# paulrozdeba/varanneal

Measured on AMD Instinct MI355X. Metric: action+grad evals/sec, Lorenz-96 D=20 N=1000, higher is better.
Workload: dtype f64; 1 GPU; lorenz96_D20_N1000_L7_B64_trapezoid; seeds_per_gpu=64, D=20, N=1000, L=7, disc=trapezoid, tile_rows=84, ntiles=12, parallelism=seeds sharded, 64 per GPU, rccl_ranks=1, ramp_launches=16000, launch_mode=hipGraph replay

## Files before the change

include/varanneal_amd.h:

```cpp
#ifndef VARANNEAL_AMD_H
#define VARANNEAL_AMD_H
#include <stdint.h>

#ifdef __cplusplus
extern "C" {
#endif

#define VA_ABI_VERSION 12

enum { VA_OK = 0, VA_EINVAL = -1, VA_ENOMEM = -2, VA_EHIP = -3, VA_EUNSUPPORTED = -4,
       VA_ESTATE = -5 };

enum { VA_DISC_EULER = 0, VA_DISC_TRAPEZOID = 1, VA_DISC_SIMPSON_HERMITE = 2,
       VA_DISC_FORWARDMAP = 3 };

enum { VA_RHS_LORENZ96 = 0, VA_RHS_USER_BASE = 1000 };

enum { VA_MEM_HOST = 0, VA_MEM_DEVICE = 1 };

typedef struct va_problem_s *va_handle;

typedef struct va_problem_desc {
    int32_t struct_size;
    int32_t device;
    int32_t batch;
    int32_t D;
    int32_t N_model;
    int32_t N_data;
    int32_t merr_nskip;
    int32_t L;
    const int32_t *Lidx;
    const double *Y;
    double dt_model;
    int32_t rm_kind;
    double rm;
    const double *rm_array;
    int32_t rf_kind;
    double rf0;
    const double *rf0_array;
    int32_t NP;
    int32_t NPest;
    const int32_t *Pidx;
    const double *P;
    int32_t disc;
    int32_t rhs;
    int32_t lbfgs_m;
    int32_t max_beta;
    int32_t keep_paths;
    int32_t tile_rows;
    int32_t eval_kernel;
    const double *t_model;
    const double *stim;
    int32_t n_stim;
    int32_t p_time_dependent;
    void *stream;
    const double *lower;
    const double *upper;
} va_problem_desc;

typedef struct va_lbfgs_opts {
    int32_t maxcor;
    double ftol;
    double gtol;
    int32_t maxiter;
    int64_t maxfun;
    int32_t maxls;
} va_lbfgs_opts;

int32_t va_abi_version(void);
const char *va_last_error(void);
int va_device_count(int32_t *count);

int va_rhs_load_module(const char *path, int32_t *rhs_id);

int va_eval_plan(const va_problem_desc *desc, int32_t ne, int32_t ghost, int32_t *out);
int va_eval_plan_reach(const va_problem_desc *desc, int32_t ne, int32_t ghost, const int32_t *reach, int32_t *out);

int va_problem_create(const va_problem_desc *desc, va_handle *out);
void va_problem_destroy(va_handle h);

int va_problem_info(va_handle h, int64_t *n_var, int64_t *ld_internal, int32_t *tile_rows,
                    int32_t *ntiles);

#define VA_TUNE_FOLD 1
#define VA_TUNE_GRAD_SC1 2
#define VA_TUNE_PRIO 3
#define VA_TUNE_GRAPH 4
#define VA_TUNE_PERSIST 5
#define VA_TUNE_PERSIST_ROWS 6
#define VA_TUNE_NNET_FUSED 7
int va_problem_tune(va_handle h, int32_t what, int32_t value);
int va_problem_persistent(va_handle h, int32_t *workgroups_per_seed, int32_t *rows_per_workgroup);

int va_problem_eval_kernel(va_handle h, int32_t *eval_kernel, int32_t *run_rows);

int va_action_grad(va_handle h, const double *XP, int64_t ld, int32_t mem, double rf_scale,
                   double *A, double *me, double *fe, double *grad, int64_t ldg);

int va_minimize_lbfgs(va_handle h, double *XP_inout, int64_t ld, int32_t mem, double rf_scale,
                      const va_lbfgs_opts *opts, double *Amin, double *me, double *fe,
                      int32_t *status, int32_t *nit, int64_t *nfev);

int va_anneal(va_handle h, double *XP_inout, int64_t ld, int32_t mem, const double *rf_scale,
              int32_t nbeta, const va_lbfgs_opts *opts, double *ame, double *pest,
              int32_t *status, int32_t *nit, int64_t *nfev, double *minpaths);

int va_get_minpath(va_handle h, int32_t seed, int32_t beta_idx, double *out);

int va_predict(va_handle h, const double *x0, const double *p, int32_t T, double t0,
               int32_t n_steps, int32_t substeps, int32_t every, const double *stim, double *out);

int va_hess_vec(va_handle h, const double *XP, const double *P, const double *V, int32_t npts, int32_t nvec, int64_t ld,
                double rf_scale, int32_t gauss_newton, int32_t tile_rows, double *HV);

int va_blocktri_selinv(va_handle h, int32_t npts, int32_t K, int32_t W, int32_t NPe, const double *Dk, const double *Bk,
                       const double *Pk, const double *Hpp, double *Skk, double *Snk, double *Spk, double *Spp, double *logdet,
                       int32_t *status);

int va_laplace(va_handle h, const double *XP, const double *P, int32_t npts, int64_t ld, const double *rf_scale,
               int32_t gauss_newton, int32_t chunk_pts, double *var_x, double *cov_xx, double *cov_px, double *cov_pp,
               double *logdet, int32_t *status);

int va_predict_tangent(va_handle h, const double *x0, const double *p, const double *V0, int32_t T, int32_t nvec, double t0,
                       int32_t n_steps, int32_t substeps, int32_t every, const double *stim, double *out, double *dX,
                       double *var, double *cov);

int va_hmc(va_handle h, double *XP, int64_t ld, int32_t mem, double rf_scale, int32_t n_iter, int32_t n_leap, const double *eps,
           double jitter, const double *minv, int64_t minv_n, uint64_t seed, const double *noise, int32_t thin,
           const int64_t *keep_idx, int32_t n_keep_idx, double *mean, double *var, double *A_trace, double *dH, int32_t *accepted,
           int32_t *n_divergent, double *kept);
int va_hmc_noise(uint64_t seed, int32_t chain, int32_t iteration, int64_t n, uint32_t *words, double *normals, double *uniforms);

int va_eval_timed(va_handle h, double rf_scale, int32_t iters, float *elapsed_ms);
int va_eval_timed_prepare(va_handle h, double rf_scale, int32_t iters);

int va_lbfgs_timed(va_handle h, int32_t iters, float *ms_update, float *ms_direction);
int va_eval_ls_timed(va_handle h, double rf_scale, int32_t iters, float *ms_eval);

int va_read_eval_outputs(va_handle h, double *A, double *me, double *fe, double *grad, int64_t ldg);

int va_debug_read_partials(va_handle h, double *out, int64_t n);

int va_debug_read_persist(va_handle h, double *out, int64_t n);

int va_get_counters(va_handle h, int64_t *eval_launches, int64_t *seed_evals, int64_t *cycles);

typedef struct va_comm_s *va_comm;
#define VA_COMM_ID_BYTES 128
int va_comm_unique_id(char id[VA_COMM_ID_BYTES]);
int va_comm_create(const char id[VA_COMM_ID_BYTES], int32_t world, int32_t rank, int32_t device, va_comm *out);
void va_comm_destroy(va_comm c);
int va_gather_results(va_handle h, va_comm c, int32_t nbeta, double *table, int32_t *status);

enum { VA_ACT_SIGMOID = 0,
       VA_ACT_TANH = 1, VA_ACT_LINEAR = 2,
       VA_ACT_RELU = 3,
       VA_ACT_SOFTPLUS = 4,
       VA_ACT_USER_BASE = 1000  };

typedef struct va_nnet_desc {
    int32_t struct_size;
    int32_t device;
    int32_t batch;
    int32_t n_layers;
    const int32_t *structure;
    int32_t M;
    int32_t L_in, L_out;
    const int32_t *Lidx_in;
    const int32_t *Lidx_out;
    const double *data_in;
    const double *data_out;
    double rm_in, rm_out;
    double rf0;
    int32_t NP, NPest;
    const int32_t *Pidx;
    const double *P;
    int32_t activation;
    int32_t lbfgs_m;
    int32_t max_beta;
    int32_t keep_paths;
    void *stream;
    const double *rm_in_matrix;
    const double *rm_out_matrix;
} va_nnet_desc;

int va_act_load_module(const char *path, int32_t *act_id);

int va_nnet_problem_create(const va_nnet_desc *desc, va_handle *out);

#ifdef __cplusplus
}
#endif
#endif
```

varanneal_amd/_build.py:

```python
import os
import subprocess
import sys

HERE = os.path.dirname(os.path.abspath(__file__))
CSRC = os.path.join(HERE, "csrc")
OUT = os.path.join(HERE, "libvaranneal_amd.so")
SOURCES = ["va_capi.hip", "va_kernels.hip", "va_eval5.hip", "va_lbfgsb.hip", "va_nnet.hip", "va_hmc.hip"]
HEADERS = ["va_core.h", "va_tile2.h", "va_tile3.h", "va_tile4.h", "va_tile5.h", "va_eval3.h", "va_eval4.h", "va_eval5.h", "va_eval_flat.h", "va_epilogue.h", "va_persist.h", "va_persist_geo.h", "va_predict.h", "va_predict_geo.h", "va_predict_tlm.h", "va_predict_tlm_geo.h", "va_hvp.h", "va_hvp_geo.h", "va_selinv.h", "va_selinv_geo.h", "va_hmc.h", "va_hmc_geo.h", "va_eval_geo.h", "va_measure.h", "va_device.h", "va_nnet.h", "va_nnet_geo.h", "va_nnet_kernels.h", os.path.join("..", "..", "include", "varanneal_amd.h")]
HIPCC = os.environ.get("HIPCC", "/opt/rocm/bin/hipcc")
SCHED = ["-mllvm", "-amdgpu-sched-strategy=iterative-maxocc"]
FLAGS = ["--offload-arch=gfx950", "-O3", "-std=c++17", "-fPIC", "-shared", "-Wall", "-Wno-unused-function", "-ldl"] + SCHED


def needs_build():
    if not os.path.exists(OUT):
        return True
    t = os.path.getmtime(OUT)
    deps = [os.path.join(CSRC, f) for f in SOURCES + HEADERS] + [os.path.abspath(__file__)]
    return any(os.path.getmtime(d) > t for d in deps)


def _compile_link(out, defines, verbose):
    from concurrent.futures import ThreadPoolExecutor
    objdir = os.path.join(HERE, "build", os.path.basename(out).replace(".so", ""))
    os.makedirs(objdir, exist_ok=True)
    cflags = [f for f in FLAGS if f not in ("-shared", "-ldl")]

    def stale(obj, dep, cmd):
        try:
            with open(dep) as fh:
                txt = fh.read()
            if txt.split("\n", 1)[0] != "# " + " ".join(cmd):
                return True
            t = os.path.getmtime(obj)
            files = txt.split(":", 1)[1].replace("\\\n", " ").split()
            return any(os.path.getmtime(f) > t for f in files)
        except (OSError, IndexError):
            return True

    def one(src):
        obj = os.path.join(objdir, src.replace(".hip", ".o"))
        dep = obj + ".d"
        cmd = [HIPCC] + cflags + defines + ["-c", "-o", obj, os.path.join(CSRC, src)]
        if not stale(obj, dep, cmd):
            return obj
        if verbose:
            print(" ".join(cmd), flush=True)
        subprocess.check_call(cmd + ["-MD", "-MF", dep + ".tmp"])
        with open(dep + ".tmp") as fh:
            body = fh.read()
        with open(dep, "w") as fh:
            fh.write("# " + " ".join(cmd) + "\n" + body)
        os.remove(dep + ".tmp")
        return obj
    with ThreadPoolExecutor(max_workers=min(len(SOURCES), os.cpu_count() or 1)) as ex:
        objs = list(ex.map(one, SOURCES))
    cmd = [HIPCC, "--offload-arch=gfx950", "-shared", "-fPIC", "-o", out] + objs + ["-ldl"]
    if verbose:
        print(" ".join(cmd), flush=True)
    subprocess.check_call(cmd)
    return out


def build_stamps(verbose=True):
    return _compile_link(os.path.join(HERE, "libvaranneal_amd_stamps.so"), ["-DVA_STAMPS"], verbose)


def build_variant(tag, defines, verbose=True):
    return _compile_link(os.path.join(HERE, "libvaranneal_amd_%s.so" % tag), list(defines), verbose)


def build(force=False, verbose=True):
    if not force and not needs_build():
        return OUT
    return _compile_link(OUT, [], verbose)


if __name__ == "__main__":
    if "--variant" in sys.argv:
        i = sys.argv.index("--variant")
        build_variant(sys.argv[i + 1], sys.argv[i + 2:])
    elif "--stamps" in sys.argv:
        build_stamps()
    else:
        build(force="--force" in sys.argv)
```

varanneal_amd/_capi.py:

```python
import ctypes as C
import os

import numpy as np

_HERE = os.path.dirname(os.path.abspath(__file__))
LIB_PATH = os.environ.get("VARANNEAL_AMD_LIB", os.path.join(_HERE, "libvaranneal_amd.so"))

VA_OK = 0
VA_EUNSUPPORTED = -4
ABI_VERSION = 12
ERRNAMES = {-1: "VA_EINVAL", -2: "VA_ENOMEM", -3: "VA_EHIP", -4: "VA_EUNSUPPORTED", -5: "VA_ESTATE"}
DISC = {"euler": 0, "trapezoid": 1, "SimpsonHermite": 2, "forwardmap": 3}
RHS = {"lorenz96": 0}
MEM_HOST, MEM_DEVICE = 0, 1

c_dp = C.POINTER(C.c_double)
c_ip = C.POINTER(C.c_int32)
c_lp = C.POINTER(C.c_int64)


class VaLibraryError(RuntimeError):
    pass


# ... 43 lines not shown
                ("maxiter", C.c_int32), ("maxfun", C.c_int64), ("maxls", C.c_int32)]


def make_opts(opt_args=None):
    o = dict(opt_args or {})
    return LbfgsOpts(int(o.get("maxcor", 10)), float(o.get("ftol", 2.2204460492503131e-09)),
                     float(o.get("gtol", 1e-5)), int(min(int(o.get("maxiter", 15000)), 2 ** 31 - 1)),
                     int(o.get("maxfun", 15000)), int(o.get("maxls", 20)))


def _f64(a):
    return np.ascontiguousarray(a, dtype=np.float64)


def make_desc(batch, D, N_model, Y, Lidx, dt_model, RM, RF0, P, Pidx, disc="trapezoid",
              rhs="lorenz96", merr_nskip=1, lbfgs_m=10, max_beta=1, keep_paths=0, tile_rows=0,
              eval_kernel=0, device=0, stream=None, t_model=None, stim=None, p_time_dependent=False, bounds=None):
    Y = _f64(Y)
    N_data, L = Y.shape
    Lidx = np.ascontiguousarray(Lidx, dtype=np.int32)
    Pidx = np.ascontiguousarray(Pidx, dtype=np.int32)
    P = _f64(P)
    if p_time_dependent:
        if P.ndim == 2:
            P = np.ascontiguousarray(np.broadcast_to(P, (batch,) + P.shape))
        if P.ndim != 3 or P.shape[:2] != (batch, N_model):
            raise ValueError("time-dependent P must have shape (batch, N_model, NP)")
    elif P.ndim == 1:
        P = np.ascontiguousarray(np.broadcast_to(P, (batch, P.shape[0])))
    keep = [Y, Lidx, Pidx, P]
    d = ProblemDesc()
    d.struct_size = C.sizeof(ProblemDesc)
    d.device, d.batch, d.D, d.N_model, d.N_data = device, batch, D, N_model, N_data
    d.merr_nskip, d.L = merr_nskip, L
    d.Lidx = Lidx.ctypes.data_as(c_ip)
    d.Y = Y.ctypes.data_as(c_dp)
    d.dt_model = float(dt_model)
    if isinstance(RM, np.ndarray):
        rm = _f64(RM)
        if rm.shape not in [(N_data, L), (N_data, L, L)]:
            raise ValueError("RM array must have shape (N_data, L) or (N_data, L, L)")
        keep.append(rm)
        d.rm_kind, d.rm, d.rm_array = rm.ndim - 1, 0.0, rm.ctypes.data_as(c_dp)
    else:
        d.rm_kind, d.rm, d.rm_array = 0, float(RM), None
    if isinstance(RF0, np.ndarray):
        rf = _f64(RF0)
        if rf.shape not in [(N_model - 1, D), (N_model - 1, D, D)]:
            raise ValueError("RF0 array must have shape (N_model-1, D) or (N_model-1, D, D)")
        keep.append(rf)
        d.rf_kind, d.rf0, d.rf0_array = rf.ndim - 1, 0.0, rf.ctypes.data_as(c_dp)
    else:
        d.rf_kind, d.rf0, d.rf0_array = 0, float(RF0), None
    d.NP, d.NPest = P.shape[-1], len(Pidx)
    d.p_time_dependent = 1 if p_time_dependent else 0
    d.Pidx = Pidx.ctypes.data_as(c_ip)
    d.P = P.ctypes.data_as(c_dp)
    d.disc = DISC[disc] if isinstance(disc, str) else int(disc)
    d.rhs = RHS[rhs] if isinstance(rhs, str) else int(rhs)
    d.lbfgs_m, d.max_beta, d.keep_paths, d.tile_rows = lbfgs_m, max_beta, keep_paths, tile_rows
    d.eval_kernel = eval_kernel
    if t_model is not None:
        tm = _f64(t_model)
        if tm.shape != (N_model,):
            raise ValueError("t_model must have shape (N_model,)")
        keep.append(tm)
        d.t_model = tm.ctypes.data_as(c_dp)
    else:
        d.t_model = None
    if stim is not None:
        st = _f64(stim)
        st = st.reshape(N_model, -1)
        keep.append(st)
        d.stim, d.n_stim = st.ctypes.data_as(c_dp), st.shape[1]
    else:
        d.stim, d.n_stim = None, 0
    d.stream = stream
    d.lower = d.upper = None
    if bounds is not None:
        n_var = N_model * (D + len(Pidx)) if p_time_dependent else N_model * D + len(Pidx)
        if len(bounds) != n_var:
            raise ValueError("bounds must have one (lo, hi) pair per entry of the path vector (%d), got %d" % (n_var, len(bounds)))
        lo = np.array([-np.inf if b[0] is None else b[0] for b in bounds], dtype=np.float64)
        hi = np.array([np.inf if b[1] is None else b[1] for b in bounds], dtype=np.float64)
        keep += [lo, hi]
        d.lower, d.upper = lo.ctypes.data_as(c_dp), hi.ctypes.data_as(c_dp)
    return d, keep


_lib = None


def lib():
    global _lib
    if _lib is not None:
        return _lib
    if not os.path.exists(LIB_PATH):
        raise VaLibraryError("%s not found: build it with `python -m varanneal_amd._build` "
                             "(hipcc --offload-arch=gfx950). There is no CPU fallback." % LIB_PATH)
    try:
        L = C.CDLL(LIB_PATH)
    except OSError as e:
        raise VaLibraryError("cannot load %s: %s" % (LIB_PATH, e))
    h = C.c_void_p
    L.va_abi_version.restype = C.c_int32
    if L.va_abi_version() != ABI_VERSION:
        raise VaLibraryError("%s has ABI version %d, this binding expects %d: rebuild it with "
                             "`python -m varanneal_amd._build --force`" % (LIB_PATH, L.va_abi_version(), ABI_VERSION))
    L.va_last_error.restype = C.c_char_p
    L.va_device_count.argtypes = [c_ip]
    L.va_problem_create.argtypes = [C.POINTER(ProblemDesc), C.POINTER(h)]
    L.va_nnet_problem_create.argtypes = [C.POINTER(NnetDesc), C.POINTER(h)]
    L.va_rhs_load_module.argtypes = [C.c_char_p, c_ip]
    L.va_act_load_module.argtypes = [C.c_char_p, c_ip]
    L.va_eval_plan.argtypes = [C.POINTER(ProblemDesc), C.c_int32, C.c_int32, C.POINTER(C.c_int32)]
    L.va_eval_plan_reach.argtypes = [C.POINTER(ProblemDesc), C.c_int32, C.c_int32, C.POINTER(C.c_int32), C.POINTER(C.c_int32)]
    L.va_problem_destroy.argtypes = [h]
    L.va_problem_destroy.restype = None
    L.va_problem_info.argtypes = [h, c_lp, c_lp, c_ip, c_ip]
    L.va_action_grad.argtypes = [h, C.c_void_p, C.c_int64, C.c_int32, C.c_double, C.c_void_p,
                                 C.c_void_p, C.c_void_p, C.c_void_p, C.c_int64]
    L.va_minimize_lbfgs.argtypes = [h, C.c_void_p, C.c_int64, C.c_int32, C.c_double,
                                    C.POINTER(LbfgsOpts), c_dp, c_dp, c_dp, c_ip, c_ip, c_lp]
    L.va_anneal.argtypes = [h, C.c_void_p, C.c_int64, C.c_int32, c_dp, C.c_int32,
                            C.POINTER(LbfgsOpts), c_dp, c_dp, c_ip, c_ip, c_lp, c_dp]
    L.va_get_minpath.argtypes = [h, C.c_int32, C.c_int32, c_dp]
    L.va_predict.argtypes = [h, c_dp, c_dp, C.c_int32, C.c_double, C.c_int32, C.c_int32, C.c_int32, c_dp, c_dp]
    L.va_predict_tangent.argtypes = [h, c_dp, c_dp, c_dp, C.c_int32, C.c_int32, C.c_double, C.c_int32, C.c_int32, C.c_int32] + [c_dp] * 5
    L.va_predict_tangent.restype = C.c_int
    L.va_hess_vec.argtypes = [h, c_dp, c_dp, c_dp, C.c_int32, C.c_int32, C.c_int64, C.c_double, C.c_int32, C.c_int32, c_dp]
    L.va_hess_vec.restype = C.c_int
    L.va_blocktri_selinv.argtypes = [h, C.c_int32, C.c_int32, C.c_int32, C.c_int32] + [c_dp] * 9 + [c_ip]
    L.va_blocktri_selinv.restype = C.c_int
    L.va_laplace.argtypes = [h, c_dp, c_dp, C.c_int32, C.c_int64, c_dp, C.c_int32, C.c_int32] + [c_dp] * 5 + [c_ip]
    L.va_laplace.restype = C.c_int
    L.va_hmc.argtypes = [h, C.c_void_p, C.c_int64, C.c_int32, C.c_double, C.c_int32, C.c_int32, c_dp, C.c_double, c_dp, C.c_int64,
                         C.c_uint64, c_dp, C.c_int32, c_lp, C.c_int32, c_dp, c_dp, c_dp, c_dp, c_ip, c_ip, c_dp]
    L.va_hmc.restype = C.c_int
    L.va_hmc_noise.argtypes = [C.c_uint64, C.c_int32, C.c_int32, C.c_int64, C.POINTER(C.c_uint32), c_dp, c_dp]
    L.va_hmc_noise.restype = C.c_int
    L.va_eval_timed.argtypes = [h, C.c_double, C.c_int32, C.POINTER(C.c_float)]
    L.va_eval_timed_prepare.argtypes = [h, C.c_double, C.c_int32]
    L.va_get_counters.argtypes = [h, c_lp, c_lp, c_lp]
    L.va_comm_unique_id.argtypes = [C.c_char_p]
    L.va_comm_create.argtypes = [C.c_char_p, C.c_int32, C.c_int32, C.c_int32, C.POINTER(h)]
    L.va_comm_destroy.argtypes = [h]
    L.va_comm_destroy.restype = None
    L.va_gather_results.argtypes = [h, h, C.c_int32, c_dp, c_ip]
    L.va_lbfgs_timed.argtypes = [h, C.c_int32, C.POINTER(C.c_float), C.POINTER(C.c_float)]
    L.va_eval_ls_timed.argtypes = [h, C.c_double, C.c_int32, C.POINTER(C.c_float)]
    L.va_read_eval_outputs.argtypes = [h, C.c_void_p, C.c_void_p, C.c_void_p, C.c_void_p, C.c_int64]
    L.va_debug_read_partials.argtypes = [h, c_dp, C.c_int64]
    L.va_problem_eval_kernel.argtypes = [h, c_ip, c_ip]
    L.va_problem_tune.argtypes = [h, C.c_int32, C.c_int32]
    L.va_debug_read_persist.argtypes = [h, c_dp, C.c_int64]
    L.va_debug_read_persist.restype = C.c_int
    L.va_problem_persistent.argtypes = [h, c_ip, c_ip]
    L.va_problem_persistent.restype = C.c_int
    for fn in ("va_device_count", "va_rhs_load_module", "va_act_load_module", "va_eval_plan", "va_eval_plan_reach", "va_problem_eval_kernel", "va_problem_tune", "va_problem_create", "va_nnet_problem_create",
               "va_problem_info", "va_action_grad",
               "va_minimize_lbfgs", "va_anneal", "va_get_minpath", "va_predict", "va_eval_timed", "va_eval_timed_prepare",
               "va_get_counters", "va_debug_read_partials", "va_read_eval_outputs", "va_lbfgs_timed", "va_eval_ls_timed",
               "va_comm_unique_id", "va_comm_create", "va_gather_results"):
        getattr(L, fn).restype = C.c_int
    _lib = L
    return L


EXPORTS = ["va_abi_version", "va_last_error", "va_device_count", "va_rhs_load_module", "va_act_load_module", "va_eval_plan", "va_eval_plan_reach", "va_problem_eval_kernel", "va_problem_tune", "va_problem_create",
           "va_problem_destroy", "va_problem_info", "va_action_grad", "va_minimize_lbfgs",
           "va_anneal", "va_get_minpath", "va_predict", "va_predict_tangent", "va_hess_vec", "va_blocktri_selinv", "va_laplace", "va_hmc", "va_hmc_noise", "va_eval_timed", "va_eval_timed_prepare", "va_problem_persistent", "va_debug_read_persist", "va_get_counters", "va_nnet_problem_create", "va_debug_read_partials",
           "va_read_eval_outputs", "va_lbfgs_timed", "va_eval_ls_timed", "va_comm_unique_id", "va_comm_create", "va_comm_destroy",
           "va_gather_results"]


def check(rc):
    if rc != VA_OK:
        raise (VaUnsupported if rc == VA_EUNSUPPORTED else VaError)(rc, lib().va_last_error().decode("utf-8", "replace"))


def eval_plan(batch, D, N_model, disc, ne, ghost=0, rm_array=False, rm_full=False, rf_array=False, rf_full=False,
              merr_nskip=1, tile_rows=0, eval_kernel=0, bounded=False, p_time_dependent=False, reach=None, Lidx=None,
              builtin=False):
    d = ProblemDesc()
    d.struct_size = C.sizeof(ProblemDesc)
    d.rhs = 0 if builtin else 1000
    d.batch, d.D, d.N_model, d.merr_nskip = batch, D, N_model, merr_nskip
    d.N_data = (N_model - 1) // merr_nskip + 1
    d.rm_kind = (2 if rm_full else 1) if rm_array else 0
    d.rf_kind = (2 if rf_full else 1) if rf_array else 0
    d.disc = DISC[disc] if isinstance(disc, str) else int(disc)
    d.tile_rows, d.eval_kernel = tile_rows, eval_kernel
    d.p_time_dependent = 1 if p_time_dependent else 0
    dummy = (C.c_double * 1)()
    if bounded:
        d.lower = C.cast(dummy, c_dp); d.upper = C.cast(dummy, c_dp)
    out = (C.c_int32 * 4)()
    if reach is not None and Lidx is not None and len(Lidx) > 0:
        li = np.ascontiguousarray(Lidx, dtype=np.int32)
        d.L = len(li)
        d.Lidx = li.ctypes.data_as(c_ip)
        r = (C.c_int32 * 4)(*[int(v) for v in reach])
        check(lib().va_eval_plan_reach(C.byref(d), int(ne), int(ghost), r, out))
    else:
        check(lib().va_eval_plan(C.byref(d), int(ne), int(ghost), out))
    return (out[0], out[1], out[2], out[3]) if out[0] else None


def hmc_noise(seed, chain, iteration, n):
    n = int(n)
    words = np.empty((n + 1, 4), np.uint32); normals = np.empty(n); uniforms = np.empty(2)
    check(lib().va_hmc_noise(int(seed) & (2 ** 64 - 1), int(chain), int(iteration), n, words.ctypes.data_as(C.POINTER(C.c_uint32)),
                             normals.ctypes.data_as(c_dp), uniforms.ctypes.data_as(c_dp)))
    return words, normals, uniforms


_modules = {}


def load_rhs_module(path):
    path = os.path.abspath(path)
    if path not in _modules:
        rid = C.c_int32()
        check(lib().va_rhs_load_module(path.encode(), C.byref(rid)))
        _modules[path] = rid.value
    return _modules[path]


_act_modules = {}


def load_act_module(path):
    path = os.path.abspath(path)
    if path not in _act_modules:
        aid = C.c_int32()
        check(lib().va_act_load_module(path.encode(), C.byref(aid)))
        _act_modules[path] = aid.value
    return _act_modules[path]


class Comm(object):

    @staticmethod
    def unique_id():
        buf = C.create_string_buffer(128)
        check(lib().va_comm_unique_id(buf))
        return buf.raw

    def __init__(self, uid, world, rank, device=0):
        self._L = lib()
        self.world, self.rank = world, rank
        self._c = C.c_void_p()
        check(self._L.va_comm_create(uid, world, rank, device, C.byref(self._c)))

    def close(self):
        if getattr(self, "_c", None) is not None and self._c.value:
            self._L.va_comm_destroy(self._c)
            self._c = C.c_void_p()

    __del__ = close


class Problem(object):

    def __init__(self, batch, D, N_model, Y, Lidx, dt_model, RM, RF0, P, Pidx, **kw):
        self._L = lib()
        self.desc, self._keep = make_desc(batch, D, N_model, Y, Lidx, dt_model, RM, RF0, P, Pidx, **kw)
        self.B, self.D, self.N = batch, D, N_model
        self.NP, self.NPest = self.desc.NP, self.desc.NPest
        self.n_var = N_model * D + self.NPest
        if self.desc.p_time_dependent:
            self.n_var = N_model * (D + self.NPest)
            self.NPe_t, self.NPt = self.NPest, self.NP
            self.N, self.D, self.NP, self.NPest = 1, self.n_var, 0, 0
        self.max_beta = self.desc.max_beta
        self._h = C.c_void_p()
        check(self._L.va_problem_create(C.byref(self.desc), C.byref(self._h)))

    def close(self):
        if getattr(self, "_h", None) is not None and self._h.value:
            self._L.va_problem_destroy(self._h)
            self._h = C.c_void_p()

    __del__ = close

    def __enter__(self):
        return self

    def __exit__(self, *a):
        self.close()

    def info(self):
        nv, ld = C.c_int64(), C.c_int64()
        T, nt = C.c_int32(), C.c_int32()
        check(self._L.va_problem_info(self._h, C.byref(nv), C.byref(ld), C.byref(T), C.byref(nt)))
        ek, rr = C.c_int32(), C.c_int32()
        check(self._L.va_problem_eval_kernel(self._h, C.byref(ek), C.byref(rr)))
        return dict(n_var=nv.value, ld=ld.value, tile_rows=T.value, ntiles=nt.value, eval_kernel=ek.value,
                    run_rows=rr.value)

    TUNE = {"fold": 1, "grad_sc1": 2, "prio": 3, "graph": 4, "persist": 5, "persist_rows": 6, "nnet_fused": 7}

    def debug_read_persist(self, n):
        out = np.empty(n)
        check(self._L.va_debug_read_persist(self._h, out.ctypes.data_as(c_dp), n))
        return out

    def persistent(self):
        g, t = C.c_int32(), C.c_int32()
        on = self._L.va_problem_persistent(self._h, C.byref(g), C.byref(t))
        return (g.value, t.value) if on else None

    def tune(self, **knobs):
        for k, v in knobs.items():
            check(self._L.va_problem_tune(self._h, self.TUNE[k], int(v)))

    def _xp(self, XP):
        XP = _f64(XP)
        if XP.shape != (self.B, self.n_var):
            raise ValueError("XP must have shape (B, N*D+NPest) = (%d, %d), got %s" %
                             (self.B, self.n_var, XP.shape))
        return XP

    def action_grad(self, XP, rf_scale=1.0, want_grad=True):
        XP = self._xp(XP)
        A = np.empty(self.B); me = np.empty(self.B); fe = np.empty(self.B)
        g = np.empty((self.B, self.n_var)) if want_grad else None
        check(self._L.va_action_grad(self._h, XP.ctypes.data, self.n_var, MEM_HOST, float(rf_scale),
                                     A.ctypes.data, me.ctypes.data, fe.ctypes.data,
                                     g.ctypes.data if want_grad else None, self.n_var))
        return A, me, fe, g

    def action_grad_device(self, xp_ptr, ld, rf_scale, A_ptr, me_ptr, fe_ptr, g_ptr, ldg):
        check(self._L.va_action_grad(self._h, xp_ptr, ld, MEM_DEVICE, float(rf_scale), A_ptr, me_ptr,
                                     fe_ptr, g_ptr, ldg))

    def minimize_lbfgs(self, XP, rf_scale, opt_args=None):
        XP = self._xp(XP).copy()
        o = make_opts(opt_args)
        A = np.empty(self.B); me = np.empty(self.B); fe = np.empty(self.B)
        st = np.empty(self.B, np.int32); nit = np.empty(self.B, np.int32); nfev = np.empty(self.B, np.int64)
        check(self._L.va_minimize_lbfgs(self._h, XP.ctypes.data, self.n_var, MEM_HOST, float(rf_scale),
                                        C.byref(o), A.ctypes.data_as(c_dp), me.ctypes.data_as(c_dp),
                                        fe.ctypes.data_as(c_dp), st.ctypes.data_as(c_ip),
                                        nit.ctypes.data_as(c_ip), nfev.ctypes.data_as(c_lp)))
        return dict(x=XP, A=A, me=me, fe=fe, status=st, nit=nit, nfev=nfev)

    def anneal(self, XP, rf_scale, opt_args=None, want_paths=False, xp_device=None, ld=None):
        rf = _f64(rf_scale)
        nb = rf.shape[0]
        o = make_opts(opt_args)
        B = self.B
        ame = np.empty((B, nb, 3)); pest = np.empty((B, nb, self.NPest))
        st = np.empty((B, nb), np.int32); nit = np.empty((B, nb), np.int32); nfev = np.empty((B, nb), np.int64)
        mp = np.empty((B, nb, self.N * self.D + self.NP)) if want_paths else None
        if xp_device is None:
            XP = self._xp(XP).copy()
            ptr, stride, mem = XP.ctypes.data, self.n_var, MEM_HOST
        else:
            ptr, stride, mem = xp_device, ld, MEM_DEVICE
        check(self._L.va_anneal(self._h, ptr, stride, mem, rf.ctypes.data_as(c_dp), nb, C.byref(o),
                                ame.ctypes.data_as(c_dp), pest.ctypes.data_as(c_dp),
                                st.ctypes.data_as(c_ip), nit.ctypes.data_as(c_ip),
                                nfev.ctypes.data_as(c_lp), mp.ctypes.data_as(c_dp) if want_paths else None))
        return dict(x=XP if xp_device is None else None, A=ame[:, :, 0], me=ame[:, :, 1],
                    fe=ame[:, :, 2], pest=pest, status=st, nit=nit, nfev=nfev, minpaths=mp)

    def predict(self, x0, p, n_steps, t0=0.0, substeps=1, every=1, stim=None):
        if not isinstance(self.desc, ProblemDesc):
            raise NotImplementedError("predict: a network handle has no differential equation to integrate")
        D, NP = self.desc.D, self.desc.NP
        x0 = _f64(x0).reshape(-1, D)
        T = x0.shape[0]
        p = _f64(p).reshape(-1, NP) if NP else np.zeros((T, 0))
        if p.shape[0] == 1 and T > 1:
            p = np.ascontiguousarray(np.broadcast_to(p, (T, NP)))
        if p.shape[0] != T:
            raise ValueError("predict: %d states but %d parameter vectors" % (T, p.shape[0]))
        n_steps, substeps, every = int(n_steps), int(substeps), int(every)
        st = None
        if stim is not None:
            st = _f64(stim).reshape(max(n_steps, 0) + 1, -1)
            if st.shape[1] != self.desc.n_stim and self.desc.n_stim:
                raise ValueError("predict: the stimulus must have %d rows of %d column(s)" % (n_steps + 1, self.desc.n_stim))
        out = np.empty((T, n_steps // every + 1 if every >= 1 and n_steps >= 1 else 1, D))
        check(self._L.va_predict(self._h, x0.ctypes.data_as(c_dp), p.ctypes.data_as(c_dp), T, float(t0), n_steps, substeps,
                                 every, st.ctypes.data_as(c_dp) if st is not None else None, out.ctypes.data_as(c_dp)))
        return out

    def predict_tangent(self, x0, p, V0, n_steps, t0=0.0, substeps=1, every=1, stim=None, want=("dx", "var")):
        if not isinstance(self.desc, ProblemDesc):
            raise NotImplementedError("predict_tangent: a network handle has no differential equation to integrate")
        bad = set(want) - {"dx", "var", "cov"}
        if bad:
            raise ValueError("predict_tangent: want holds 'dx', 'var', 'cov', not %s" % sorted(bad))
        D, NP, nw = self.desc.D, self.desc.NP, self.desc.D + self.NPest
        x0 = _f64(x0).reshape(-1, D)
        T = x0.shape[0]
        p = _f64(p).reshape(-1, NP) if NP else np.zeros((T, 0))
        if p.shape[0] == 1 and T > 1:
            p = np.ascontiguousarray(np.broadcast_to(p, (T, NP)))
        if p.shape[0] != T:
            raise ValueError("predict_tangent: %d states but %d parameter vectors" % (T, p.shape[0]))
        V0 = _f64(V0)
        if V0.size == 0:
            raise ValueError("predict_tangent: at least one direction (nvec = 0)")
        if V0.shape[-1:] != (nw,) or V0.size % (T * nw):
            raise ValueError("predict_tangent: V0 must have shape (%d, nvec, D + NPest = %d), got %s" % (T, nw, V0.shape))
        V0 = V0.reshape(T, -1, nw)
        nvec = V0.shape[1]
        n_steps, substeps, every = int(n_steps), int(substeps), int(every)
        st = None
        if stim is not None:
            st = _f64(stim).reshape(max(n_steps, 0) + 1, -1)
            if st.shape[1] != self.desc.n_stim and self.desc.n_stim:
                raise ValueError("predict_tangent: the stimulus must have %d rows of %d column(s)" % (n_steps + 1, self.desc.n_stim))
        n_out = n_steps // every + 1 if every >= 1 and n_steps >= 1 else 1
        r = dict(out=np.empty((T, n_out, D)))
        for name, shape in (("dx", (T, nvec, n_out, D)), ("var", (T, n_out, D)), ("cov", (T, n_out, D, D))):
            if name in want:
                r[name] = np.empty(shape)
        ptr = lambda a: a.ctypes.data_as(c_dp) if a is not None else None
        check(self._L.va_predict_tangent(self._h, ptr(x0), ptr(p), ptr(V0), T, nvec, float(t0), n_steps, substeps, every, ptr(st),
                                         ptr(r["out"]), ptr(r.get("dx")), ptr(r.get("var")), ptr(r.get("cov"))))
        return r

    def hess_vec(self, XP, V, rf_scale, P=None, gauss_newton=False, tile_rows=0):
        if not isinstance(self.desc, ProblemDesc):
            raise NotImplementedError("hess_vec: the network action has no second derivatives here (ODE handles only)")
        n = self.n_var
        XP = _f64(XP).reshape(-1, n)
        npts = XP.shape[0]
        V = _f64(V)
        one = V.ndim == 2 and npts == 1
        V = V.reshape(npts, -1, n)
        NP = self.desc.NP
        if P is None:
            P = np.ctypeslib.as_array(self.desc.P, shape=(NP,)) if (NP and not self.desc.p_time_dependent) else np.zeros(NP)
        P = _f64(P).reshape(-1, NP) if NP else np.zeros((npts, 0))
        if P.shape[0] == 1 and npts > 1:
            P = np.ascontiguousarray(np.broadcast_to(P, (npts, NP)))
        if P.shape[0] != npts:
            raise ValueError("hess_vec: %d points but %d parameter vectors" % (npts, P.shape[0]))
        HV = np.empty_like(V)
        check(self._L.va_hess_vec(self._h, XP.ctypes.data_as(c_dp), P.ctypes.data_as(c_dp), V.ctypes.data_as(c_dp), npts,
                                  V.shape[1], n, float(rf_scale), 1 if gauss_newton else 0, int(tile_rows), HV.ctypes.data_as(c_dp)))
        return HV[0] if one else HV

    def blocktri_selinv(self, Dk, Bk, Pk, Hpp, want=("Skk", "Snk", "Spk", "Spp")):
        Dk = _f64(Dk)
        npts, K, W = Dk.shape[:3]
        Hpp = _f64(Hpp).reshape(npts, -1)
        NPe = int(round(np.sqrt(Hpp.shape[1])))
        Bk, Pk = _f64(Bk).reshape(npts, K - 1, W, W), _f64(Pk).reshape(npts, K, NPe, W)
# ... 164 lines not shown
```

varanneal_amd/csrc/va_capi.hip:

```cpp
#include <dlfcn.h>
#include <link.h>
#include <stdarg.h>
#include <stdio.h>
#include <stdlib.h>
#include <string.h>

#include <algorithm>
#include <memory>
#include <mutex>
#include <string>
#include <vector>

#include "../../include/varanneal_amd.h"
#include "va_device.h"
#include "va_eval_geo.h"
#include "va_nnet.h"
#include "va_eval_flat.h"
#include "va_persist.h"
#include "va_predict.h"
#include "va_predict_tlm.h"
#include "va_hvp.h"
#include "va_selinv.h"
#include "va_hmc.h"

using namespace va;

namespace {

thread_local std::string g_err;

int fail(int code, const char *fmt, ...)
{
    char buf[512];
    va_list ap;
    va_start(ap, fmt);
    vsnprintf(buf, sizeof buf, fmt, ap);
    va_end(ap);
    g_err = buf;
    return code;
}

#define HIPCHK(expr)                                                                       \
    do {                                                                                   \
        hipError_t e_ = (expr);                                                            \
        if (e_ != hipSuccess)                                                              \
            return fail(e_ == hipErrorOutOfMemory ? VA_ENOMEM : VA_EHIP, "%s: %s (%s:%d)", \
                        #expr, hipGetErrorString(e_), __FILE__, __LINE__);                 \
    } while (0)

#define TRY(expr)                       \
    do {                                \
        if (int rc_ = (expr)) return rc_; \
    } while (0)
#define UPLOAD(dst, src, n) h->upload(dst, src, n, #dst)

struct UserRhs {
    ModuleVariant variant;
    std::string path;
    void *dl = nullptr;
    RhsTable table = {};
    HvpTable hvp = {};
    std::vector<int> colp;
};
struct UserAct {
    std::string path;
    void *dl = nullptr;
    NnetActLaunch launch = nullptr;
};
std::vector<UserAct> g_user_act;
std::vector<UserRhs> g_user_rhs;
std::mutex g_user_rhs_mutex;

}

struct va_problem_s {
    Dev dv;
    int device = 0, rhs = 0, keep_paths = 0;
    RhsTable rt = {};
    HvpTable rt_hvp = {};
    NnetActLaunch nn_act = nullptr;
    bool persist = false, tune_persist = true;
    int pz_G = 0, pz_T = 0, pz_maxG = 0;
    void *pz_misc = nullptr;
    size_t pz_xch_bytes = 0;
    bool is_nnet = false;
    bool fold = false;
    bool tune_graph = true;
    hipGraphExec_t timed_gexec = nullptr;
    int timed_chunk = 0;
    Dev timed_dv;
    NnetDev timed_nn;
    double timed_armed_rf = -1.0;
    NnetDev nn;
    hipStream_t stream = nullptr;
    bool own_stream = false;
    std::vector<void *> allocs;
    int *h_nactive = nullptr;
    double *d_rf = nullptr;
    hipEvent_t ev0 = nullptr, ev1 = nullptr;
    int64_t n_eval_launch = 0, n_seed_evals = 0, n_seed_evals_direct = 0, n_cycles = 0;
    int last_nbeta = 0;

    template <class T> int alloc(T **p, size_t n, bool zero = true)
    {
        void *q = nullptr;
        size_t bytes = sizeof(T) * (n ? n : 1);
        HIPCHK(hipMalloc(&q, bytes));
        allocs.push_back(q);
        if (zero) HIPCHK(hipMemsetAsync(q, 0, bytes, stream));
        *p = (T *)q;
        return VA_OK;
    }
    template <class T> int upload(T *dst, const T *src, size_t n, const char *name)
    {
        hipError_t e = hipMemcpyAsync(dst, src, sizeof(T) * n, hipMemcpyHostToDevice, stream);
        if (e != hipSuccess) return fail(VA_EHIP, "H2D %s: %s", name, hipGetErrorString(e));
        return VA_OK;
    }
};

struct HandleDeleter { void operator()(va_problem_s *h) const { va_problem_destroy(h); } };
typedef std::unique_ptr<va_problem_s, HandleDeleter> HandleOwner;

namespace {

void run_eval(va_handle h, int epi)
{
    if (epi != EPI_FINALIZE) h->timed_armed_rf = -1.0;
    h->dv.lsrun = epi == EPI_LS ? 1 : 0;
    EvalOp op{false, h->stream, hipSuccess};
    if (h->is_nnet ? !h->nn.small : !h->fold) {
        h->dv.epi = EPI_NONE;
        if (h->is_nnet) launch_nnet_eval(h->dv, h->nn, h->stream, h->nn_act);
        else h->rt.eval(h->dv, op);
        if (epi == EPI_FINALIZE) launch_finalize_eval(h->dv, h->stream);
        else if (epi == EPI_LS) launch_ls(h->dv, h->stream);
        return;
    }
    h->dv.epi = epi;
    if (h->is_nnet) { launch_nnet_eval(h->dv, h->nn, h->stream, h->nn_act); return; }
    h->rt.eval(h->dv, op);
}

int alloc_solver_state(va_handle h)
{
    Dev &dv = h->dv;
    const Dims &dm = dv.dm;
    const size_t B = dm.B, ld = dm.ld, m = dm.m, max_beta = dv.max_beta;
    const size_t guard = (((size_t)(dm.T + 8) * dm.D + 15) / 16) * 16;
    TRY(h->alloc(&dv.x, B * ld + 2 * guard)); TRY(h->alloc(&dv.g, B * ld));
    TRY(h->alloc(&dv.gt, B * ld)); TRY(h->alloc(&dv.d, B * ld + 2 * guard));
    dv.x += guard; dv.d += guard;
    TRY(h->alloc(&dv.S, B * m * ld)); TRY(h->alloc(&dv.Y, B * m * ld));
    TRY(h->alloc(&dv.st, B));
    TRY(h->alloc(&dv.evp, B * dm.nprow * EP_N));
    dv.npbig = (!h->is_nnet && !dv.cpv && dm.NPt > RHS_MAX_NP) ? dm.NPt - RHS_MAX_NP : 0;
    if (dv.npbig) TRY(h->alloc(&dv.evp_big, B * dm.nprow * dv.npbig));
    if (dv.cpv) TRY(h->alloc(&dv.evv, B * dm.nprow * dv.cpv));
    TRY(h->alloc(&dv.upp, B * dm.nchunks * dv.ups));
    TRY(h->alloc(&dv.dpp, B * dm.nchunks * DP_N));
    TRY(h->alloc(&h->d_rf, max_beta));
    TRY(h->alloc(&dv.ame, B * max_beta * 3));
    TRY(h->alloc(&dv.pest, B * max_beta * (dm.NPest ? dm.NPest : 1)));
    TRY(h->alloc(&dv.status, B * max_beta)); TRY(h->alloc(&dv.nit, B * max_beta));
    TRY(h->alloc(&dv.nfev, B * max_beta));
    if (h->keep_paths) TRY(h->alloc(&dv.minpaths, B * max_beta * (size_t)(dm.ND + dm.NP), false));
    if (dm.bounded) {
        TRY(h->alloc(&dv.lb_z, B * ld)); TRY(h->alloc(&dv.lb_r, B * ld)); TRY(h->alloc(&dv.lb_xp, B * ld));
        TRY(h->alloc(&dv.lb_t, B * ld)); TRY(h->alloc(&dv.lb_iwhere, B * ld));
        TRY(h->alloc(&dv.lb_mat, B * 3 * m * m)); TRY(h->alloc(&dv.lb_dtd, B));
    }
    TRY(h->alloc(&dv.cnt_eval, B * CNT_STRIDE)); TRY(h->alloc(&dv.cnt_upd, B * CNT_STRIDE)); TRY(h->alloc(&dv.cnt_dir, B * CNT_STRIDE));
    TRY(h->alloc(&dv.n_active, 1));
    TRY(h->alloc(&dv.n_evals, 1));
    TRY(h->alloc(&dv.outA, B)); TRY(h->alloc(&dv.outme, B)); TRY(h->alloc(&dv.outfe, B));
    dv.rf_ladder = h->d_rf;
    return VA_OK;
}

int finish_create(va_handle h)
{
    hipError_t e = hipHostMalloc((void **)&h->h_nactive, 4 * sizeof(int), hipHostMallocDefault);
    if (e != hipSuccess) return fail(VA_ENOMEM, "hipHostMalloc: %s", hipGetErrorString(e));
    e = hipEventCreate(&h->ev0);
    if (e == hipSuccess) e = hipEventCreate(&h->ev1);
    if (e != hipSuccess) return fail(VA_EHIP, "hipEventCreate: %s", hipGetErrorString(e));
    e = hipStreamSynchronize(h->stream);
    if (e != hipSuccess) return fail(VA_EHIP, "create sync: %s", hipGetErrorString(e));
    launch_init_states(h->dv, PH_IDLE, 1.0, h->stream);
    return VA_OK;
}

int copy_in(va_handle h, const double *XP, int64_t ld, int32_t mem)
{
    const Dims &dm = h->dv.dm;
    const size_t w = sizeof(double) * (dm.ND + dm.NPest);
    HIPCHK(hipMemcpy2DAsync(h->dv.x, sizeof(double) * dm.ld, XP, sizeof(double) * ld, w, dm.B,
                            mem == VA_MEM_DEVICE ? hipMemcpyDeviceToDevice : hipMemcpyHostToDevice,
                            h->stream));
    return VA_OK;
}

int copy_out(va_handle h, const double *src, double *dst, int64_t ld, int32_t mem)
{
    const Dims &dm = h->dv.dm;
    const size_t w = sizeof(double) * (dm.ND + dm.NPest);
    HIPCHK(hipMemcpy2DAsync(dst, sizeof(double) * ld, src, sizeof(double) * dm.ld, w, dm.B,
                            mem == VA_MEM_DEVICE ? hipMemcpyDeviceToDevice : hipMemcpyDeviceToHost,
                            h->stream));
    return VA_OK;
}

int check_xp(va_handle h, const void *XP, int64_t ld, int32_t mem)
{
    if (!h) return fail(VA_EINVAL, "null handle");
    if (!XP) return fail(VA_EINVAL, "XP is NULL");
    if (ld < h->dv.dm.ND + h->dv.dm.NPest) return fail(VA_EINVAL, "ld (%lld) < n_var (%d)", (long long)ld, h->dv.dm.ND + h->dv.dm.NPest);
    if (mem != VA_MEM_HOST && mem != VA_MEM_DEVICE) return fail(VA_EINVAL, "bad mem kind %d", mem);
    return VA_OK;
}

int set_opts(va_handle h, const va_lbfgs_opts *o)
{
    if (!o) return fail(VA_EINVAL, "opts is NULL");
    if (o->maxls <= 0) return fail(VA_EINVAL, "maxls must be positive");
    if (o->maxcor <= 0) return fail(VA_EINVAL, "maxcor must be positive");
    Opts &d = h->dv.o;
    d.m = o->maxcor < h->dv.dm.m ? o->maxcor : h->dv.dm.m;
    d.maxiter = o->maxiter; d.maxls = o->maxls; d.maxfun = o->maxfun;
    d.ftol = o->ftol; d.gtol = o->gtol;
    return VA_OK;
}

bool profiler_attached()
{
    static const bool attached = [] {
        bool found = false;
        dl_iterate_phdr([](struct dl_phdr_info *info, size_t, void *out) -> int {
            const char *n = info->dlpi_name;
            if (n && (strstr(n, "librocprofiler-sdk.so") || strstr(n, "librocprofiler-sdk-tool"))) { *(bool *)out = true; return 1; }
            return 0;
        }, &found);
        return found;
    }();
    return attached;
}

long long ladder_cycle_bound(const Dev &dv, int nbeta)
{
    const double per_step = (double)dv.o.maxfun + dv.o.maxls + 4.0;
    const double bound = per_step * nbeta;
    return bound > 4e18 ? (long long)4e18 : (long long)bound;
}

int arm_ladder(va_handle h, const double *rf_scale, int nbeta, bool zero_dpp)
{
    Dev &dv = h->dv;
    HIPCHK(hipMemcpyAsync(h->d_rf, rf_scale, sizeof(double) * nbeta, hipMemcpyHostToDevice, h->stream));
    dv.nbeta = nbeta; h->last_nbeta = nbeta;
    *h->h_nactive = dv.dm.B;
    HIPCHK(hipMemcpyAsync(dv.n_active, h->h_nactive, sizeof(int), hipMemcpyHostToDevice, h->stream));
    if (zero_dpp) HIPCHK(hipMemsetAsync(dv.dpp, 0, sizeof(double) * dv.dm.B * dv.dm.nchunks * DP_N, h->stream));
    launch_init_states(dv, PH_START, -1.0, h->stream);
    h->timed_armed_rf = -1.0;
    return VA_OK;
}

int read_progress(va_handle h, void *misc = nullptr)
{
    const Dev &dv = h->dv;
    HIPCHK(hipMemcpyAsync(h->h_nactive, dv.n_active, sizeof(int), hipMemcpyDeviceToHost, h->stream));
    HIPCHK(hipMemcpyAsync(h->h_nactive + 2, dv.n_evals, sizeof(unsigned long long), hipMemcpyDeviceToHost, h->stream));
    if (misc) HIPCHK(hipMemcpyAsync(misc, h->pz_misc, 16, hipMemcpyDeviceToHost, h->stream));
    HIPCHK(hipStreamSynchronize(h->stream));
    return VA_OK;
}

void book_ladder(va_handle h, long long cyc)
{
    h->n_cycles += cyc; h->n_eval_launch += cyc;
    h->n_seed_evals = h->n_seed_evals_direct + (int64_t)*(unsigned long long *)(h->h_nactive + 2);
}

int run_ladder_persist(va_handle h, const double *rf_scale, int nbeta, bool *fell_back);

int run_ladder(va_handle h, const double *rf_scale, int nbeta)
{
    Dev &dv = h->dv;
    if (nbeta < 1 || nbeta > dv.max_beta) return fail(VA_EINVAL, "nbeta=%d outside [1, max_beta=%d]", nbeta, dv.max_beta);
    if (h->persist && h->tune_persist) {
        bool fell_back = false;
        const int rc = run_ladder_persist(h, rf_scale, nbeta, &fell_back);
        if (!fell_back) return rc;
    }
    TRY(arm_ladder(h, rf_scale, nbeta, true));
    if (dv.dm.bounded) launch_clamp_x(dv, h->stream);
    const long long max_cycles = ladder_cycle_bound(dv, nbeta);
    long long cyc = 0;
    int poll = 4;
    hipGraphExec_t gexec = nullptr;
    bool use_graph = h->tune_graph && !profiler_attached();
    auto enqueue = [&](int n) {
// ... 55 lines not shown
    TRY(read_progress(h, &misc));
    HIPCHK(hipGetLastError());
    book_ladder(h, (long long)misc.cycles);
    if (misc.abort_flag == 1) {
        h->persist = false;
        *fell_back = true;
        return VA_OK;
    }
    if (misc.abort_flag == 2) return fail(VA_ESTATE, "ladder did not finish within %lld cycles", max_cycles);
    if (*h->h_nactive > 0) return fail(VA_ESTATE, "persistent ladder ended with %d live seeds", *h->h_nactive);
    return VA_OK;
}

template <class T>
int fetch_table(va_handle h, const T *dev, T *host, int nbeta, int per)
{
    if (!host) return VA_OK;
    const Dev &dv = h->dv;
    HIPCHK(hipMemcpy2DAsync(host, sizeof(T) * nbeta * per, dev, sizeof(T) * dv.max_beta * per,
                            sizeof(T) * nbeta * per, dv.dm.B, hipMemcpyDeviceToHost, h->stream));
    return VA_OK;
}

void colp_refusal(const va_problem_desc *d, const ModuleVariant &mv, char *msg, size_t n)
{
    if (const char *flat_only = flat_only_reason(d)) snprintf(msg, n, "%s", flat_only);
    else if (d->D > 64 && (d->D & 1)) snprintf(msg, n, "odd D = %d > 64 (k_eval3, which has no column-parameter form)", d->D);
    else if (d->D > 64 && mv.kernel != 5) snprintf(msg, n, "a non-autonomous model (model time or stimulus) on the streaming kernel k_eval5");
    else if (d->D <= 64 && !tile4_ok(d->D)) snprintf(msg, n, "D = %d fits neither k_eval4 (even D <= 64 filling a wave) nor k_eval5", d->D);
    else if (d->eval_kernel != 0 && d->eval_kernel != mv.kernel) snprintf(msg, n, "eval_kernel = %d (the module carries kernel %d)", d->eval_kernel, mv.kernel);
    else snprintf(msg, n, "the module's column-run instantiation does not fit this problem (weights, discretisation or run length): regenerate it");
}

struct ModulePlan {
    EvalPlan plan;
    bool variant = false;
    int cps = 0, cpv = 0;
};
int plan_module(const va_problem_desc *d, const UserRhs &u, ModulePlan &mp)
{
    const ModuleVariant &mv = u.variant;
    const bool bigp = d->NP > RHS_MAX_NP;
    mp.plan = plan_eval(d, bigp && !mv.column_params() ? mv.flat_form() : mv.form());
    mp.variant = mp.plan.emode != 1 && variant_key(mp.plan, d) == mv.key();
    if (!mp.variant && mp.plan.emode != 1) mp.plan = plan_eval(d, mv.flat_form());
    if (mp.variant && mv.column_params()) { mp.cps = u.colp[0]; mp.cpv = u.colp[1] * d->D; }
    if (d->NP > RHS_BIG_NP && !mp.cpv) {
        char why[192];
        colp_refusal(d, mv, why, sizeof why);
        return fail(VA_EUNSUPPORTED, "%d parameters: only the column-parameter form on k_eval4 / k_eval5 carries more than %d, "
                                     "and this problem cannot run it: %s", d->NP, RHS_BIG_NP, why);
    }
    if (mp.plan.emode == 4 && mp.cpv > mp.plan.g4.XW)
        return fail(VA_EUNSUPPORTED, "runs of %d rows are too short for %d vector entries on k_eval4", mp.plan.g4.K, mp.cpv);
    return VA_OK;
}


int begin_create(int device, void *stream, int lbfgs_m, int max_beta, int keep_paths, HandleOwner &h)
{
    const int m = lbfgs_m > 0 ? lbfgs_m : 10;
    if (m > MAX_M) return fail(VA_EINVAL, "lbfgs_m=%d > %d", m, MAX_M);
    int ndev = 0;
    HIPCHK(hipGetDeviceCount(&ndev));
    if (device < 0 || device >= ndev) return fail(VA_EINVAL, "device %d of %d", device, ndev);
    HIPCHK(hipSetDevice(device));

    h.reset(new va_problem_s());
    h->device = device; h->keep_paths = keep_paths;
    if (stream) h->stream = (hipStream_t)stream;
    else {
        hipError_t e = hipStreamCreateWithFlags(&h->stream, hipStreamNonBlocking);
        if (e != hipSuccess) return fail(VA_EHIP, "hipStreamCreate: %s", hipGetErrorString(e));
        h->own_stream = true;
    }
    Dev &dv = h->dv;
    memset(&dv, 0, sizeof dv);
    dv.dm.m = m;
    dv.ups = UP_OLD + 4 * m; dv.max_beta = max_beta > 0 ? max_beta : 1; dv.nbeta = 1;
    dv.o.m = m; dv.o.maxiter = 15000; dv.o.maxls = 20; dv.o.maxfun = 15000; dv.o.ftol = 2.2204460492503131e-09; dv.o.gtol = 1e-5;
    return VA_OK;
}

void set_ld(Dims &dm)
{
    dm.ld = ((dm.ND + dm.NPest + 15) / 16) * 16;
    dm.chunk = VEC_CHUNK; dm.nchunks = (dm.ld + VEC_CHUNK - 1) / VEC_CHUNK;
}

int validate_desc(const va_problem_desc *d, UserRhs &user_copy, const UserRhs **user)
{
    if (d->struct_size != (int32_t)sizeof(va_problem_desc)) return fail(VA_EINVAL, "struct_size %d != %zu", d->struct_size, sizeof(va_problem_desc));
    if (d->batch < 1 || d->D < 1 || d->N_model < 2 || d->N_data < 1 || d->L < 0 || d->merr_nskip < 1)
        return fail(VA_EINVAL, "bad sizes (batch=%d D=%d N_model=%d N_data=%d L=%d nskip=%d)", d->batch, d->D, d->N_model, d->N_data, d->L, d->merr_nskip);
    if ((int64_t)(d->N_data - 1) * d->merr_nskip + 1 != d->N_model)
        return fail(VA_EINVAL, "N_model (%d) must equal (N_data-1)*merr_nskip+1 (%lld)", d->N_model,
                    (long long)(d->N_data - 1) * d->merr_nskip + 1);
    if (d->disc < VA_DISC_EULER || d->disc > VA_DISC_FORWARDMAP) return fail(VA_EINVAL, "unknown disc %d", d->disc);
    if (d->disc == VA_DISC_SIMPSON_HERMITE && (d->N_model % 2) == 0)
        return fail(VA_EINVAL, "SimpsonHermite needs an odd number of time points (N_model=%d)", d->N_model);
    *user = nullptr;
    if (d->rhs >= VA_RHS_USER_BASE) {
        std::lock_guard<std::mutex> lock(g_user_rhs_mutex);
        if ((size_t)(d->rhs - VA_RHS_USER_BASE) >= g_user_rhs.size()) return fail(VA_EINVAL, "rhs module id %d was never registered", d->rhs);
        user_copy = g_user_rhs[d->rhs - VA_RHS_USER_BASE];
        *user = &user_copy;
        const RhsTable &t = user_copy.table;
        if (t.NP != d->NP || t.D != d->D || t.NSTIM != d->n_stim)
            return fail(VA_EINVAL, "rhs module %s was generated for D=%d NP=%d n_stim=%d, problem has D=%d NP=%d n_stim=%d",
                        user_copy.path.c_str(), t.D, t.NP, t.NSTIM, d->D, d->NP, d->n_stim);
    } else if (d->rhs != VA_RHS_LORENZ96) return fail(VA_EUNSUPPORTED, "unknown built-in rhs %d", d->rhs);
    if (d->rhs == VA_RHS_LORENZ96 && (d->NP != RhsL96::NP || d->D < 4))
        return fail(VA_EINVAL, "Lorenz-96 needs NP=1 and D>=4 (NP=%d D=%d)", d->NP, d->D);
    if (d->n_stim < 0 || (d->n_stim > 0 && !d->stim)) return fail(VA_EINVAL, "n_stim=%d without a stimulus array", d->n_stim);
    if (d->NP > RHS_BIG_NP && !(*user && !user_copy.colp.empty()))
        return fail(VA_EUNSUPPORTED, "NP=%d > %d: only a generated module in column-parameter form (shared scalars + per-column "
                                     "vectors) carries more, and this model has none", d->NP, RHS_BIG_NP);
    if (d->NPest < 0 || d->NPest > d->NP) return fail(VA_EINVAL, "bad NP/NPest (%d/%d)", d->NP, d->NPest);
    const bool tdp = d->p_time_dependent != 0;
    if (d->NP > RHS_MAX_NP && tdp) return fail(VA_EUNSUPPORTED, "time-dependent parameters: at most %d of them", RHS_MAX_NP);
    if (tdp && d->disc != VA_DISC_TRAPEZOID && d->disc != VA_DISC_SIMPSON_HERMITE)
        return fail(VA_EUNSUPPORTED, "time-dependent parameters: trapezoid and SimpsonHermite only (upstream's euler/forwardmap "
                                     "branches are inconsistent, va_ode.py:345-349)");
    if (tdp && (int64_t)d->N_model * (d->D + d->NPest) > 2000000000LL) return fail(VA_EUNSUPPORTED, "n_var does not fit 32-bit indexing");
    if (!d->Y || (d->L > 0 && !d->Lidx) || !d->P || (d->NPest > 0 && !d->Pidx)) return fail(VA_EINVAL, "null array in desc");
    if ((d->rm_kind && !d->rm_array) || (d->rf_kind && !d->rf0_array)) return fail(VA_EINVAL, "rm/rf array kind without array");
    if ((d->lower != nullptr) != (d->upper != nullptr)) return fail(VA_EINVAL, "lower and upper bounds come together");
    std::vector<char> seen(d->D, 0);
    for (int l = 0; l < d->L; ++l) {
        if (d->Lidx[l] < 0 || d->Lidx[l] >= d->D) return fail(VA_EINVAL, "Lidx[%d]=%d outside [0,D)", l, d->Lidx[l]);
        if (seen[d->Lidx[l]] && d->rm_kind != 2) return fail(VA_EUNSUPPORTED, "Lidx lists state column %d twice", d->Lidx[l]);
        seen[d->Lidx[l]] = 1;
    }
    for (int k = 0; k < d->NPest; ++k)
        if (d->Pidx[k] < 0 || d->Pidx[k] >= d->NP) return fail(VA_EINVAL, "Pidx[%d]=%d outside [0,NP)", k, d->Pidx[k]);
    if (d->lbfgs_m > MAX_M) return fail(VA_EINVAL, "lbfgs_m=%d > %d", d->lbfgs_m, MAX_M);
    if (d->rm_kind < 0 || d->rm_kind > 2) return fail(VA_EINVAL, "rm_kind %d", d->rm_kind);
    if (d->lower) {
        const int nv = tdp ? d->N_model * (d->D + d->NPest) : d->D * d->N_model + d->NPest;
        for (int i = 0; i < nv; ++i)
            if (!(d->lower[i] <= d->upper[i])) return fail(VA_EINVAL, "lower[%d] > upper[%d] (or NaN)", i, i);
    }
    return VA_OK;
}

int plan_problem(va_handle h, const va_problem_desc *d, const UserRhs *user, EvalPlan &plan)
{
    Dev &dv = h->dv;
    h->rhs = d->rhs;
    if (!user) {
        builtin_rhs_table(h->rt);
        builtin_hvp_table(h->rt_hvp);
        EvalForm l96;
        l96.ne = RhsL96s::NE; l96.ghost = RhsL96g::GHOST; l96.has_reach5 = true;
        l96.reach5[0] = t5_xl<RhsL96s>(); l96.reach5[1] = t5_xr<RhsL96s>(); l96.reach5[2] = t5_gl<RhsL96s>(); l96.reach5[3] = t5_gr<RhsL96s>();
        plan = plan_eval(d, l96);
        return VA_OK;
    }
    ModulePlan mp;
    TRY(plan_module(d, *user, mp));
    plan = mp.plan;
    h->rt = user->table;
    h->rt_hvp = user->hvp;
    if (mp.variant) h->rt.eval = user->table.eval_var;
    dv.dm.lin = user->variant.has_linear;
    dv.cps = mp.cps; dv.cpv = mp.cpv;
    dv.cpnsg = (mp.cpv && plan.emode == 5) ? plan.g5.NSG : 0;
    return VA_OK;
}

int fill_dims(va_handle h, const va_problem_desc *d, const EvalPlan &plan)
{
    Dev &dv = h->dv;
    Dims &dm = dv.dm;
    const bool tdp = d->p_time_dependent != 0;
    dm.D = d->D; dm.N = d->N_model; dm.ND = dm.D * dm.N; dm.L = d->L; dm.N_data = d->N_data;
    dm.nskip = d->merr_nskip; dm.NP = d->NP; dm.NPest = d->NPest; dm.B = d->batch;
    dm.disc = d->disc;
    dm.tdp = tdp ? 1 : 0; dm.NPt = d->NP; dm.NPe = d->NPest;
    dm.bounded = (d->lower && d->upper) ? 1 : 0;
    if (tdp) { dm.ND = dm.N * (dm.D + dm.NPe); dm.NP = 0; dm.NPest = 0; }
    set_ld(dm);
    dm.emode = plan.emode; dm.RY = plan.RY; dm.NT = plan.NT; dm.maxr = plan.maxr; dm.T = plan.T; dm.ntiles = plan.ntiles;
    dm.ghost = plan.ghost;
    dv.g4 = plan.g4; dv.g5 = plan.g5;
    if (dm.emode == 4 && (unsigned long long)dm.B * dm.ntiles * dm.ntiles >= (1ull << 32))
        return fail(VA_EUNSUPPORTED, "batch x tiles too large for the wave-private kernel: pass eval_kernel=3");
    dv.ntiles_magic = (unsigned)(((1ull << 32) + dm.ntiles - 1) / dm.ntiles);
    h->fold = (long)dm.B * dm.ntiles <= 8L * 256;
    dm.nprow = dm.ntiles;
    dm.dt = d->dt_model;
    dm.cme = d->L > 0 ? 1.0 / ((double)dm.L * dm.N_data) : 0.0;
    dm.cfe = 1.0 / ((double)dm.D * (dm.N - 1));
    dm.rm = d->rm; dm.rf0 = d->rf0;
    const int npcols = dv.cpv ? dv.cps : d->NP;
    dv.evcols = EP_GP + npcols <= 8 ? 8 : (EP_GP + npcols <= 16 ? 16 : 32);
    dv.gaux = h->fold ? 1 : 0;
    dv.prio = 1;
    return VA_OK;
}

int prepare_kernels(va_handle h)
{
    Dev &dv = h->dv;
    const Dims &dm = dv.dm;
    size_t need = eval_lds_bytes(dv);
    if (dm.emode == 5) { dv.lsrun = 1; need = std::max(need, eval_lds_bytes(dv)); dv.lsrun = 0; }
    const size_t cap = 160 * 1024;
    if (need > cap)
        return fail(VA_EUNSUPPORTED, "a tile of %d rows x D=%d needs %zu B of LDS (> %zu): state too wide for this kernel",
                    dm.T, dm.D, need, cap);
    EvalOp op{true, nullptr, hipSuccess};
    h->rt.eval(dv, op);
    hipError_t e = op.err;
    if (e == hipSuccess && dm.bounded) e = prepare_lbfgsb(dv);
    if (e != hipSuccess) return fail(VA_EHIP, "hipFuncSetAttribute(MaxDynamicSharedMemorySize): %s", hipGetErrorString(e));
    return VA_OK;
}

struct OdeData {
    std::vector<double> Ys, rms, rf_fill, lo, hi;
    std::vector<int> lmap, colp_map;
    size_t LY = 0, np_seed = 0, rm_elems = 0;
    bool warr5 = false;
    int *lmap_d = nullptr, *pidx_d = nullptr, *ystrip_d = nullptr, *lidx_d = nullptr;
    double *Y_d = nullptr, *rm_d = nullptr, *rf_d = nullptr, *P_d = nullptr, *t_d = nullptr, *st_d = nullptr, *lo_d = nullptr, *hi_d = nullptr;
};

int alloc_problem_data(va_handle h, const va_problem_desc *d, const EvalPlan &plan, OdeData &o)
{
    Dev &dv = h->dv;
    Dims &dm = dv.dm;
    const size_t B = dm.B;
    TRY(h->alloc(&o.lmap_d, dm.D));
    const size_t LY = dm.emode == 5 ? (size_t)dv.g5.LY : (size_t)dm.L;
    o.LY = LY;
    TRY(h->alloc(&o.Y_d, (size_t)dm.N_data * LY + 4 * LY + 16));
    o.Y_d += 2 * (LY / 2) + (LY & 1) * 2;
    if (dm.emode == 5) TRY(h->alloc(&o.ystrip_d, plan.ystrip.size()));
    o.np_seed = dm.tdp ? (size_t)dm.N * dm.NPt : (size_t)dm.NPt;
    TRY(h->alloc(&o.pidx_d, dm.NPe));
    TRY(h->alloc(&o.P_d, B * o.np_seed));
    o.rm_elems = (size_t)dm.N_data * dm.L * (d->rm_kind == 2 ? dm.L : 1);
    o.warr5 = dm.emode == 5 && dv.g5.warr;
    if (o.warr5) {
        TRY(h->alloc(&o.rm_d, (size_t)dm.N_data * LY + 4 * LY + 16));
        o.rm_d += LY;
    } else if (d->rm_kind) TRY(h->alloc(&o.rm_d, o.rm_elems));
    if (d->rm_kind == 2) TRY(h->alloc(&o.lidx_d, dm.L));
    if (o.warr5) {
        TRY(h->alloc(&o.rf_d, (size_t)(dm.N + 3) * dm.D + 16));
        o.rf_d += dm.D;
    } else if (d->rf_kind) TRY(h->alloc(&o.rf_d, (size_t)(dm.N - 1) * dm.D * (d->rf_kind == 2 ? dm.D : 1)));
    if (dm.bounded) {
        const int nv = dm.ND + dm.NPest;
        o.lo.assign(dm.ld, -HUGE_VAL); o.hi.assign(dm.ld, HUGE_VAL);
        for (int i = 0; i < nv; ++i) { o.lo[i] = d->lower[i]; o.hi[i] = d->upper[i]; }
        bool boxed = true;
        for (int i = 0; i < nv; ++i) boxed = boxed && o.lo[i] > -HUGE_VAL && o.hi[i] < HUGE_VAL;
        if (boxed) dm.bounded |= 2;
        TRY(h->alloc(&o.lo_d, (size_t)dm.ld)); TRY(h->alloc(&o.hi_d, (size_t)dm.ld));
    }
    if (d->t_model) TRY(h->alloc(&o.t_d, (size_t)dm.N));
    if (d->n_stim > 0) TRY(h->alloc(&o.st_d, (size_t)dm.N * d->n_stim));
    return VA_OK;
}

int upload_problem_data(va_handle h, const va_problem_desc *d, const UserRhs *user, const EvalPlan &plan, OdeData &o)
{
    Dev &dv = h->dv;
    Dims &dm = dv.dm;
    const size_t B = dm.B, LY = o.LY;
    std::vector<int> perm(dm.L), lidx_sorted(dm.L);
    for (int l = 0; l < dm.L; ++l) perm[l] = l;
    if (d->rm_kind != 2) std::stable_sort(perm.begin(), perm.end(), [&](int a, int b) { return d->Lidx[a] < d->Lidx[b]; });
    for (int l = 0; l < dm.L; ++l) lidx_sorted[l] = d->Lidx[perm[l]];
    o.Ys.assign((size_t)dm.N_data * LY, 0.0);
    for (int n = 0; n < dm.N_data; ++n)
        for (int l = 0; l < dm.L; ++l) o.Ys[(size_t)n * LY + l] = d->Y[(size_t)n * dm.L + perm[l]];
    if (o.warr5 && d->rm_kind == 0) o.rms.assign((size_t)dm.N_data * LY, d->rm);
    if (d->rm_kind == 1) {
        o.rms.assign((size_t)dm.N_data * LY, 0.0);
        for (int n = 0; n < dm.N_data; ++n)
            for (int l = 0; l < dm.L; ++l) o.rms[(size_t)n * LY + l] = d->rm_array[(size_t)n * dm.L + perm[l]];
    }
    o.lmap.assign(dm.D, -1);
    for (int l = 0; l < dm.L; ++l) o.lmap[lidx_sorted[l]] = l;
    dm.obsmask = 0ull;
    if (dm.D <= 64) for (int l = 0; l < dm.L; ++l) dm.obsmask |= 1ull << lidx_sorted[l];
    TRY(UPLOAD(o.lmap_d, o.lmap.data(), dm.D));
    if (dm.emode == 5) { TRY(UPLOAD(o.ystrip_d, plan.ystrip.data(), plan.ystrip.size())); dv.ystrip = o.ystrip_d; }
    TRY(UPLOAD(o.Y_d, o.Ys.data(), (size_t)dm.N_data * LY));
    if (dm.NPe) TRY(UPLOAD(o.pidx_d, d->Pidx, dm.NPe));
    TRY(UPLOAD(o.P_d, d->P, B * o.np_seed));
    if (d->rm_kind || o.warr5) TRY(UPLOAD(o.rm_d, d->rm_kind != 2 ? o.rms.data() : d->rm_array, d->rm_kind != 2 ? o.rms.size() : o.rm_elems));
    if (d->rm_kind == 2) TRY(UPLOAD(o.lidx_d, d->Lidx, dm.L));
    if (o.warr5 && d->rf_kind == 0) o.rf_fill.assign((size_t)(dm.N - 1) * dm.D, d->rf0);
    if (d->rf_kind || o.warr5) TRY(UPLOAD(o.rf_d, d->rf_kind ? d->rf0_array : o.rf_fill.data(), (size_t)(dm.N - 1) * dm.D * (d->rf_kind == 2 ? dm.D : 1)));
    if (dm.bounded) { TRY(UPLOAD(o.lo_d, o.lo.data(), (size_t)dm.ld)); TRY(UPLOAD(o.hi_d, o.hi.data(), (size_t)dm.ld)); }
    dv.pp.lo = o.lo_d; dv.pp.hi = o.hi_d;
    if (d->t_model) TRY(UPLOAD(o.t_d, d->t_model, (size_t)dm.N));
    if (d->n_stim > 0) TRY(UPLOAD(o.st_d, d->stim, (size_t)dm.N * d->n_stim));
    dv.pp.lmap = o.lmap_d; dv.pp.Y = o.Y_d; dv.pp.rf0_arr = (d->rf_kind == 1 || o.warr5) ? o.rf_d : nullptr;
    dv.pp.rf0_full = d->rf_kind == 2 ? o.rf_d : nullptr;
    dv.pp.rm_arr = (d->rm_kind == 1 || o.warr5) ? o.rm_d : nullptr;
    dv.pp.rm_full = d->rm_kind == 2 ? o.rm_d : nullptr; dv.pp.Lidx = o.lidx_d;
    dv.pp.Pidx = o.pidx_d; dv.pp.Pfull = o.P_d;
    if (dv.cpv) {
        const int NT = dv.cps + dv.cpv;
        std::vector<int> pest(d->NP, -1);
        o.colp_map.assign(2 * (size_t)NT, 0);
        for (int k = 0; k < d->NPest; ++k) pest[d->Pidx[k]] = k;
        for (int j = 0; j < NT; ++j) { o.colp_map[j] = user->colp[2 + j]; o.colp_map[NT + j] = pest[o.colp_map[j]]; }
        int *cm_d = nullptr;
        TRY(h->alloc(&cm_d, o.colp_map.size()));
        TRY(UPLOAD(cm_d, o.colp_map.data(), o.colp_map.size()));
        dv.cpmap = cm_d;
    }
    dv.pp.tmodel = o.t_d; dv.pp.stim = o.st_d; dv.pp.nstim = d->n_stim;
    return VA_OK;
}

int choose_persist(va_handle h, const va_problem_desc *d)
{
    Dev &dv = h->dv;
    const Dims &dm = dv.dm;
    const size_t B = dm.B;
    if (dm.bounded || dm.tdp || dm.lin || d->NP > RHS_MAX_NP || dm.emode == 5 || !h->rt.seed) return VA_OK;
    int G = 0, T = 0, ncu = 0;
    HIPCHK(hipDeviceGetAttribute(&ncu, hipDeviceAttributeMultiprocessorCount, d->device));
    h->pz_maxG = ncu / (int)B;
    if (h->pz_maxG < 1 || !persist_geometry(dm.N, dm.D, dm.L, dm.NP, dm.NPest, dm.m, dm.disc, PZ_LDS_BYTES, h->pz_maxG, 0, &G, &T)) return VA_OK;
    Dev dvp = dv;
    dvp.dm.T = T; dvp.dm.ntiles = G;
    EvalOp op{true, nullptr, hipSuccess};
    h->rt.seed(dvp, op);
    if (op.err != hipSuccess) { (void)hipGetLastError(); return VA_OK; }
    h->persist = true; h->pz_G = G; h->pz_T = T;
    const size_t units = B * 2 * (size_t)h->pz_maxG * (size_t)pz_row_granules(dm.D) * 2;
    TRY(h->alloc(&dv.pz.xch, units));
    h->pz_xch_bytes = units * 8;
    unsigned long long *misc = nullptr;
    TRY(h->alloc(&misc, 2 + PZ_NSTAMP));
    h->pz_misc = misc;
    dv.pz.abort_flag = (int *)misc; dv.pz.cycles = misc + 1; dv.pz.stamps = (double *)(misc + 2);
    return VA_OK;
}

int cu_count(int device)
{
    int ncu = 256;
    if (hipDeviceGetAttribute(&ncu, hipDeviceAttributeMultiprocessorCount, device) != hipSuccess) { (void)hipGetLastError(); ncu = 256; }
    return ncu;
}

void fill_nnet_dims(va_handle h, const va_nnet_desc *d, const NnetPlan &p)
{
    Dev &dv = h->dv;
    NnetDev &nn = h->nn;
    memset(&nn, 0, sizeof nn);
    Dims &dm = dv.dm;
    dm.D = p.NDnet; dm.N = d->M; dm.ND = (int)p.nvar; dm.NP = 0; dm.NPest = 0; dm.B = d->batch;
    dm.L = d->L_in + d->L_out; dm.N_data = d->M; dm.nskip = 1; dm.disc = VA_DISC_FORWARDMAP;
    set_ld(dm);
    dm.cme = 1.0 / ((double)(d->L_in + d->L_out) * d->M);
    dm.cfe = d->rf0 / ((double)(p.NDnet - p.s[0]) * d->M);
    dm.rm = d->rm_in; dm.rf0 = d->rf0;
    dv.evcols = 8;
    dm.nprow = p.nprow;
    dm.ntiles = dm.nprow; dm.T = NN_TILE; dm.emode = 0;

    nn.NL = d->n_layers; nn.M = d->M; nn.NDnet = p.NDnet; nn.NDens = p.NDnet * d->M; nn.NP = d->NP; nn.NPest = d->NPest;
    nn.act = d->activation; nn.Lin = d->L_in; nn.Lout = d->L_out; nn.rm_in = d->rm_in; nn.rm_out = d->rm_out;
    nn.mch = p.mch; nn.nmch = p.nmch;
    nn.n0 = p.n0; nn.n1 = p.n1; nn.n2 = p.n2; nn.n3 = p.n3; nn.n4 = p.n4; nn.nraw = p.nraw;
    nn.small = p.small;
    nn.nfb = p.nfb; nn.wfsz = p.wfsz; nn.fb_slots = p.fb_slots; nn.fused = p.fused;
}

int create_nnet_image(va_handle h, const va_nnet_desc *d, const NnetPlan &p)
{
    Dev &dv = h->dv;
    NnetDev &nn = h->nn;
    const Dims &dm = dv.dm;
    const int NL = d->n_layers;
    const size_t B = dm.B;
    int *s_d = nullptr, *off_d = nullptr, *woff_d = nullptr, *boff_d = nullptr, *lin_d = nullptr, *lout_d = nullptr, *pmap_d = nullptr;
    double *din_d = nullptr, *dout_d = nullptr, *P_d = nullptr;
    NnetTile *t1_d = nullptr, *t2_d = nullptr, *t3_d = nullptr;
    TRY(h->alloc(&s_d, NL)); TRY(h->alloc(&off_d, NL + 1)); TRY(h->alloc(&woff_d, NL - 1)); TRY(h->alloc(&boff_d, NL - 1));
    TRY(h->alloc(&lin_d, p.s[0])); TRY(h->alloc(&lout_d, p.s[NL - 1])); TRY(h->alloc(&pmap_d, d->NP));
    TRY(h->alloc(&din_d, (size_t)d->M * d->L_in)); TRY(h->alloc(&dout_d, (size_t)d->M * d->L_out));
    TRY(h->alloc(&P_d, B * d->NP)); TRY(h->alloc(&nn.Pw, B * d->NP));
    TRY(h->alloc(&nn.delta, B * dm.ld));
    TRY(h->alloc(&nn.Xw, B * dm.ld));
    if (p.fold_rows) TRY(h->alloc(&nn.raw, B * nn.nraw * EP_GP));
    TRY(h->alloc(&nn.gpart, B * nn.nmch * (size_t)d->NP));
    int *wfoff_d = nullptr;
    if (p.fb_ok) {
        TRY(h->alloc(&nn.Wf, B * (size_t)nn.wfsz));
        TRY(h->alloc(&wfoff_d, 2 * (NL - 1)));
        TRY(h->alloc(&dv.pz.stamps, (size_t)PZ_NSTAMP));
        TRY(h->alloc(&nn.fb_cu, (size_t)16));
    }
    TRY(h->alloc(&t1_d, p.t1.size())); TRY(h->alloc(&t2_d, p.t2.size())); TRY(h->alloc(&t3_d, p.t3.size()));
    TRY(alloc_solver_state(h));
    TRY(UPLOAD(s_d, p.s.data(), NL)); TRY(UPLOAD(off_d, p.off.data(), NL + 1));
    TRY(UPLOAD(woff_d, p.woff.data(), NL - 1)); TRY(UPLOAD(boff_d, p.boff.data(), NL - 1));
    TRY(UPLOAD(lin_d, p.lin.data(), p.s[0])); TRY(UPLOAD(lout_d, p.lout.data(), p.s[NL - 1])); TRY(UPLOAD(pmap_d, p.pmap.data(), d->NP));
    if (d->L_in) TRY(UPLOAD(din_d, d->data_in, (size_t)d->M * d->L_in));
    if (d->L_out) TRY(UPLOAD(dout_d, d->data_out, (size_t)d->M * d->L_out));
    TRY(UPLOAD(P_d, d->P, B * d->NP));
    if (p.fb_ok) { TRY(UPLOAD(wfoff_d, p.wfoff.data(), 2 * (NL - 1))); nn.wfoff = wfoff_d; }
    TRY(UPLOAD(t1_d, p.t1.data(), p.t1.size())); TRY(UPLOAD(t2_d, p.t2.data(), p.t2.size()));
    if (!p.t3.empty()) TRY(UPLOAD(t3_d, p.t3.data(), p.t3.size()));
    nn.s = s_d; nn.off = off_d; nn.woff = woff_d; nn.boff = boff_d; nn.lmap_in = lin_d; nn.lmap_out = lout_d;
    nn.pmap = pmap_d; nn.din = din_d; nn.dout = dout_d; nn.Pfix = P_d; nn.t1 = t1_d; nn.t2 = t2_d; nn.t3 = t3_d;
    if (d->rm_in_matrix) {
        double *ri = nullptr, *ro = nullptr; int *li = nullptr, *lo = nullptr;
        TRY(h->alloc(&ri, (size_t)d->L_in * d->L_in + 1)); TRY(h->alloc(&ro, (size_t)d->L_out * d->L_out + 1));
        TRY(h->alloc(&li, d->L_in + 1)); TRY(h->alloc(&lo, d->L_out + 1));
        if (d->L_in) { TRY(UPLOAD(ri, d->rm_in_matrix, (size_t)d->L_in * d->L_in)); TRY(UPLOAD(li, d->Lidx_in, d->L_in)); }
        if (d->L_out) { TRY(UPLOAD(ro, d->rm_out_matrix, (size_t)d->L_out * d->L_out)); TRY(UPLOAD(lo, d->Lidx_out, d->L_out)); }
        nn.rmm_in = ri; nn.rmm_out = ro; nn.lidx_in = li; nn.lidx_out = lo;
    }
    if (p.fb_ok) {
        const hipError_t e = prepare_nnet_fb(nn, h->nn_act);
        if (e != hipSuccess) { (void)hipGetLastError(); nn.Wf = nullptr; }
    }
    return VA_OK;
}

}

extern "C" {

int32_t va_abi_version(void) { return VA_ABI_VERSION; }
const char *va_last_error(void) { return g_err.c_str(); }

int va_device_count(int32_t *count)
{
    if (!count) return fail(VA_EINVAL, "count is NULL");
    int n = 0;
    HIPCHK(hipGetDeviceCount(&n));
    *count = n;
    return VA_OK;
}

int va_eval_plan_reach(const va_problem_desc *d, int32_t ne, int32_t ghost, const int32_t *reach, int32_t *out)
{
    if (!d || !out) return fail(VA_EINVAL, "null argument");
    if (d->struct_size != (int32_t)sizeof(va_problem_desc)) return fail(VA_EINVAL, "struct_size %d != %zu", d->struct_size, sizeof(va_problem_desc));
    out[0] = out[1] = out[2] = out[3] = 0;
    if ((ne <= 0 && ghost <= 0) || d->D < 1 || d->N_model < 2 || d->batch < 1) return VA_OK;
    if (d->L > 0 && !d->Lidx) return fail(VA_EINVAL, "Lidx is NULL");
    EvalForm form;
    form.ne = ne; form.ghost = ghost; form.has_reach5 = reach != nullptr;
    if (reach) for (int k = 0; k < 4; ++k) form.reach5[k] = reach[k];
    const VariantKey key = variant_key(plan_eval(d, form), d);
    out[0] = key.kernel; out[1] = key.disc; out[2] = key.K; out[3] = key.W;
    return VA_OK;
}

int va_eval_plan(const va_problem_desc *d, int32_t ne, int32_t ghost, int32_t *out)
{
    return va_eval_plan_reach(d, ne, ghost, nullptr, out);
}

int va_rhs_load_module(const char *path, int32_t *rhs_id)
{
    if (!path || !rhs_id) return fail(VA_EINVAL, "null argument");
    std::lock_guard<std::mutex> lock(g_user_rhs_mutex);
    for (size_t i = 0; i < g_user_rhs.size(); ++i)
        if (g_user_rhs[i].path == path) { *rhs_id = VA_RHS_USER_BASE + (int32_t)i; return VA_OK; }
    UserRhs u;
    u.path = path;
    u.dl = dlopen(path, RTLD_NOW | RTLD_LOCAL);
    if (!u.dl) return fail(VA_EINVAL, "dlopen(%s): %s", path, dlerror());
    typedef void (*info_fn)(int *);
    typedef int (*table_fn)(RhsTable *, int);
    table_fn table = (table_fn)dlsym(u.dl, "va_user_rhs_table");
    if (!table) { dlclose(u.dl); return fail(VA_EINVAL, "%s lacks va_user_rhs_table", path); }
    RhsTable &t = u.table;
    const int table_bytes = table(&t, (int)sizeof(RhsTable));
    if (table_bytes != (int)sizeof(RhsTable) || t.dev_bytes != (int)sizeof(Dev) || t.seed_bytes != (int)sizeof(SeedState)
        || t.predict_bytes != (int)sizeof(PredictArgs)) {
        dlclose(u.dl);
        return fail(VA_EINVAL, "%s was built against different headers (table %d vs %zu bytes, Dev %d vs %zu bytes): rebuild it", path,
                    table_bytes, sizeof(RhsTable), t.dev_bytes, sizeof(Dev));
    }
    typedef int (*hvp_fn)(HvpTable *, int);
    if (hvp_fn hv = (hvp_fn)dlsym(u.dl, "va_user_hvp_table")) {
        const int hb = hv(&u.hvp, (int)sizeof(HvpTable));
        if (hb != (int)sizeof(HvpTable) || u.hvp.hvp_bytes != (int)sizeof(HvpArgs) || u.hvp.tlm_bytes != (int)sizeof(PredictTlmArgs)) {
            dlclose(u.dl);
            return fail(VA_EINVAL, "%s was built against different headers (HvpTable %d vs %zu bytes): rebuild it", path, hb, sizeof(HvpTable));
        }
    }
    if (info_fn vinfo = (info_fn)dlsym(u.dl, "va_user_variant_info")) {
        int uv[UV_N];
        vinfo(uv);
        u.variant = ModuleVariant::decode(uv);
        if (!t.eval_var) u.variant.kernel = 0;
    }
    if (info_fn cmap = (info_fn)dlsym(u.dl, "va_user_colp_map")) {
        u.colp.assign(2 + RHS_MAX_NP + (size_t)CP_VMAX * (t.D > 0 ? t.D : 1), 0);
        cmap(u.colp.data());
        u.colp.resize(2 + (size_t)u.colp[0] + (size_t)u.colp[1] * t.D);
    }
    if (u.colp.empty()) u.variant.n_colp_vectors = 0;
    if (t.NP < 0 || (t.NP > RHS_BIG_NP && u.colp.empty())) {
        dlclose(u.dl);
        return fail(VA_EUNSUPPORTED, "%s: NP=%d > %d and no column-parameter form", path, t.NP, RHS_BIG_NP);
    }
    g_user_rhs.push_back(u);
    *rhs_id = VA_RHS_USER_BASE + (int32_t)g_user_rhs.size() - 1;
    return VA_OK;
}

int va_act_load_module(const char *path, int32_t *act_id)
{
    if (!path || !act_id) return fail(VA_EINVAL, "null argument");
    std::lock_guard<std::mutex> lock(g_user_rhs_mutex);
    for (size_t i = 0; i < g_user_act.size(); ++i)
        if (g_user_act[i].path == path) { *act_id = VA_ACT_USER_BASE + (int32_t)i; return VA_OK; }
    UserAct u;
    u.path = path;
    u.dl = dlopen(path, RTLD_NOW | RTLD_LOCAL);
    if (!u.dl) return fail(VA_EINVAL, "dlopen(%s): %s", path, dlerror());
    typedef void (*info_fn)(int *);
    info_fn info = (info_fn)dlsym(u.dl, "va_user_act_info");
    u.launch = (NnetActLaunch)dlsym(u.dl, "va_user_act_launch");
    if (!info || !u.launch) { dlclose(u.dl); return fail(VA_EINVAL, "%s lacks va_user_act_info / va_user_act_launch", path); }
    int ai[3] = {0, 0, 0};
    info(ai);
    if (ai[0] != (int)sizeof(Dev) || ai[1] != (int)sizeof(NnetDev) || ai[2] != (int)sizeof(SeedState)) {
        dlclose(u.dl);
        return fail(VA_EINVAL, "%s was built against different headers: rebuild it", path);
    }
    g_user_act.push_back(u);
    *act_id = VA_ACT_USER_BASE + (int32_t)g_user_act.size() - 1;
    return VA_OK;
}

int va_problem_create(const va_problem_desc *d, va_handle *out)
{
    if (!d || !out) return fail(VA_EINVAL, "null argument");
    *out = nullptr;
    UserRhs user_copy;
    const UserRhs *user = nullptr;
    TRY(validate_desc(d, user_copy, &user));
    EvalPlan plan;
    OdeData data;
    HandleOwner h;
    TRY(begin_create(d->device, d->stream, d->lbfgs_m, d->max_beta, d->keep_paths, h));
    TRY(plan_problem(h.get(), d, user, plan));
    TRY(fill_dims(h.get(), d, plan));
    TRY(prepare_kernels(h.get()));
    TRY(alloc_problem_data(h.get(), d, plan, data));
    TRY(alloc_solver_state(h.get()));
    TRY(upload_problem_data(h.get(), d, user, plan, data));
    TRY(choose_persist(h.get(), d));
    TRY(finish_create(h.get()));
    *out = h.release();
    return VA_OK;
}

int va_nnet_problem_create(const va_nnet_desc *d, va_handle *out)
{
    if (!d || !out) return fail(VA_EINVAL, "null argument");
    *out = nullptr;
    if (d->struct_size != (int32_t)sizeof(va_nnet_desc)) return fail(VA_EINVAL, "struct_size %d != %zu", d->struct_size, sizeof(va_nnet_desc));
    if (d->batch < 1 || d->n_layers < 2 || d->M < 1 || !d->structure) return fail(VA_EINVAL, "bad sizes (batch=%d n_layers=%d M=%d)", d->batch, d->n_layers, d->M);
    if ((d->rm_in_matrix != nullptr) != (d->rm_out_matrix != nullptr)) return fail(VA_EINVAL, "rm_in_matrix and rm_out_matrix come together");
    NnetActLaunch user_act = nullptr;
    if (d->activation >= VA_ACT_USER_BASE) {
        std::lock_guard<std::mutex> lock(g_user_rhs_mutex);
        if ((size_t)(d->activation - VA_ACT_USER_BASE) >= g_user_act.size()) return fail(VA_EINVAL, "activation module id %d was never registered", d->activation);
        user_act = g_user_act[d->activation - VA_ACT_USER_BASE].launch;
    } else if (d->activation < VA_ACT_SIGMOID || d->activation > VA_ACT_SOFTPLUS) return fail(VA_EUNSUPPORTED, "unknown activation %d", d->activation);
    NnetPlan plan;
    const char *why = "";
    if (int rc = plan_nnet(d, cu_count(d->device), plan, &why)) return fail(rc, "%s", why);
    HandleOwner h;
    TRY(begin_create(d->device, d->stream, d->lbfgs_m, d->max_beta, d->keep_paths, h));
    h->rhs = -1; h->is_nnet = true; h->nn_act = user_act;
    fill_nnet_dims(h.get(), d, plan);
    TRY(create_nnet_image(h.get(), d, plan));
    TRY(finish_create(h.get()));
    *out = h.release();
    return VA_OK;
}

void va_problem_destroy(va_handle h)
{
    if (!h) return;
    (void)hipSetDevice(h->device);
    if (h->stream) (void)hipStreamSynchronize(h->stream);
    if (h->timed_gexec) (void)hipGraphExecDestroy(h->timed_gexec);
    for (void *p : h->allocs) (void)hipFree(p);
    if (h->h_nactive) (void)hipHostFree(h->h_nactive);
    if (h->ev0) (void)hipEventDestroy(h->ev0);
    if (h->ev1) (void)hipEventDestroy(h->ev1);
    if (h->own_stream && h->stream) (void)hipStreamDestroy(h->stream);
    delete h;
}

int va_problem_info(va_handle h, int64_t *n_var, int64_t *ld_internal, int32_t *tile_rows, int32_t *ntiles)
{
    if (!h) return fail(VA_EINVAL, "null handle");
    if (n_var) *n_var = h->dv.dm.ND + h->dv.dm.NPest;
    if (ld_internal) *ld_internal = h->dv.dm.ld;
    if (tile_rows) *tile_rows = h->dv.dm.T;
    if (ntiles) *ntiles = h->dv.dm.ntiles;
    return VA_OK;
}

int va_problem_eval_kernel(va_handle h, int32_t *eval_kernel, int32_t *run_rows)
{
    if (!h) return fail(VA_EINVAL, "null handle");
    if (eval_kernel) *eval_kernel = h->is_nnet ? 0 : h->dv.dm.emode;
    if (run_rows) *run_rows = h->is_nnet ? 0 : h->dv.dm.maxr;
    return VA_OK;
}

int va_problem_persistent(va_handle h, int32_t *workgroups_per_seed, int32_t *rows_per_workgroup)
{
    if (!h) return 0;
    const bool on = h->persist && h->tune_persist;
    if (workgroups_per_seed) *workgroups_per_seed = on ? h->pz_G : 0;
    if (rows_per_workgroup) *rows_per_workgroup = on ? h->pz_T : 0;
    return on ? 1 : 0;
}

int va_action_grad(va_handle h, const double *XP, int64_t ld, int32_t mem, double rf_scale,
                   double *A, double *me, double *fe, double *grad, int64_t ldg)
{
    int rc = check_xp(h, XP, ld, mem);
    if (rc) return rc;
    if (!A || !me || !fe) return fail(VA_EINVAL, "A/me/fe must not be NULL");
    if (grad && ldg < h->dv.dm.ND + h->dv.dm.NPest) return fail(VA_EINVAL, "ldg < n_var");
    HIPCHK(hipSetDevice(h->device));
    Dev &dv = h->dv;
    if ((rc = copy_in(h, XP, ld, mem))) return rc;
    launch_init_states(dv, PH_START, rf_scale, h->stream);
    h->timed_armed_rf = rf_scale;
    run_eval(h, EPI_FINALIZE);
    const hipMemcpyKind k = mem == VA_MEM_DEVICE ? hipMemcpyDeviceToDevice : hipMemcpyDeviceToHost;
    HIPCHK(hipMemcpyAsync(A, dv.outA, sizeof(double) * dv.dm.B, k, h->stream));
    HIPCHK(hipMemcpyAsync(me, dv.outme, sizeof(double) * dv.dm.B, k, h->stream));
    HIPCHK(hipMemcpyAsync(fe, dv.outfe, sizeof(double) * dv.dm.B, k, h->stream));
    if (grad && (rc = copy_out(h, dv.gt, grad, ldg, mem))) return rc;
    HIPCHK(hipStreamSynchronize(h->stream));
    HIPCHK(hipGetLastError());
    h->n_eval_launch += 1; h->n_seed_evals += dv.dm.B; h->n_seed_evals_direct += dv.dm.B;
    return VA_OK;
}

int va_anneal(va_handle h, double *XP, int64_t ld, int32_t mem, const double *rf_scale, int32_t nbeta,
              const va_lbfgs_opts *opts, double *ame, double *pest, int32_t *status, int32_t *nit,
              int64_t *nfev, double *minpaths)
{
    int rc = check_xp(h, XP, ld, mem);
    if (rc) return rc;
    if (!rf_scale) return fail(VA_EINVAL, "rf_scale is NULL");
    if (minpaths && !h->dv.minpaths) return fail(VA_ESTATE, "minpaths requested but the problem was created with keep_paths=0");
    if ((rc = set_opts(h, opts))) return rc;
    HIPCHK(hipSetDevice(h->device));
    Dev &dv = h->dv;
    if ((rc = copy_in(h, XP, ld, mem))) return rc;
    if ((rc = run_ladder(h, rf_scale, nbeta))) return rc;
    if ((rc = copy_out(h, dv.x, XP, ld, mem))) return rc;
    if ((rc = fetch_table(h, dv.ame, ame, nbeta, 3))) return rc;
    if (dv.dm.NPest && (rc = fetch_table(h, dv.pest, pest, nbeta, dv.dm.NPest))) return rc;
    if ((rc = fetch_table(h, dv.status, status, nbeta, 1))) return rc;
    if ((rc = fetch_table(h, dv.nit, nit, nbeta, 1))) return rc;
    if ((rc = fetch_table(h, (const int64_t *)dv.nfev, nfev, nbeta, 1))) return rc;
    if ((rc = fetch_table(h, dv.minpaths, minpaths, nbeta, dv.dm.ND + dv.dm.NP))) return rc;
    HIPCHK(hipStreamSynchronize(h->stream));
    return VA_OK;
}

int va_minimize_lbfgs(va_handle h, double *XP, int64_t ld, int32_t mem, double rf_scale,
                      const va_lbfgs_opts *opts, double *Amin, double *me, double *fe,
                      int32_t *status, int32_t *nit, int64_t *nfev)
{
    if (!h) return fail(VA_EINVAL, "null handle");
    const int B = h->dv.dm.B;
    std::vector<double> ame((size_t)B * 3);
    int rc = va_anneal(h, XP, ld, mem, &rf_scale, 1, opts, ame.data(), nullptr, status, nit, nfev, nullptr);
    if (rc) return rc;
    for (int b = 0; b < B; ++b) {
        if (Amin) Amin[b] = ame[3 * b];
        if (me) me[b] = ame[3 * b + 1];
        if (fe) fe[b] = ame[3 * b + 2];
    }
    return VA_OK;
}

int va_predict(va_handle h, const double *x0, const double *p, int32_t T, double t0, int32_t n_steps, int32_t substeps,
               int32_t every, const double *stim, double *out)
{
    if (!h) return fail(VA_EINVAL, "null handle");
    if (!x0 || !p || !out) return fail(VA_EINVAL, "x0 / p / out must not be NULL");
    if (T < 1 || n_steps < 1 || substeps < 1 || every < 1)
        return fail(VA_EINVAL, "T, n_steps, substeps and every must be at least 1 (T=%d n_steps=%d substeps=%d every=%d)", T, n_steps, substeps, every);
    if (h->is_nnet) return fail(VA_EUNSUPPORTED, "a network handle has no differential equation to integrate");
    const Dims &dm = h->dv.dm;
    const int nstim = h->dv.pp.nstim;
    if (nstim > 0 && !stim) return fail(VA_EINVAL, "the model takes a stimulus of %d column(s): pass its %d rows from t0 on", nstim, n_steps + 1);
    if (nstim == 0 && stim) return fail(VA_EINVAL, "the model takes no stimulus, but one was passed");
    if (!h->rt.predict)
        return fail(VA_EUNSUPPORTED, "the model has no flat form f(x, i, p) for the integrator to call (more than %d parameters: "
                                     "its module carries the column-parameter form only)", RHS_BIG_NP);
    if ((int64_t)n_steps * substeps > 2000000000LL) return fail(VA_EUNSUPPORTED, "n_steps x substeps does not fit 32-bit indexing");
    PredictArgs a;
    a.T = T; a.D = dm.D; a.NP = dm.NPt; a.nstim = nstim; a.n_steps = n_steps; a.substeps = substeps; a.every = every;
    a.n_out = n_steps / every + 1; a.t0 = t0; a.dt = dm.dt;
    if (!plan_predict(a.D, T, a.NP, nstim, a.geo)) return fail(VA_EUNSUPPORTED, "va_predict: D=%d: %s", a.D, a.geo.why);
    HIPCHK(hipSetDevice(h->device));
    const size_t nx = (size_t)T * a.D, np = (size_t)T * a.NP, ns = (size_t)(n_steps + 1) * nstim, no = (size_t)T * a.n_out * a.D;
    double *buf = nullptr;
    HIPCHK(hipMalloc((void **)&buf, sizeof(double) * (nx + np + ns + no + 1)));
    struct Free { double *q; ~Free() { (void)hipFree(q); } } guard{buf};
    double *x0_d = buf, *p_d = x0_d + nx, *st_d = p_d + np, *out_d = st_d + ns;
    HIPCHK(hipMemcpyAsync(x0_d, x0, sizeof(double) * nx, hipMemcpyHostToDevice, h->stream));
    if (np) HIPCHK(hipMemcpyAsync(p_d, p, sizeof(double) * np, hipMemcpyHostToDevice, h->stream));
    if (ns) HIPCHK(hipMemcpyAsync(st_d, stim, sizeof(double) * ns, hipMemcpyHostToDevice, h->stream));
    a.x0 = x0_d; a.p = p_d; a.stim = ns ? st_d : nullptr; a.out = out_d;
    const hipError_t e = h->rt.predict(a, h->stream);
    if (e != hipSuccess) {
        (void)hipStreamSynchronize(h->stream);
        return fail(VA_EHIP, "k_predict launch: %s", hipGetErrorString(e));
    }
    HIPCHK(hipMemcpyAsync(out, out_d, sizeof(double) * no, hipMemcpyDeviceToHost, h->stream));
    HIPCHK(hipStreamSynchronize(h->stream));
    HIPCHK(hipGetLastError());
    return VA_OK;
}

int va_predict_tangent(va_handle h, const double *x0, const double *p, const double *V0, int32_t T, int32_t nvec, double t0,
                       int32_t n_steps, int32_t substeps, int32_t every, const double *stim, double *out, double *dX, double *var,
                       double *cov)
{
    if (!h) return fail(VA_EINVAL, "null handle");
    if (!x0 || !p || !V0 || !out) return fail(VA_EINVAL, "x0 / p / V0 / out must not be NULL");
    if (T < 1 || n_steps < 1 || substeps < 1 || every < 1)
        return fail(VA_EINVAL, "T, n_steps, substeps and every must be at least 1 (T=%d n_steps=%d substeps=%d every=%d)", T, n_steps, substeps, every);
    if (nvec < 1) return fail(VA_EINVAL, "nvec must be at least 1 (nvec=%d)", nvec);
    if (h->is_nnet) return fail(VA_EUNSUPPORTED, "a network handle has no differential equation to integrate");
    const Dims &dm = h->dv.dm;
    const int nstim = h->dv.pp.nstim;
    if (nstim > 0 && !stim) return fail(VA_EINVAL, "the model takes a stimulus of %d column(s): pass its %d rows from t0 on", nstim, n_steps + 1);
    if (nstim == 0 && stim) return fail(VA_EINVAL, "the model takes no stimulus, but one was passed");
    if (dm.lin) return fail(VA_EUNSUPPORTED, "va_predict_tangent: the module's dense linear part was split off (LINEAR): build it with linear=False");
    if (!h->rt.predict || !h->rt_hvp.predict_tlm)
        return fail(VA_EUNSUPPORTED, "va_predict_tangent: the model has no flat form f(x, i, p) to differentiate (more than %d parameters: "
                                     "its module carries the column-parameter form only)", RHS_BIG_NP);
    if ((int64_t)n_steps * substeps > 2000000000LL) return fail(VA_EUNSUPPORTED, "n_steps x substeps does not fit 32-bit indexing");
    PredictTlmArgs a;
    a.T = T; a.D = dm.D; a.NP = dm.NPt; a.NPest = dm.NPest; a.nvec = nvec; a.nstim = nstim; a.n_steps = n_steps; a.substeps = substeps;
    a.every = every; a.n_out = n_steps / every + 1; a.t0 = t0; a.dt = dm.dt; a.Pidx = h->dv.pp.Pidx;
    const bool reduce = var || cov;
    const size_t per = predict_tlm_traj_doubles(a.D, a.NP, a.NPest, nvec, a.n_out, cov != nullptr);
    const long C = predict_tlm_chunk_trajs(per, T);
    if (C < 1)
        return fail(VA_EUNSUPPORTED, "va_predict_tangent: one trajectory with %d direction(s) and %d output row(s) takes %.1f MiB of device "
// ... 306 lines not shown
    const size_t tot = nx + np + 2 * nv + npart + nd + nb + npk + nh + nws + nd + npk + nh + C + nvar + nxx + npx;
    double *buf = nullptr;
    HIPCHK(hipMalloc((void **)&buf, sizeof(double) * (tot + 1) + sizeof(int) * C));
    struct Free { double *q; ~Free() { (void)hipFree(q); } } guard{buf};
    double *x_d = buf, *p_d = x_d + nx, *v_d = p_d + np, *hv_d = v_d + nv, *part_d = hv_d + nv, *d_d = part_d + npart, *b_d = d_d + nd,
           *pk_d = b_d + nb, *h_d = pk_d + npk, *ws_d = h_d + nh, *skk_d = ws_d + nws, *spk_d = skk_d + nd, *spp_d = spk_d + npk,
           *ld_d = spp_d + nh, *var_d = ld_d + C, *xx_d = var_d + nvar, *px_d = xx_d + nxx;
    int *st_d = (int *)(px_d + npx + 1);
    hipError_t e = launch_hcolour(hg, v_d, C, h->stream);
    if (e != hipSuccess) return fail(VA_EHIP, "k_hcolour launch: %s", hipGetErrorString(e));
    for (int p0 = 0; p0 < npts; p0 += C) {
        const int n = npts - p0 < C ? npts - p0 : C;
        HIPCHK(hipMemcpyAsync(x_d, XP + (size_t)p0 * ld, sizeof(double) * n * ld, hipMemcpyHostToDevice, h->stream));
        if (hd.NPt) HIPCHK(hipMemcpyAsync(p_d, P + (size_t)p0 * hd.NPt, sizeof(double) * n * hd.NPt, hipMemcpyHostToDevice, h->stream));
        HIPCHK(hipMemsetAsync(hv_d, 0, sizeof(double) * (size_t)n * nvec * ld, h->stream));
        for (int q0 = 0; q0 < n;) {
            int q1 = q0 + 1;
            while (q1 < n && rf_scale[p0 + q1] == rf_scale[p0 + q0]) ++q1;
            e = hvp_on_device(h, geo, x_d + (size_t)q0 * ld, p_d + (size_t)q0 * hd.NPt, v_d, hv_d + (size_t)q0 * nvec * ld,
                              part_d + (size_t)q0 * nvec * geo.ntiles * hd.NPt, q1 - q0, nvec, ld, rf_scale[p0 + q0], gauss_newton);
            if (e != hipSuccess) {
                (void)hipStreamSynchronize(h->stream);
                return fail(VA_EHIP, "k_hvp launch: %s", hipGetErrorString(e));
            }
            q0 = q1;
        }
        HblocksArgs ba;
        ba.h = hg; ba.HV = hv_d; ba.Dk = d_d; ba.Bk = b_d; ba.Pk = pk_d; ba.Hpp = h_d; ba.npts = n;
        SelinvArgs sa;
        sa.g = sg; sa.g.grid = n;
        sa.Dk = d_d; sa.Bk = b_d; sa.Pk = pk_d; sa.Hpp = h_d; sa.Skk = skk_d; sa.Snk = nullptr; sa.Spk = spk_d; sa.Spp = spp_d;
        sa.logdet = ld_d; sa.status = st_d; sa.ws = ws_d; sa.npts = n;
        UnpackArgs ua;
        ua.h = hg; ua.Skk = skk_d; ua.Spk = spk_d; ua.var_x = var_d; ua.cov_xx = cov_xx ? xx_d : nullptr; ua.cov_px = cov_px ? px_d : nullptr;
        ua.npts = n;
        if ((e = launch_hblocks(ba, h->stream)) != hipSuccess || (e = launch_selinv(sa, h->stream)) != hipSuccess
            || (e = launch_laplace_unpack(ua, h->stream)) != hipSuccess) {
            (void)hipStreamSynchronize(h->stream);
            return fail(VA_EHIP, "k_hblocks / k_selinv / k_laplace_unpack launch: %s", hipGetErrorString(e));
        }
        HIPCHK(hipMemcpyAsync(var_x + (size_t)p0 * ND, var_d, sizeof(double) * n * ND, hipMemcpyDeviceToHost, h->stream));
        if (cov_xx) HIPCHK(hipMemcpyAsync(cov_xx + (size_t)p0 * ND * hd.D, xx_d, sizeof(double) * n * ND * hd.D, hipMemcpyDeviceToHost, h->stream));
        if (cov_px && NPe) HIPCHK(hipMemcpyAsync(cov_px + (size_t)p0 * NPe * ND, px_d, sizeof(double) * n * NPe * ND, hipMemcpyDeviceToHost, h->stream));
        if (cov_pp && NPe) HIPCHK(hipMemcpyAsync(cov_pp + (size_t)p0 * NPe * NPe, spp_d, sizeof(double) * n * NPe * NPe, hipMemcpyDeviceToHost, h->stream));
        HIPCHK(hipMemcpyAsync(logdet + p0, ld_d, sizeof(double) * n, hipMemcpyDeviceToHost, h->stream));
        HIPCHK(hipMemcpyAsync(status + p0, st_d, sizeof(int) * n, hipMemcpyDeviceToHost, h->stream));
        HIPCHK(hipStreamSynchronize(h->stream));
    }
    HIPCHK(hipGetLastError());
    return VA_OK;
}

int va_get_minpath(va_handle h, int32_t seed, int32_t beta_idx, double *out)
{
    if (!h || !out) return fail(VA_EINVAL, "null argument");
    const Dev &dv = h->dv;
    if (!dv.minpaths) return fail(VA_ESTATE, "problem was created with keep_paths=0");
    if (seed < 0 || seed >= dv.dm.B || beta_idx < 0 || beta_idx >= h->last_nbeta)
        return fail(VA_EINVAL, "seed/beta index out of range");
    HIPCHK(hipSetDevice(h->device));
    const size_t wide = dv.dm.ND + dv.dm.NP;
    HIPCHK(hipMemcpyAsync(out, dv.minpaths + ((size_t)seed * dv.max_beta + beta_idx) * wide,
                          sizeof(double) * wide, hipMemcpyDeviceToHost, h->stream));
    HIPCHK(hipStreamSynchronize(h->stream));
    return VA_OK;
}

namespace {
int timed_chunk_of(int iters) { return iters < 250 ? iters : 250; }

bool timed_graph_current(va_handle h, int chunk)
{
    return h->timed_gexec && h->timed_chunk == chunk && h->tune_graph &&
           memcmp(&h->timed_dv, &h->dv, sizeof(Dev)) == 0 && memcmp(&h->timed_nn, &h->nn, sizeof(NnetDev)) == 0;
}

void timed_graph_drop(va_handle h)
{
    if (h->timed_gexec) { (void)hipGraphExecDestroy(h->timed_gexec); h->timed_gexec = nullptr; }
}

int timed_prepare(va_handle h, double rf_scale, int iters)
{
    Dev &dv = h->dv;
    if (h->timed_armed_rf != rf_scale) {
        launch_init_states(dv, PH_START, rf_scale, h->stream);
        h->timed_armed_rf = rf_scale;
    }
    if (!h->tune_graph || iters < 8) { timed_graph_drop(h); return VA_OK; }
    const int chunk = timed_chunk_of(iters);
    h->dv.lsrun = 0;
    h->dv.epi = (h->is_nnet ? !h->nn.small : !h->fold) ? EPI_NONE : EPI_FINALIZE;
    if (timed_graph_current(h, chunk)) return VA_OK;
    timed_graph_drop(h);
    hipGraph_t g = nullptr;
    if (hipStreamBeginCapture(h->stream, hipStreamCaptureModeThreadLocal) == hipSuccess) {
        for (int i = 0; i < chunk; ++i) run_eval(h, EPI_FINALIZE);
        if (hipStreamEndCapture(h->stream, &g) != hipSuccess || !g ||
            hipGraphInstantiate(&h->timed_gexec, g, nullptr, nullptr, 0) != hipSuccess) h->timed_gexec = nullptr;
        if (g) (void)hipGraphDestroy(g);
    }
    if (!h->timed_gexec) { (void)hipGetLastError(); return VA_OK; }
    h->timed_chunk = chunk;
    memcpy(&h->timed_dv, &h->dv, sizeof(Dev)); memcpy(&h->timed_nn, &h->nn, sizeof(NnetDev));
    (void)hipGraphUpload(h->timed_gexec, h->stream);
    HIPCHK(hipStreamSynchronize(h->stream));
    return VA_OK;
}
}

int va_eval_timed_prepare(va_handle h, double rf_scale, int32_t iters)
{
    if (!h || iters < 1 || !(rf_scale >= 0.0)) return fail(VA_EINVAL, "bad argument");
    HIPCHK(hipSetDevice(h->device));
    return timed_prepare(h, rf_scale, iters);
}

int va_eval_timed(va_handle h, double rf_scale, int32_t iters, float *elapsed_ms)
{
    if (!h || !elapsed_ms || iters < 1 || !(rf_scale >= 0.0)) return fail(VA_EINVAL, "bad argument");
    HIPCHK(hipSetDevice(h->device));
    Dev &dv = h->dv;
    int rc = timed_prepare(h, rf_scale, iters);
    if (rc) return rc;
    const int chunk = timed_chunk_of(iters);
    hipGraphExec_t gexec = (iters >= 8 && timed_graph_current(h, chunk)) ? h->timed_gexec : nullptr;
    HIPCHK(hipEventRecord(h->ev0, h->stream));
    int done = 0;
    if (gexec)
        for (; done + chunk <= iters; done += chunk) HIPCHK(hipGraphLaunch(gexec, h->stream));
    for (; done < iters; ++done) run_eval(h, EPI_FINALIZE);
    HIPCHK(hipEventRecord(h->ev1, h->stream));
    {
        hipError_t q;
        while ((q = hipEventQuery(h->ev1)) == hipErrorNotReady) {}
        if (q != hipSuccess) return fail(VA_EHIP, "hipEventQuery: %s", hipGetErrorString(q));
    }
    HIPCHK(hipEventElapsedTime(elapsed_ms, h->ev0, h->ev1));
    HIPCHK(hipGetLastError());
    h->n_eval_launch += iters; h->n_seed_evals += (int64_t)iters * dv.dm.B;
    h->n_seed_evals_direct += (int64_t)iters * dv.dm.B;
    return VA_OK;
}

int va_problem_tune(va_handle h, int32_t what, int32_t value)
{
    if (!h) return fail(VA_EINVAL, "null handle");
    timed_graph_drop(h);
    switch (what) {
    case VA_TUNE_FOLD:
        if (h->is_nnet) return fail(VA_EUNSUPPORTED, "the network action chooses its tail by the net's size");
        h->fold = value != 0; break;
    case VA_TUNE_GRAD_SC1: h->dv.gaux = value != 0 ? 1 : 0; break;
    case VA_TUNE_PRIO: h->dv.prio = value < 0 ? 0 : (value > 2 ? 2 : value); break;
    case VA_TUNE_GRAPH: h->tune_graph = value != 0; break;
    case VA_TUNE_NNET_FUSED:
        if (!h->is_nnet || !h->nn.Wf) return fail(VA_ESTATE, "not a network handle whose layers fit the fused kernel");
        h->nn.fused = value != 0 ? 1 : 0;
        h->nn.fb_stagger = value >= 2 ? (value - 2) * 100 : h->nn.fb_stagger; break;
    case VA_TUNE_PERSIST: h->tune_persist = value != 0; break;
    case VA_TUNE_PERSIST_ROWS: {
        if (!h->persist) return fail(VA_ESTATE, "the handle does not run the persistent kernel");
        int G = 0, T = 0;
        const Dims &dm = h->dv.dm;
        if (!persist_geometry(dm.N, dm.D, dm.L, dm.NP, dm.NPest, dm.m, dm.disc, PZ_LDS_BYTES, h->pz_maxG, value, &G, &T))
            return fail(VA_EINVAL, "%d rows per workgroup: not an admissible slice (>= 2 rows everywhere, even for SimpsonHermite, "
                                   "at most %d workgroups per seed, LDS)", value, h->pz_maxG);
        h->pz_G = G; h->pz_T = T;
        break;
    }
    default: return fail(VA_EINVAL, "unknown tuning knob %d", what);
    }
    return VA_OK;
}

namespace {

typedef struct ncclComm *ncclComm_t;
struct NcclId { char internal[VA_COMM_ID_BYTES]; };
struct Rccl {
    void *dl = nullptr;
    int (*GetUniqueId)(NcclId *) = nullptr;
    int (*CommInitRank)(ncclComm_t *, int, NcclId, int) = nullptr;
    int (*AllGather)(const void *, void *, size_t, int, ncclComm_t, hipStream_t) = nullptr;
    int (*CommDestroy)(ncclComm_t) = nullptr;
    const char *(*GetErrorString)(int) = nullptr;
};
Rccl g_rccl;
std::mutex g_rccl_mutex;

int rccl_load()
{
    std::lock_guard<std::mutex> lock(g_rccl_mutex);
    if (g_rccl.dl) return VA_OK;
    void *dl = dlopen("librccl.so.1", RTLD_NOW | RTLD_GLOBAL);
    if (!dl) dl = dlopen("librccl.so", RTLD_NOW | RTLD_GLOBAL);
    if (!dl) return fail(VA_EUNSUPPORTED, "librccl.so not found: %s", dlerror());
    Rccl r;
    r.GetUniqueId = (int (*)(NcclId *))dlsym(dl, "ncclGetUniqueId");
    r.CommInitRank = (int (*)(ncclComm_t *, int, NcclId, int))dlsym(dl, "ncclCommInitRank");
    r.AllGather = (int (*)(const void *, void *, size_t, int, ncclComm_t, hipStream_t))dlsym(dl, "ncclAllGather");
    r.CommDestroy = (int (*)(ncclComm_t))dlsym(dl, "ncclCommDestroy");
    r.GetErrorString = (const char *(*)(int))dlsym(dl, "ncclGetErrorString");
    if (!r.GetUniqueId || !r.CommInitRank || !r.AllGather || !r.CommDestroy || !r.GetErrorString)
        return fail(VA_EUNSUPPORTED, "librccl.so lacks an expected symbol");
    r.dl = dl;
    g_rccl = r;
    return VA_OK;
}

__global__ void k_pack_results(const Dev dv, int nbeta, double *out)
{
    const int i = blockIdx.x * blockDim.x + threadIdx.x;
    const int w = 4 + dv.dm.NPest;
    if (i >= dv.dm.B * nbeta) return;
    const int b = i / nbeta, k = i - b * nbeta;
    double *o = out + (size_t)i * w;
    const double *a = dv.ame + ((size_t)b * dv.max_beta + k) * 3;
    o[0] = a[0]; o[1] = a[1]; o[2] = a[2];
    for (int j = 0; j < dv.dm.NPest; ++j) o[3 + j] = dv.pest[((size_t)b * dv.max_beta + k) * dv.dm.NPest + j];
    o[3 + dv.dm.NPest] = (double)dv.status[(size_t)b * dv.max_beta + k];
}

}

struct va_comm_s {
    ncclComm_t comm = nullptr;
    int world = 1, rank = 0, device = 0;
};

int va_comm_unique_id(char id[VA_COMM_ID_BYTES])
{
    if (!id) return fail(VA_EINVAL, "id is NULL");
    int rc = rccl_load();
    if (rc) return rc;
    NcclId nid;
    const int e = g_rccl.GetUniqueId(&nid);
    if (e) return fail(VA_EHIP, "ncclGetUniqueId: %s", g_rccl.GetErrorString(e));
    memcpy(id, nid.internal, VA_COMM_ID_BYTES);
    return VA_OK;
}

int va_comm_create(const char id[VA_COMM_ID_BYTES], int32_t world, int32_t rank, int32_t device, va_comm *out)
{
    if (!id || !out || world < 1 || rank < 0 || rank >= world) return fail(VA_EINVAL, "bad argument");
    *out = nullptr;
    int rc = rccl_load();
    if (rc) return rc;
    HIPCHK(hipSetDevice(device));
    NcclId nid;
    memcpy(nid.internal, id, VA_COMM_ID_BYTES);
    va_comm c = new va_comm_s();
    c->world = world; c->rank = rank; c->device = device;
    const int e = g_rccl.CommInitRank(&c->comm, world, nid, rank);
    if (e) { delete c; return fail(VA_EHIP, "ncclCommInitRank: %s", g_rccl.GetErrorString(e)); }
    *out = c;
    return VA_OK;
}

void va_comm_destroy(va_comm c)
{
    if (!c) return;
    if (c->comm && g_rccl.CommDestroy) (void)g_rccl.CommDestroy(c->comm);
    delete c;
}

int va_gather_results(va_handle h, va_comm c, int32_t nbeta, double *table, int32_t *status)
{
    if (!h || !c || !table) return fail(VA_EINVAL, "null argument");
    const Dev &dv = h->dv;
    if (nbeta < 1 || nbeta > dv.max_beta) return fail(VA_EINVAL, "nbeta=%d outside [1, max_beta=%d]", nbeta, dv.max_beta);
    if (c->device != h->device) return fail(VA_EINVAL, "communicator lives on device %d, the problem on %d", c->device, h->device);
    HIPCHK(hipSetDevice(h->device));
    const int B = dv.dm.B, w = 4 + dv.dm.NPest;
    const size_t mine = (size_t)B * nbeta * w;
    double *send = nullptr, *recv = nullptr;
    HIPCHK(hipMalloc((void **)&send, sizeof(double) * mine));
    hipError_t e1 = hipMalloc((void **)&recv, sizeof(double) * mine * c->world);
    if (e1 != hipSuccess) { (void)hipFree(send); return fail(VA_ENOMEM, "hipMalloc: %s", hipGetErrorString(e1)); }
    hipLaunchKernelGGL(k_pack_results, dim3((B * nbeta + 255) / 256), dim3(256), 0, h->stream, dv, nbeta, send);
    const int e = g_rccl.AllGather(send, recv, mine,  8, c->comm, h->stream);
    std::vector<double> host(mine * c->world);
    hipError_t e2 = e ? hipSuccess : hipMemcpyAsync(host.data(), recv, sizeof(double) * host.size(), hipMemcpyDeviceToHost, h->stream);
    hipError_t e3 = hipStreamSynchronize(h->stream);
    (void)hipFree(send); (void)hipFree(recv);
    if (e) return fail(VA_EHIP, "ncclAllGather: %s", g_rccl.GetErrorString(e));
    if (e2 != hipSuccess || e3 != hipSuccess) return fail(VA_EHIP, "gather copy: %s", hipGetErrorString(e2 != hipSuccess ? e2 : e3));
    const size_t rows = (size_t)c->world * B * nbeta;
    for (size_t i = 0; i < rows; ++i) {
        memcpy(table + i * (w - 1), host.data() + i * w, sizeof(double) * (w - 1));
        if (status) status[i] = (int32_t)host[i * w + w - 1];
    }
    return VA_OK;
}

int va_lbfgs_timed(va_handle h, int32_t iters, float *ms_update, float *ms_direction)
{
    if (!h || !ms_update || !ms_direction || iters < 1) return fail(VA_EINVAL, "bad argument");
    HIPCHK(hipSetDevice(h->device));
    Dev &dv = h->dv;
    if (dv.dm.bounded) return fail(VA_EUNSUPPORTED, "va_lbfgs_timed times k_direction; a bounded handle runs k_lbfgsb_dir");
    dv.sticky = 1;
    h->timed_armed_rf = -1.0;
    auto dir = [&]() { launch_direction(dv, h->stream); };
    launch_arm_full_history(dv, h->stream);
    launch_update(dv, h->stream); dir();
    HIPCHK(hipEventRecord(h->ev0, h->stream));
// ... 93 lines not shown
```

varanneal_amd/csrc/va_device.h:

```cpp
#pragma once
#include <hip/hip_runtime.h>

#include <type_traits>

#include "va_core.h"
#include "va_tile2.h"
#include "va_tile3.h"
#include "va_tile4.h"
#include "va_tile5.h"

namespace va {

constexpr int VEC_THREADS = 256;
constexpr int VEC_CHUNK = 1024;

constexpr int CNT_STRIDE = 64;

enum { EPI_NONE = 0, EPI_FINALIZE = 1, EPI_LS = 2 };

struct Persist {
    unsigned long long *xch;
    unsigned long long *cycles;
    int *abort_flag;
    double *stamps;
    long long max_cycles;
};

struct Dev {
    Dims dm;
    Geo4 g4;
    Geo5 g5;
    const int *ystrip;
    int lsrun;
    int epi;
    unsigned ntiles_magic;
    int gaux;
    int prio;
    int sticky;
    int evcols;
    ProblemPtrs pp;
    Opts o;
    double *x, *g, *gt, *d;
    double *S, *Y;
    SeedState *st;
    double *evp;
    double *evp_big;
    int npbig;
    double *upp;
    double *dpp;
    int ups;
    const double *rf_ladder;
    int nbeta, max_beta;
    double *ame;
    double *pest;
    int *status, *nit;
    long long *nfev;
    double *minpaths;
    int *n_active;
    unsigned *cnt_eval, *cnt_upd, *cnt_dir;
    unsigned long long *n_evals;
    double *outA, *outme, *outfe;
    double *lb_z, *lb_r, *lb_xp, *lb_t, *lb_mat, *lb_dtd;
    int *lb_iwhere;
    Persist pz;
    const int *cpmap;
    double *evv;
    int cps, cpv, cpnsg;
};

struct EvalOp { bool prepare; hipStream_t s; hipError_t err; };

constexpr size_t LDS_DEFAULT_BYTES = 64 * 1024, LDS_OPTIN_BYTES = 160 * 1024;

inline int eval_grid(const Dims &dm) { return ((dm.B * dm.ntiles + 7) / 8) * 8; }

template <class KERNEL>
inline void eval_op(KERNEL kern, const Dev &dv, int threads, size_t lds, EvalOp &op)
{
    if (op.prepare) {
        if (lds <= LDS_DEFAULT_BYTES) return;
        const hipError_t e = hipFuncSetAttribute((const void *)kern, hipFuncAttributeMaxDynamicSharedMemorySize, (int)LDS_OPTIN_BYTES);
        if (e != hipSuccess) op.err = e;
        return;
    }
    hipLaunchKernelGGL(kern, dim3(eval_grid(dv.dm)), dim3(threads), lds, op.s, dv);
}

template <class F>
inline void with_disc(int disc, F &&f)
{
    switch (disc) {
    case DISC_EULER: f(std::integral_constant<int, DISC_EULER>()); break;
    case DISC_TRAPEZOID: f(std::integral_constant<int, DISC_TRAPEZOID>()); break;
    case DISC_SH: f(std::integral_constant<int, DISC_SH>()); break;
    default: f(std::integral_constant<int, DISC_FWDMAP>()); break;
    }
}

struct PredictArgs;
struct HvpArgs;
struct RhsTable {
    int bytes;
    int dev_bytes, seed_bytes, predict_bytes;
    int NP, D, NSTIM;
    void (*eval)(const Dev &, EvalOp &);
    void (*eval_var)(const Dev &, EvalOp &);
    void (*seed)(const Dev &, EvalOp &);
    hipError_t (*predict)(const PredictArgs &, hipStream_t);
};
void builtin_rhs_table(RhsTable &t);
struct PredictTlmArgs;
struct HvpTable {
    int bytes, hvp_bytes, tlm_bytes;
    hipError_t (*hvp)(const HvpArgs &, size_t lds_bytes, hipStream_t);
    hipError_t (*predict_tlm)(const PredictTlmArgs &, hipStream_t);
};
void builtin_hvp_table(HvpTable &t);

void launch_ls(const Dev &dv, hipStream_t s);
void launch_update(const Dev &dv, hipStream_t s);
void launch_direction(const Dev &dv, hipStream_t s);
void launch_init_states(const Dev &dv, int phase, double rf_scale_or_neg, hipStream_t s);
void launch_arm_full_history(const Dev &dv, hipStream_t s);
void launch_arm_ls(const Dev &dv, double rf, hipStream_t s);
void launch_clamp_x(const Dev &dv, hipStream_t s);
void launch_finalize_eval(const Dev &dv, hipStream_t s);
size_t eval_lds_bytes(const Dev &dv);
size_t update_lds_bytes(const Dims &dm);
void launch_lbfgsb_dir(const Dev &dv, hipStream_t s);
hipError_t prepare_lbfgsb(const Dev &dv);
void eval5_builtin(const Dev &dv, EvalOp &op);
size_t eval5_lds(const Dev &dv);

}
```

varanneal_amd/csrc/va_eval4.h:

```cpp
#pragma once
#include "va_eval_flat.h"
#include "va_measure.h"

namespace va {

typedef __attribute__((address_space(3))) void lds_void_t;
typedef const __attribute__((address_space(1))) void glb_void_t;

template <int NI>
__device__ __forceinline__ void tile4_dma(const Geo4 &g, const double *src, double *dst, int lane)
{
#pragma unroll
    for (int i = 0; i < NI; ++i) {
        const int sp = tile4_src_piece(g, i * 64 + lane);
        if (sp >= 0)
            __builtin_amdgcn_global_load_lds((glb_void_t *)(src + 2 * sp), (lds_void_t *)(dst + 128 * i), 16, 0, 0);
    }
}

template <class RHS, int DISC, int K, int DC, int WS, int SUB>
__global__ __launch_bounds__(256, SUB > 1 ? 1 : ((K <= 7 && K * RHS::NB <= 28) ? 3 : 2)) void k_eval4(const Dev dv)
{
    extern __shared__ __attribute__((aligned(16))) double smem[];
    constexpr bool W_SCALAR = WS != 0;
    const Dims &dm = dv.dm;
    const int nwork = dm.B * dm.ntiles;
    const int w = xcd_swizzle(blockIdx.x, nwork);
    if (w >= nwork) return;
    const int b = dm.ntiles > 1 ? (int)__umulhi((unsigned)w, dv.ntiles_magic) : w, tile = w - b * dm.ntiles;

    constexpr int HL = Halo<DISC>::HL, HR = Halo<DISC>::HR, NE = RHS::NE;
    constexpr int NV = EP_GP + RHS::NP;
    constexpr int NCV = rhs_ncv<RHS>::value;
    VA_E4_STAMP_SETUP(dv, w);
    VA_E4_STAMP(0);
    const Geo4 g = DC > 0 ? tile4_geo<HL + HR>(DC > 0 ? DC : 4, K, NE, SUB) : dv.g4;
    constexpr int NI = DC > 0 ? (tile4_geo<HL + HR>(DC > 0 ? DC : 4, K, NE, SUB).XP + 63) / 64 : T4_NI_MAX;
    const int D = DC > 0 ? DC : g.D;
    const int tid = threadIdx.x, lane = tid & 63;
    const int wave = __builtin_amdgcn_readfirstlane(tid >> 6);
    const int RK = g.RW * K;
    const int n0w = tile * g.T + wave * SUB * RK;
    double *xsw = smem + wave * g.WAVE, *r2w = xsw + SUB * g.XW, *strip = r2w + g.R2;
    const double *xg = dv.x + (size_t)b * dm.ld;

#pragma unroll
    for (int s = 0; s < SUB; ++s) tile4_dma<NI>(g, xg + (long)(n0w + s * RK - HL) * D, xsw + s * g.XW, lane);

    const auto *st = as_const(static_cast<const SeedHot *>(dv.st + b));
    const int phase = st->phase;
    if (phase != PH_START && phase != PH_LS) {
        asm volatile("s_waitcnt vmcnt(0)" ::: "memory");
        return;
    }
    const int use_d = (phase == PH_LS);
    const double stp = st->stp;
    const double *dg = dv.d + (size_t)b * dm.ld;
    if (use_d) {
#pragma unroll
        for (int s = 0; s < SUB; ++s) tile4_dma<NI>(g, dg + (long)(n0w + s * RK - HL) * D, r2w + s * g.XW, lane);
    }

    const int a = lane / D, tx = lane - a * D;
    const bool active = a < g.RW;
    Tile4 t;
    t.n0w = n0w; t.a = a; t.tx = tx; t.r0 = n0w + a * K; t.use_d = use_d;
    t.l = obs_index(dm.obsmask, tx);
    t.wobs = t.l >= 0 ? dm.rm : 0.0;
    t.c = 2.0 * st->rf_scale * dm.cfe;
    t.xs = xsw; t.es = r2w;
    t.gtg = dv.gt + (size_t)b * dm.ld;
    if constexpr (NCV > 0) {
        const int nt = dv.cps + dv.cpv;
#pragma unroll
        for (int k = 0; k < RHS::NP; ++k) {
            const int ke = as_const(dv.cpmap)[nt + k];
            double v = as_const(dv.pp.Pfull)[(size_t)b * dm.NP + as_const(dv.cpmap)[k]];
            if (ke >= 0) {
                v = as_const(xg)[dm.ND + ke];
                if (use_d) v = trial(v, stp, as_const(dg)[dm.ND + ke]);
            }
            t.p[k] = v;
        }
#pragma unroll
        for (int u = 0; u < NCV; ++u) {
            const int e = dv.cps + u * D + tx;
            const int ke = dv.cpmap[nt + e];
            double v = dv.pp.Pfull[(size_t)b * dm.NP + dv.cpmap[e]];
            if (ke >= 0) {
                v = xg[dm.ND + ke];
                if (use_d) v = trial(v, stp, dg[dm.ND + ke]);
            }
            t.pv[u] = v;
        }
    } else {
#pragma unroll
        for (int k = 0; k < RHS::NP; ++k) t.p[k] = as_const(dv.pp.Pfull)[(size_t)b * dm.NP + k];
        for (int k = 0; k < dm.NPest; ++k) {
            double v = as_const(xg)[dm.ND + k];
            if (use_d) v = trial(v, stp, as_const(dg)[dm.ND + k]);
            const int dst = as_const(dv.pp.Pidx)[k];
#pragma unroll
            for (int j = 0; j < RHS::NP; ++j) t.p[j] = (dst == j) ? v : t.p[j];
        }
    }
    T4Regs<K, NE> rg[SUB];
    ColAcc<RHS> acc;
    acc.clear();
    if constexpr (WS == 2) {
        const __amdgpu_buffer_rsrc_t yr = __builtin_amdgcn_make_buffer_rsrc(
            (void *)dv.pp.Y, 0, (int)(sizeof(double) * dm.N_data * dm.L), 0x00020000);
        const bool obs = active && t.l >= 0;
#pragma unroll
        for (int s = 0; s < SUB; ++s) {
            const int m0 = t.r0 + s * RK;
            int nd = m0 / dm.nskip, rem = m0 - nd * dm.nskip;
            unsigned has = 0u;
#pragma unroll
            for (int k = 0; k < K; ++k) {
                typedef unsigned v2u __attribute__((ext_vector_type(2)));
                const bool h = obs && rem == 0 && nd < dm.N_data && m0 + k < dm.N;
                const v2u v = __builtin_amdgcn_raw_buffer_load_b64(yr, h ? (nd * dm.L + t.l) * 8 : 0x7ffffff0, 0, 0);
                rg[s].yv[k] = __hiloint2double((int)v.y, (int)v.x);
                has |= h ? (1u << k) : 0u;
                if (++rem == dm.nskip) { rem = 0; ++nd; }
            }
            rg[s].has = has;
        }
    } else if constexpr (W_SCALAR) {
        const __amdgpu_buffer_rsrc_t yr = __builtin_amdgcn_make_buffer_rsrc(
            (void *)dv.pp.Y, 0, (int)(sizeof(double) * dm.N_data * dm.L), 0x00020000);
        const int voff = (active && t.l >= 0) ? (t.r0 * dm.L + t.l) * 8 : 0x7ffffff0;
#pragma unroll
        for (int s = 0; s < SUB; ++s) {
#pragma unroll
            for (int k = 0; k < K; ++k) {
                typedef unsigned v2u __attribute__((ext_vector_type(2)));
                const v2u v = __builtin_amdgcn_raw_buffer_load_b64(yr, voff, (s * RK + k) * dm.L * 8, 0);
                rg[s].yv[k] = __hiloint2double((int)v.y, (int)v.x);
            }
        }
    } else if (active) {
#pragma unroll
        for (int s = 0; s < SUB; ++s) {
            Tile4 ts = t;
            ts.r0 = t.r0 + s * RK;
            tile4_obs<K, NE>(dm, dv.pp, ts, rg[s]);
        }
    }
    static_assert(SUB == 1 || WS != 0, "sub-tiles are compiled for the scalar-weight variants only");
    constexpr bool RFW = WS == 0 && tile4_rfw_in_lds<K, NE, HL, DC>();
    double wq[SUB][K + HL];
    if constexpr (RFW) {
        if (dv.pp.rf0_arr && active) {
#pragma unroll
            for (int s = 0; s < SUB; ++s) {
                Tile4 ts = t;
                ts.r0 = t.r0 + s * RK;
                tile4_rfw_load<K, HL>(dm, dv.pp, ts, D, wq[s]);
            }
        }
    }

    VA_E4_STAMP(1);
    asm volatile("s_waitcnt vmcnt(0)" ::: "memory");
    __builtin_amdgcn_wave_barrier();
    VA_E4_STAMP(2);
    if (dv.prio == 1) {
        const int grp = (int)(blockIdx.x >> 8);
        if (grp == 1) __builtin_amdgcn_s_setprio(1);
        else if (grp >= 2) __builtin_amdgcn_s_setprio(2);
    } else if (dv.prio == 2) {
        if (tile == 0 || tile == dm.ntiles - 1) __builtin_amdgcn_s_setprio(3);
    }
    if (use_d) {
#pragma unroll
        for (int s = 0; s < SUB; ++s) {
#pragma unroll
            for (int i = 0; i < NI; ++i) {
                const int q = i * 64 + lane;
                if (q < g.XP) {
                    double x0, x1, d0, d1;
                    ld2(xsw + s * g.XW + 2 * q, x0, x1); ld2(r2w + s * g.XW + 2 * q, d0, d1);
                    st2(xsw + s * g.XW + 2 * q, trial(x0, stp, d0), trial(x1, stp, d1));
                }
            }
#pragma unroll
            for (int k = 0; k < K; ++k) {
                const int j = k + HL;
                rg[s].dval[k] = active ? r2w[s * g.XW + a * g.PITCH + tx + (j < K ? j * D : g.PITCH + (j - K) * D)] : 0.0;
            }
        }
        wave_sync_lds();
    } else {
#pragma unroll
        for (int s = 0; s < SUB; ++s)
#pragma unroll
            for (int k = 0; k < K; ++k) rg[s].dval[k] = 0.0;
    }
    const bool lsq = dv.epi != EPI_FINALIZE;
    if constexpr (RFW) {
        if (dv.pp.rf0_arr && active) tile4_rfw_store<K, HL>(g, t, D, wq[0]);
    }
    unsigned old = 0;
    double gvv[SUB][K];
    auto publish = [&]() {
#pragma unroll
        for (int k = 0; k < NV; ++k) {
            if ((k == EP_GTD || k == EP_GN2 || k == EP_GMAX) && !lsq) continue;
            if (k == EP_GTD && !use_d) continue;
            const double r = (k == EP_GMAX) ? wave_max(acc.v[k]) : wave_sum_mfma(acc.v[k]);
            if (lane == 0) strip[k] = r;
        }
        if constexpr (NCV > 0) {
#pragma unroll
            for (int u = 0; u < NCV; ++u) {
                double sv = 0.0;
                for (int a2 = 0; a2 < g.RW; ++a2) sv += __shfl(acc.v[EP_N + u], a2 * D + tx, 64);
                if (lane < D) xsw[u * D + lane] = sv;
            }
        }
        asm volatile("s_waitcnt lgkmcnt(0)" ::: "memory");
        VA_E4_STAMP(5);
        __builtin_amdgcn_s_barrier();
        VA_E4_STAMP(6);
        if (wave == 0) {
            if (lane < NV) {
                const double r0 = strip[lane], r1 = strip[g.WAVE + lane], r2 = strip[2 * g.WAVE + lane], r3 = strip[3 * g.WAVE + lane];
                double v = (lane == EP_GMAX) ? fmax(fmax(r0, r1), fmax(r2, r3)) : ((r0 + r1) + r2) + r3;
                if ((lane == EP_GTD && !use_d) || ((lane == EP_GTD || lane == EP_GN2 || lane == EP_GMAX) && !lsq)) v = 0.0;
                st_sc1(dv.evp + ((size_t)b * dm.ntiles + tile) * EP_N + lane, v);
            }
            if constexpr (NCV > 0) {
                double *vrow = dv.evv + ((size_t)b * dm.ntiles + tile) * dv.cpv;
                for (int e = lane; e < NCV * D; e += 64) {
                    const double r0 = smem[e], r1 = smem[g.WAVE + e], r2 = smem[2 * g.WAVE + e], r3 = smem[3 * g.WAVE + e];
                    st_sc1(vrow + e, ((r0 + r1) + r2) + r3);
                }
            }
        }
    };
    auto count = [&]() {
        if (wave == 0 && dv.epi != EPI_NONE) {
            asm volatile("s_waitcnt vmcnt(0)" ::: "memory");
            if (lane == 0) old = __hip_atomic_fetch_add(dv.cnt_eval + (size_t)b * CNT_STRIDE, 1u, __ATOMIC_RELAXED, __HIP_MEMORY_SCOPE_AGENT);
        }
    };
#pragma unroll
    for (int s = 0; s < SUB; ++s) {
        const int n0s = n0w + s * RK;
        const bool edge = (n0s - HL < 0) || (n0s + RK + HR > dm.N);
        t.r0 = n0s + a * K; t.xs = xsw + s * g.XW;
        if (active) {
            if (edge) tile4_rows<RHS, DISC, K, true, DC, WS>(dm, dv.pp, g, t, rg[s], acc);
            else tile4_rows<RHS, DISC, K, false, DC, WS>(dm, dv.pp, g, t, rg[s], acc);
        }
        wave_sync_lds();
        if (s == SUB - 1) VA_E4_STAMP(3);
        if (!lsq && s == SUB - 1) publish();
#pragma unroll
        for (int k = 0; k < K; ++k) gvv[s][k] = 0.0;
        if (active) {
            if (edge) {
                if (lsq) tile4_grad<RHS, DISC, K, true, DC, WS, true>(dm, g, t, rg[s], acc, gvv[s]);
                else tile4_grad<RHS, DISC, K, true, DC, WS, false>(dm, g, t, rg[s], acc, gvv[s]);
            } else {
                if (lsq) tile4_grad<RHS, DISC, K, false, DC, WS, true>(dm, g, t, rg[s], acc, gvv[s]);
                else tile4_grad<RHS, DISC, K, false, DC, WS, false>(dm, g, t, rg[s], acc, gvv[s]);
            }
        }
        if (!lsq && s == SUB - 1) count();
        if (s + 1 < SUB) wave_sync_lds();
    }
    VA_E4_STAMP(4);
    if (lsq) { publish(); count(); }
    {
        const __amdgpu_buffer_rsrc_t gr = __builtin_amdgcn_make_buffer_rsrc(
            (void *)(dv.gt + (size_t)b * dm.ld), 0, (int)(sizeof(double) * dm.N * D), 0x00020000);
        const int npieces = RK * D / 2;
#pragma unroll
        for (int s = 0; s < SUB; ++s) {
            wave_sync_lds();
            if (active) {
#pragma unroll
                for (int k = 0; k < K; ++k) r2w[(a * K + k) * D + tx] = gvv[s][k];
            }
            wave_sync_lds();
            const int base = (n0w + s * RK) * D * 8;
#pragma unroll
            for (int i = 0; i < (K * 32 + 63) / 64; ++i) {
                if (i * 64 >= npieces) break;
                typedef unsigned v4u __attribute__((ext_vector_type(4)));
                const int q = i * 64 + lane;
                double g0, g1;
                ld2(r2w + 2 * (q < npieces ? q : 0), g0, g1);
                const v4u v = {(unsigned)__double2loint(g0), (unsigned)__double2hiint(g0), (unsigned)__double2loint(g1), (unsigned)__double2hiint(g1)};
                const int voff = q < npieces ? q * 16 : 0x7ffffff0;
                if (dv.gaux) __builtin_amdgcn_raw_buffer_store_b128(v, gr, voff, base, 16);
                else __builtin_amdgcn_raw_buffer_store_b128(v, gr, voff, base, 0);
            }
        }
    }
    VA_E4_STAMP_ACK();
    bool last = false;
    if (wave == 0 && dv.epi != EPI_NONE) {
        old = __builtin_amdgcn_readfirstlane(old);
        asm volatile("" ::: "memory");
        last = old == (unsigned)dm.ntiles - 1u;
        if (last) {
            if (lane == 0) __hip_atomic_store(dv.cnt_eval + (size_t)b * CNT_STRIDE, 0u, __ATOMIC_RELAXED, __HIP_MEMORY_SCOPE_AGENT);
            eval_epilogue<true, (NCV > 0)>(dv, b, lane, reinterpret_cast<SeedHot *>(xsw), dv.epi);
        }
    }
    VA_E4_STAMP_TAIL(last);
}


inline size_t eval4_lds_bytes(const Dev &dv) { return sizeof(double) * (size_t)dv.g4.NW * dv.g4.WAVE; }

template <class RHS, int DISC, int K, int DC, int WS>
inline void eval4_op(const Dev &dv, EvalOp &op)
{
    eval_op(k_eval4<RHS, DISC, K, DC, WS, 1>, dv, 256, eval4_lds_bytes(dv), op);
}

}
```

varanneal_amd/csrc/va_eval_geo.h:

```cpp
#pragma once
#include <stddef.h>

#include <algorithm>
#include <vector>

#include "../../include/varanneal_amd.h"
#include "va_core.h"
#include "va_tile3.h"
#include "va_tile4.h"
#include "va_tile5.h"

namespace va {

struct EvalForm {
    int ne = 0;
    int ghost = 0;
    bool has_reach5 = false;
    int reach5[4] = {0, 0, 0, 0};
    int lin = 0;
};

struct EvalPlan {
    int emode = 0, RY = 0, NT = 0, maxr = 0, T = 0, ntiles = 0;
    int ghost = 2;
    Geo4 g4{};
    Geo5 g5{};
    std::vector<int> ystrip;
};

inline const char *flat_only_reason(const va_problem_desc *d)
{
    if (d->lower && d->upper) return "box bounds (carried by the flat kernel only)";
    if (d->p_time_dependent) return "time-dependent parameters";
    if (d->rm_kind == 2 || d->rf_kind == 2) return "full RM / RF matrices (flat kernel only)";
    return nullptr;
}

inline int shorter_run(int K, bool sh) { return K - ((sh || K == 5) ? (K == 5 ? 1 : 2) : 1); }

template <class F>
inline int fewest_rounds_run(const va_problem_desc *d, int rows1, int kmin, bool sh, F resident)
{
    int K = 6;
    long best = -1;
    for (int k = kmin; k <= 8; ++k) {
        if (sh && (k & 1)) continue;
        const long wgs = (long)d->batch * ((d->N_model + rows1 * k - 1) / (rows1 * k)), per_round = resident(k);
        const long cost = ((wgs + per_round - 1) / per_round) * (k + 2) * 4 + (k == 6 ? 0 : 1);
        if (best < 0 || cost < best) { best = cost; K = k; }
    }
    return K;
}

inline bool plan_eval5(const va_problem_desc *d, const EvalForm &f, EvalPlan &p)
{
    const int D = d->D, N = d->N_model, ne = f.ne;
    const bool sh = d->disc == VA_DISC_SIMPSON_HERMITE;
    const int *reach5 = f.reach5;
    const bool ws5 = d->rm_kind <= 1 && d->rf_kind <= 1 && d->merr_nskip >= 1 && d->L >= 1;
    if (!(f.has_reach5 && ne > 0 && ws5 && D > 64 && (!sh || (N & 1)) && tile5_ok(D, reach5[0], reach5[1], reach5[2], reach5[3])))
        return false;
    Geo5 g = tile5_cols(D, reach5[0], reach5[1], reach5[2], reach5[3]);
    g.ne = ne;
    const long per_row = (long)d->batch * g.NSG;
    long nseg = (4L * 256) / per_row;
    if (d->tile_rows > 0) nseg = (N + d->tile_rows - 1) / d->tile_rows;
    if (nseg > N / 32) nseg = N / 32;
    if (nseg < 1) nseg = 1;
    g.SEGL = (int)((N + nseg - 1) / nseg);
    g.SEGL = (g.SEGL + 1) & ~1;
    g.NSEG = (N + g.SEGL - 1) / g.SEGL;
    std::vector<int> ls(d->Lidx, d->Lidx + d->L), ystrip(2 * g.NS, 0);
    std::sort(ls.begin(), ls.end());
    g.YPMAX = 1;
    for (int s5 = 0; s5 < g.NS; ++s5) {
        const int c0 = tile5_c0(D, g.NS, s5), c1 = tile5_c0(D, g.NS, s5 + 1);
        const int l0 = (int)(std::lower_bound(ls.begin(), ls.end(), c0) - ls.begin());
        const int l1 = (int)(std::lower_bound(ls.begin(), ls.end(), c1) - ls.begin());
        int start = l0 & ~1;
        int yp = (l1 - start + 1) / 2;
        if (yp < 1) yp = 1;
        ystrip[2 * s5] = start; ystrip[2 * s5 + 1] = yp;
        if (yp > g.YPMAX) g.YPMAX = yp;
    }
    if (g.YPMAX > 32) return false;
    g.xdpp = (reach5[2] <= 2 && reach5[3] <= 2) ? 1 : 0;
    auto fits = [&](int nslot, bool lsr) { return (size_t)g.WPG * tile5_wave_doubles(g, nslot, lsr) * sizeof(double) <= 40 * 1024; };
    g.nslot = fits(4, false) ? 4 : 3;
    g.nslot_ls = fits(4, true) ? 4 : 3;
    g.warr = (d->rm_kind == 1 || d->rf_kind == 1 || d->merr_nskip > 1) ? 1 : 0;
    if (g.warr) g.nslot = g.nslot_ls = 3;
    g.LY = (d->L + 1) & ~1;
    p.g5 = g;
    p.ystrip = ystrip;
    p.emode = 5; p.RY = 0; p.NT = 64 * g.WPG; p.maxr = 2; p.T = g.SEGL;
    p.ntiles = g.NSEG * g.NSG;
    return true;
}

inline bool plan_eval4(const va_problem_desc *d, const EvalForm &f, EvalPlan &p)
{
    const int D = d->D, N = d->N_model, ne = f.ne;
    const bool sh = d->disc == VA_DISC_SIMPSON_HERMITE;
    if (!tile4_ok(D) || ne <= 0) return false;
    const int RW = 64 / D, rows1 = 4 * RW;
    int K = 6;
    auto ntl = [&](int k) { return (long)d->batch * ((N + rows1 * k - 1) / (rows1 * k)); };
    if (ntl(K) < 256) K = 4;
    else if (ntl(K) >= 8 * 256) {
        long best = -1;
        for (int k = 5; k <= 7; ++k) {
            if (sh && (k & 1)) continue;
            const long cost = (long)((N + rows1 * k - 1) / (rows1 * k)) * (k + (sh ? 3 : 2));
            if (best < 0 || cost <= best) { best = cost; K = k; }
        }
    } else {
        K = fewest_rounds_run(d, rows1, sh ? 4 : 5, sh, [&](int k) { return sh ? 256L * (k <= 7 ? 3 : 2) : 256L; });
        if (sh && D == 20 && d->rhs == VA_RHS_LORENZ96 && d->rm_kind == 0 && d->rf_kind == 0 && ntl(12) <= 2 * 256 && ntl(K) > 3 * 256) K = 12;
    }
    if (d->tile_rows > 0) {
        K = (d->tile_rows + rows1 - 1) / rows1;
        const bool k12 = D == 20 && d->rm_kind == 0 && d->rf_kind == 0 && (d->merr_nskip == 1 || d->rhs == VA_RHS_LORENZ96);
        K = K < 4 ? 4 : (K >= 12 && k12 ? 12 : (K > 8 ? 8 : K));
        if (sh && (K & 1)) ++K;
    }
    {
        const bool ws4 = (d->rm_kind == 0 && d->rf_kind == 0 && d->merr_nskip == 1) || (D == 20 && d->rhs == VA_RHS_LORENZ96);
        if (!ws4 && (K == 6 || K == 7)) K = sh ? 4 : 5;
    }
    if (d->tile_rows <= 0) {
        while (K > 4) {
            const Geo4 gt = sh ? tile4_geo<3>(D, K, ne, 1) : tile4_geo<2>(D, K, ne, 1);
            if (sizeof(double) * (size_t)gt.NW * gt.WAVE <= 80 * 1024) break;
            K = shorter_run(K, sh);
        }
    }
    const int SUB = 1;
    const Geo4 g4 = sh ? tile4_geo<3>(D, K, ne, SUB) : tile4_geo<2>(D, K, ne, SUB);
    if (!((D == 20 || (g4.XP + 63) / 64 <= T4_NI_MAX) && tile4_magic_ok(g4))) return false;
    p.g4 = g4;
    p.emode = 4; p.RY = 4 * RW; p.NT = 256; p.maxr = K; p.T = g4.T;
    p.ntiles = (N + p.T - 1) / p.T;
    return true;
}

inline bool plan_eval3(const va_problem_desc *d, const EvalForm &f, EvalPlan &p)
{
    const int D = d->D, N = d->N_model;
    const bool sh = d->disc == VA_DISC_SIMPSON_HERMITE;
    const int HLR = sh ? 3 : 2;
    if (f.ghost <= 0 || D > 1024) return false;
    const int RY = tile3_RY(D), NT = tile3_threads(D);
    int K = 6;
    if ((long)d->batch * ((N + RY * K - 1) / (RY * K)) < 256) K = 4;
    else if ((long)d->batch * ((N + RY * K - 1) / (RY * K)) < 8 * 256 && NT == 256) {
        K = fewest_rounds_run(d, RY, 5, sh, [](int) { return 256L; });
    }
    if (d->tile_rows > 0) {
        K = (d->tile_rows + RY - 1) / RY;
        K = K < 4 ? 4 : (K > 8 ? 8 : K);
        if (sh && (K & 1)) ++K;
    }
    if (D > 64 && d->tile_rows <= 0 && (long)d->batch * ((N + RY * 8 - 1) / (RY * 8)) >= 256)
        K = 8;
    if (NT == 1024 && K > 6) K = 6;
    for (;;) {
        const size_t elems = (size_t)tile3_stage_elems(K, D, f.ghost, RY, HLR) + tile3_s_elems(K, D, f.ghost, RY);
        if (sizeof(double) * elems <= (D <= 64 ? 60 : (D <= 512 ? 78 : 150)) * 1024 || K <= 4) break;
        K = shorter_run(K, sh);
    }
    p.emode = 3; p.RY = RY; p.NT = NT; p.maxr = K; p.T = RY * K;
    p.ntiles = (N + p.T - 1) / p.T;
    return true;
}

inline void plan_flat(const va_problem_desc *d, const EvalForm &f, EvalPlan &p)
{
    const int D = d->D, N = d->N_model;
    const bool sh = d->disc == VA_DISC_SIMPSON_HERMITE;
    const int HLR = sh ? 3 : 2;
    const size_t narr = 3 + (f.lin ? 1 : 0);
    auto rows_in = [&](size_t kib) { return (int)((kib * 1024) / (narr * sizeof(double) * D)) - HLR; };
    int tmax = rows_in(24);
    if (f.lin) {
        for (size_t kib : {24, 48, 80}) { tmax = rows_in(kib); if (tmax + HLR >= 16) break; }
    }
    if (tmax < 2) tmax = rows_in(48);
    if (tmax < 2) tmax = rows_in(150);
    if (f.lin && d->tile_rows > tmax && d->tile_rows <= rows_in(150)) tmax = d->tile_rows;
    int tmin = (EVAL_THREADS + D - 1) / D;
    if (tmax < 2) tmax = 2;
    if (tmin > tmax) tmin = tmax;
    int T;
    if (d->tile_rows > 0) T = d->tile_rows < tmax ? d->tile_rows : tmax;
    else {
        int want = (1024 + d->batch - 1) / d->batch;
        T = N / (want > 0 ? want : 1);
        if (T < tmin) T = tmin;
        if (T > tmax) T = tmax;
    }
    if (T > N) T = N;
    if (sh && (T & 1)) T += (T + 1 <= tmax) ? 1 : -1;
    if (T < 2) T = 2;
    p.emode = 1; p.RY = 0; p.NT = EVAL_THREADS; p.maxr = 0; p.T = T;
    p.ntiles = (N + T - 1) / T;
}

inline EvalPlan plan_eval(const va_problem_desc *d, const EvalForm &f)
{
    EvalPlan p;
    p.ghost = f.ghost > 0 ? f.ghost : 2;
    if ((f.ne <= 0 && f.ghost <= 0) || flat_only_reason(d)) { plan_flat(d, f, p); return p; }
    int want = d->eval_kernel;
    if (want == 2) want = 3;
    if (want == 5) { if (plan_eval5(d, f, p)) return p; want = 0; }
    if (want < 1 || want > 5) {
        if (tile4_ok(d->D) && f.ne > 0) want = 4;
        else if (plan_eval5(d, f, p)) return p;
        else want = 3;
    }
    if (want == 4 && plan_eval4(d, f, p)) return p;
    if (want >= 3 && plan_eval3(d, f, p)) return p;
    plan_flat(d, f, p);
    return p;
}

struct VariantKey {
    int kernel = 0, disc = 0, K = 0, W = 0;
    bool operator==(const VariantKey &o) const { return kernel == o.kernel && disc == o.disc && K == o.K && W == o.W; }
};
inline VariantKey variant_key(const EvalPlan &p, const va_problem_desc *d)
{
    VariantKey k;
    if (p.emode != 3 && p.emode != 4 && p.emode != 5) return k;
    k.kernel = p.emode; k.disc = d->disc;
    if (p.emode == 5) return k;
    k.K = p.maxr;
    k.W = p.emode == 4 ? ((d->rm_kind == 0 && d->rf_kind == 0 && d->merr_nskip == 1) ? 1 : 0) : p.NT;
    return k;
}

struct ModuleVariant {
    int kernel = 0, disc = 0, K = 0, W = 0;
    int ne = 0, ghost = 0, reach[4] = {0, 0, 0, 0};
    int has_linear = 0;
    int n_colp_vectors = 0;

    static ModuleVariant decode(const int *v)
    {
        ModuleVariant m;
        m.kernel = v[UV_KERNEL]; m.disc = v[UV_DISC]; m.K = v[UV_K]; m.W = v[UV_W];
        m.ne = v[UV_NE]; m.ghost = v[UV_GHOST];
        for (int k = 0; k < 4; ++k) m.reach[k] = v[UV_REACH + k];
        m.has_linear = v[UV_LINEAR] ? 1 : 0; m.n_colp_vectors = v[UV_NCV];
        return m;
    }
    bool column_params() const { return n_colp_vectors > 0 && (kernel == 4 || kernel == 5); }
    EvalForm flat_form() const { EvalForm f; f.lin = has_linear; return f; }
    EvalForm form() const
    {
        EvalForm f = flat_form();
        f.ne = (kernel == 4 || kernel == 5) ? ne : 0;
        f.ghost = kernel == 3 ? ghost : 0;
        f.has_reach5 = kernel == 5;
        for (int k = 0; k < 4; ++k) f.reach5[k] = reach[k];
        return f;
    }
    VariantKey key() const
    {
        VariantKey k;
        k.kernel = kernel; k.disc = disc;
        if (kernel == 5) return k;
        k.K = K; k.W = kernel == 4 ? (W != 0 ? 1 : 0) : W;
        return k;
    }
};

}
```

varanneal_amd/csrc/va_kernels.hip:

```cpp
#include "va_device.h"
#include "va_eval_flat.h"
#include "va_eval3.h"
#include "va_eval4.h"
#include "va_tile5.h"
#include "va_persist.h"
#include "va_predict.h"
#include "va_predict_tlm.h"
#include "va_hvp.h"

namespace va {

size_t eval_lds_bytes(const Dev &dv)
{
    switch (dv.dm.emode) {
    case 5: return eval5_lds(dv);
    case 4: return eval4_lds_bytes(dv);
    case 3: return eval3_lds_bytes(dv.dm);
    default: return eval_flat_lds_bytes(dv.dm);
    }
}

template <class RHS, int K, int DC, int NTMAX>
static void eval3_rhs(const Dev &dv, EvalOp &op)
{
    with_disc(dv.dm.disc, [&](auto disc) { eval3_op<RHS, decltype(disc)::value, K, DC, NTMAX>(dv, op); });
}

template <class RHS, int K>
static void eval3_d(const Dev &dv, EvalOp &op)
{
    if (dv.dm.D == 200) eval3_rhs<RHS, K, 200, 256>(dv, op);
    else if (dv.dm.D <= 64) eval3_rhs<RHS, K, 0, 256>(dv, op);
    else if (dv.dm.D <= 128) eval3_rhs<RHS, K, 0, 512>(dv, op);
    else if (dv.dm.D <= 256) eval3_rhs<RHS, K, 0, 256>(dv, op);
    else if (dv.dm.D <= 512) eval3_rhs<RHS, K, 0, 512>(dv, op);
    else eval3_rhs<RHS, K, 0, 1024>(dv, op);
}

template <class RHS, int K, int DC, int WS>
static void eval4_rhs(const Dev &dv, EvalOp &op)
{
    with_disc(dv.dm.disc, [&](auto disc) { eval4_op<RHS, decltype(disc)::value, K, DC, WS>(dv, op); });
}

template <class RHS, int K>
static void eval4_d(const Dev &dv, EvalOp &op)
{
    const bool sw = !dv.pp.rm_arr && !dv.pp.rf0_arr, ws = sw && dv.dm.nskip == 1;
    if (dv.dm.D == 20) {
        if (ws) eval4_rhs<RHS, K, 20, 1>(dv, op);
        else if (sw) eval4_rhs<RHS, K, 20, 2>(dv, op);
        else eval4_rhs<RHS, K, 20, 0>(dv, op);
    } else { if (ws) eval4_rhs<RHS, K, 0, 1>(dv, op); else eval4_rhs<RHS, K, 0, 0>(dv, op); }
}

static void eval_builtin(const Dev &dv, EvalOp &op)
{
    if (dv.dm.emode == 5) eval5_builtin(dv, op);
    else if (dv.dm.emode == 4) {
        switch (dv.dm.maxr) {
        case 4: eval4_d<RhsL96s, 4>(dv, op); break;
        case 5: eval4_d<RhsL96s, 5>(dv, op); break;
        case 6: eval4_d<RhsL96s, 6>(dv, op); break;
        case 7: eval4_d<RhsL96s, 7>(dv, op); break;
        case 12: if (dv.dm.nskip == 1) eval4_rhs<RhsL96s, 12, 20, 1>(dv, op); else eval4_rhs<RhsL96s, 12, 20, 2>(dv, op); break;
        default: eval4_d<RhsL96s, 8>(dv, op); break;
        }
    } else if (dv.dm.emode == 3) {
        switch (dv.dm.maxr) {
        case 4: eval3_d<RhsL96g, 4>(dv, op); break;
        case 5: eval3_d<RhsL96g, 5>(dv, op); break;
        case 6: eval3_d<RhsL96g, 6>(dv, op); break;
        case 7: eval3_d<RhsL96g, 7>(dv, op); break;
        default: eval3_d<RhsL96g, 8>(dv, op); break;
        }
    } else eval_flat_op<RhsL96>(dv, op);
}

void builtin_rhs_table(RhsTable &t)
{
    t = RhsTable{(int)sizeof(RhsTable), (int)sizeof(Dev), (int)sizeof(SeedState), (int)sizeof(PredictArgs), RhsL96::NP, 0, 0,
                 eval_builtin, nullptr, seed_op<RhsL96>, launch_predict<RhsL96, 0>};
}
void builtin_hvp_table(HvpTable &t)
{
    t = HvpTable{(int)sizeof(HvpTable), (int)sizeof(HvpArgs), (int)sizeof(PredictTlmArgs), launch_hvp<RhsL96>, launch_predict_tlm<RhsL96, 0>};
}

constexpr int TAIL_MAX_WAVES = 16;
static int tail_waves(const Dims &dm) { const int w = (dm.nprow + 127) / 128; return w < 1 ? 1 : (w > TAIL_MAX_WAVES ? TAIL_MAX_WAVES : w); }

template <bool CP>
__global__ __launch_bounds__(64 * TAIL_MAX_WAVES) void k_ls(const Dev dv)
{
    __shared__ SeedHot sh;
    __shared__ double part[TAIL_MAX_WAVES * 32];
    const int b = blockIdx.x, lane = threadIdx.x & 63;
    const int wave = __builtin_amdgcn_readfirstlane(threadIdx.x >> 6), nw = blockDim.x >> 6;
    const int phase = dv.st[b].phase;
    if (phase != PH_START && phase != PH_LS) return;
    double ev[EP_N];
    reduce_eval_block(dv, b, lane, wave, nw, part, ev);
    if (wave == 0) eval_epilogue<false, CP>(dv, b, lane, &sh, EPI_LS, ev);
}
void launch_ls(const Dev &dv, hipStream_t s)
{
    if (dv.cpv) hipLaunchKernelGGL(k_ls<true>, dim3(dv.dm.B), dim3(64 * tail_waves(dv.dm)), 0, s, dv);
    else hipLaunchKernelGGL(k_ls<false>, dim3(dv.dm.B), dim3(64 * tail_waves(dv.dm)), 0, s, dv);
}

template <bool CP>
__global__ __launch_bounds__(64 * TAIL_MAX_WAVES) void k_finalize_eval(const Dev dv)
{
    __shared__ double part[TAIL_MAX_WAVES * 32];
    const int b = blockIdx.x, lane = threadIdx.x & 63;
    const int wave = __builtin_amdgcn_readfirstlane(threadIdx.x >> 6), nw = blockDim.x >> 6;
    double ev[EP_N];
    reduce_eval_block(dv, b, lane, wave, nw, part, ev);
    if (wave == 0) eval_epilogue<false, CP>(dv, b, lane, nullptr, EPI_FINALIZE, ev);
}
void launch_finalize_eval(const Dev &dv, hipStream_t s)
{
    if (dv.cpv) hipLaunchKernelGGL(k_finalize_eval<true>, dim3(dv.dm.B), dim3(64 * tail_waves(dv.dm)), 0, s, dv);
    else hipLaunchKernelGGL(k_finalize_eval<false>, dim3(dv.dm.B), dim3(64 * tail_waves(dv.dm)), 0, s, dv);
}

__global__ void k_init_states(const Dev dv, int phase, double rf)
{
    const int b = blockIdx.x * blockDim.x + threadIdx.x;
    if (b >= dv.dm.B) return;
    SeedState &s = dv.st[b];
    s.phase = phase; s.beta_idx = 0; s.iter = 0; s.col = 0; s.head = 0; s.ifun = 0; s.iback = 0;
    s.ls_task = LS_START; s.upd = 0; s.slot = 0; s.dir = 0; s.store_idx = -1; s.nold = 0;
    s.nfev = 0; s.f = 0.0; s.fold = 0.0; s.me = 0.0; s.fe = 0.0; s.theta = 1.0; s.stp = 0.0;
    s.stp_upd = 0.0; s.gd = 0.0; s.gdold = 0.0; s.gn2 = 0.0; s.dr = 0.0; s.cg = -1.0; s.gd_dir = 0.0; s.stpmx = 1e10;
    s.rf_scale = rf < 0.0 ? dv.rf_ladder[0] : rf;
    dv.cnt_eval[(size_t)b * CNT_STRIDE] = 0u; dv.cnt_upd[(size_t)b * CNT_STRIDE] = 0u; dv.cnt_dir[(size_t)b * CNT_STRIDE] = 0u;
}
void launch_init_states(const Dev &dv, int phase, double rf, hipStream_t s)
{
    hipLaunchKernelGGL(k_init_states, dim3((dv.dm.B + 63) / 64), dim3(64), 0, s, dv, phase, rf);
}

__global__ void k_clamp_x(const Dev dv)
{
    const long i = (long)blockIdx.x * blockDim.x + threadIdx.x;
    if (i >= dv.dm.ld) return;
    double *x = dv.x + (size_t)blockIdx.y * dv.dm.ld;
    x[i] = fmin(fmax(x[i], dv.pp.lo[i]), dv.pp.hi[i]);
}
void launch_clamp_x(const Dev &dv, hipStream_t s)
{
    hipLaunchKernelGGL(k_clamp_x, dim3((dv.dm.ld + 255) / 256, dv.dm.B), dim3(256), 0, s, dv);
}

__global__ void k_arm_full_history(const Dev dv)
{
    const int b = blockIdx.x * blockDim.x + threadIdx.x;
    if (b >= dv.dm.B) return;
    SeedState &s = dv.st[b];
    const int m = dv.o.m;
    s.phase = PH_IDLE; s.col = m; s.head = 1 % m; s.nold = m - 1; s.slot = 0;
    for (int j = 0; j < m; ++j) s.order[j] = (j + 1) % m;
    s.upd = UPD_G | UPD_HIST; s.dir = 1; s.stp_upd = 1.0; s.dr = 1.0; s.theta = 1.0; s.store_idx = -1;
}
__global__ void k_arm_ls(const Dev dv, double rf)
{
    const int b = blockIdx.x * blockDim.x + threadIdx.x;
    if (b >= dv.dm.B) return;
    SeedState &s = dv.st[b];
    s.phase = PH_LS; s.ifun = 1; s.iback = 0; s.stp = 1e-3; s.ls_task = LS_FG; s.rf_scale = rf;
    s.iter = 1; s.nfev = 2; s.f = 1.0; s.fold = 1.0; s.gd = -1.0; s.gdold = -1.0; s.stpmx = 1e10;
    LsState &l = s.ls;
    l.brackt = 0; l.stage = 1; l.ginit = -1.0; l.gtest = -1e-3; l.gx = -1.0; l.gy = -1.0;
    l.finit = -1e300; l.fx = -1e300; l.fy = -1e300; l.stx = 0.0; l.sty = 0.0; l.stmin = 0.0; l.stmax = 5e-3;
    l.width = 1e10; l.width1 = 2e10;
}
void launch_arm_ls(const Dev &dv, double rf, hipStream_t s)
{
    hipLaunchKernelGGL(k_arm_ls, dim3((dv.dm.B + 63) / 64), dim3(64), 0, s, dv, rf);
}
void launch_arm_full_history(const Dev &dv, hipStream_t s)
{
    hipLaunchKernelGGL(k_arm_full_history, dim3((dv.dm.B + 63) / 64), dim3(64), 0, s, dv);
}

__device__ __forceinline__ double bcast_lane(double x, int i)
{
    const int lo = __builtin_amdgcn_readlane(__double2loint(x), i);
    const int hi = __builtin_amdgcn_readlane(__double2hiint(x), i);
    return __hiloint2double(hi, lo);
}

__host__ __device__ inline int coeffs_lds_doubles(int m) { return UP_N + 2 * m * m + 3 * MAX_M; }

__device__ __forceinline__ void coeffs_wave(const Dev &dv, int b, int lane, double *lds)
{
    const Dims &dm = dv.dm;
    const int M = MAX_M, m = dm.m;
    double *up = lds, *sSY = up + UP_N, *sYY = sSY + m * m, *sp = sYY + m * m, *cYs = sp + M, *cSs = cYs + M;
    SeedState &s = dv.st[b];
    const int nold = s.nold, col = s.col, sn = s.slot;
    const bool hist = (s.upd & UPD_HIST) != 0;
    const double dr = s.dr;
    double theta = s.theta;
    const int K = UP_OLD + 4 * nold;
    for (int k = lane; k < K; k += 64)
        up[k] = col_reduce<true>(dv.upp + (size_t)b * dm.nchunks * dv.ups + k, dm.nchunks, dv.ups, 0, 1, false);
    const int myslot = lane < col ? s.order[lane] : 0;
    for (int e0 = 0; e0 < m * m; e0 += 256) {
        double t0[4], t1[4];
#pragma unroll
        for (int u = 0; u < 4; ++u) {
            const int e = e0 + lane + 64 * u;
            const int i = e / m, j = e - i * m;
            t0[u] = e < m * m ? s.SY[i * M + j] : 0.0;
            t1[u] = e < m * m ? s.YY[i * M + j] : 0.0;
        }
#pragma unroll
// ... 272 lines not shown
```

varanneal_amd/csrc/va_measure.h:

```cpp
#pragma once

#ifdef VA_STAMPS
#define VA_E4_STAMP_SETUP(dv, w)                                                                                                   \
    unsigned long long *tl = reinterpret_cast<unsigned long long *>((dv).upp) + ((size_t)blockIdx.x * 4 + (threadIdx.x >> 6)) * 10; \
    if ((threadIdx.x & 63) == 0) {                                                                                                 \
        tl[8] = (unsigned long long)__builtin_amdgcn_s_getreg((31 << 11) | 4);                                                     \
        tl[9] = ((unsigned long long)__builtin_amdgcn_s_getreg((31 << 11) | 20) << 32) | (unsigned long long)(w);                  \
    }
#define VA_E4_STAMP(i) do { if ((threadIdx.x & 63) == 0) tl[i] = wall_clock64(); } while (0)
#define VA_E4_STAMP_TAIL(last) do { if (last) { asm volatile("s_waitcnt vmcnt(0)" ::: "memory"); tl[1] = wall_clock64(); } } while (0)
#define VA_E4_STAMP_ACK() do { asm volatile("s_waitcnt vmcnt(0)" ::: "memory"); if ((threadIdx.x & 63) == 0) tl[7] = wall_clock64(); } while (0)
#else
#define VA_E4_STAMP_ACK() do { } while (0)
#define VA_E4_STAMP_SETUP(dv, w)
#define VA_E4_STAMP(i) do { } while (0)
#define VA_E4_STAMP_TAIL(last) do { } while (0)
#endif

#ifdef VA_PZ_STAMPS
#define PZ_MARK_SETUP() long long pz_acc[PZ_NSTAMP - 1] = {0, 0, 0, 0, 0, 0, 0, 0, 0, 0, 0, 0, 0}, pz_prev = wall_clock64(); \
    const long long pz_c0 = clock64(), pz_w0 = pz_prev
#define PZ_MARK(i) do { if (tid == 0) { const long long t_ = wall_clock64(); pz_acc[i] += t_ - pz_prev; pz_prev = t_; } } while (0)
#define PZ_MARK_FLUSH(stamps, cyc) do { if (blockIdx.x == 0 && tid == 0) {                                   \
        pz_acc[9] = clock64() - pz_c0; pz_acc[10] = wall_clock64() - pz_w0;                                  \
        for (int i_ = 0; i_ < PZ_NSTAMP - 1; ++i_) (stamps)[i_] = (double)pz_acc[i_];                        \
        (stamps)[PZ_NSTAMP - 1] = (double)(cyc); } } while (0)
#else
#define PZ_MARK_SETUP() do { } while (0)
#define PZ_MARK(i) do { } while (0)
#define PZ_MARK_FLUSH(stamps, cyc) do { } while (0)
#endif

#ifdef VA_FB_STAMPS
#define FB_MARK_SETUP() long long fb_acc[8] = {0, 0, 0, 0, 0, 0, 0, 0}, fb_prev = wall_clock64(); const long long fb_w0 = fb_prev
#define FB_MARK(i) do { if (tid == 0) { const long long t_ = wall_clock64(); fb_acc[i] += t_ - fb_prev; fb_prev = t_; } } while (0)
#define FB_MARK_FLUSH(stamps) do { if (blockIdx.x == 1 && blockIdx.y == 0 && tid == 0 && (stamps)) {           \
        fb_acc[7] = wall_clock64() - fb_w0;                                                                    \
        for (int i_ = 0; i_ < 8; ++i_) (stamps)[i_] = (double)fb_acc[i_]; } } while (0)
#else
#define FB_MARK_SETUP() do { } while (0)
#define FB_MARK(i) do { } while (0)
#define FB_MARK_FLUSH(stamps) do { } while (0)
#endif
```

varanneal_amd/csrc/va_user_rhs.hip:

```cpp
#include "va_eval_flat.h"
#include "va_eval3.h"
#include "va_eval4.h"
#include "va_eval5.h"
#include "va_persist.h"
#include "va_predict.h"
#include "va_predict_tlm.h"
#include "va_hvp.h"

#ifndef VA_USER_RHS_HEADER
#error "compile with -DVA_USER_RHS_HEADER='\"path/to/generated_header.h\"'"
#endif
#include VA_USER_RHS_HEADER

namespace {
#if defined(VA_USER_COLP)
#define VA_USER_COLT va::RhsUserColP
#elif defined(VA_USER_COL)
#define VA_USER_COLT va::RhsUserCol
#endif
#if defined(VA_USER_EK) && VA_USER_EK == 5 && defined(VA_USER_COLT)
#define VA_USER_VARIANT 5
#elif defined(VA_USER_EK) && VA_USER_EK == 4 && defined(VA_USER_COLT)
#define VA_USER_VARIANT 4
#elif defined(VA_USER_EK) && VA_USER_EK == 3 && defined(VA_USER_GHOST)
#define VA_USER_VARIANT 3
#endif
#if !defined(VA_USER_VARIANT)
constexpr void (*user_eval_var)(const va::Dev &, va::EvalOp &) = nullptr;
#elif VA_USER_VARIANT == 5
constexpr auto user_eval_var = va::eval5_op<VA_USER_COLT, VA_USER_DISC, VA_USER_COLT::D>;
#elif VA_USER_VARIANT == 4
constexpr auto user_eval_var = va::eval4_op<VA_USER_COLT, VA_USER_DISC, VA_USER_K, VA_USER_COLT::D, VA_USER_W != 0>;
#else
constexpr auto user_eval_var = va::eval3_op<va::RhsUserG, VA_USER_DISC, VA_USER_K, va::RhsUserG::D, VA_USER_W>;
#endif

template <class R> void fill_table(va::RhsTable &t)
{
    t = va::RhsTable{(int)sizeof(va::RhsTable), (int)sizeof(va::Dev), (int)sizeof(va::SeedState), (int)sizeof(va::PredictArgs),
                     R::NP, R::D, R::NSTIM, nullptr, user_eval_var, nullptr, nullptr};
    if constexpr (va::rhs_flat<R>::value) { t.eval = va::eval_flat_op<R>; t.predict = va::launch_predict<R, R::D>; }
    if constexpr (va::seed_kernel_exists<R>()) t.seed = va::seed_op<R>;
}
template <class R> void fill_hvp_table(va::HvpTable &t)
{
    t = va::HvpTable{(int)sizeof(va::HvpTable), (int)sizeof(va::HvpArgs), (int)sizeof(va::PredictTlmArgs), nullptr, nullptr};
    if constexpr (va::rhs_flat<R>::value && !va::rhs_linear<R>::value) { t.hvp = va::launch_hvp<R>; t.predict_tlm = va::launch_predict_tlm<R, R::D>; }
}
}

extern "C" {

int va_user_rhs_table(va::RhsTable *out, int bytes)
{
    if (bytes == (int)sizeof(va::RhsTable)) fill_table<va::RhsUser>(*out);
    return (int)sizeof(va::RhsTable);
}

int va_user_hvp_table(va::HvpTable *out, int bytes)
{
    if (bytes == (int)sizeof(va::HvpTable)) fill_hvp_table<va::RhsUser>(*out);
    return (int)sizeof(va::HvpTable);
}

void va_user_variant_info(int *out)
{
    for (int k = 0; k < va::UV_N; ++k) out[k] = 0;
    out[va::UV_LINEAR] = va::rhs_linear<va::RhsUser>::value ? 1 : 0;
#ifdef VA_USER_VARIANT
    out[va::UV_KERNEL] = VA_USER_VARIANT; out[va::UV_DISC] = VA_USER_DISC; out[va::UV_K] = VA_USER_K; out[va::UV_W] = VA_USER_W;
#if VA_USER_VARIANT == 5
    out[va::UV_NE] = VA_USER_COLT::NE;
    out[va::UV_REACH] = va::t5_xl<VA_USER_COLT>(); out[va::UV_REACH + 1] = va::t5_xr<VA_USER_COLT>();
    out[va::UV_REACH + 2] = va::t5_gl<VA_USER_COLT>(); out[va::UV_REACH + 3] = va::t5_gr<VA_USER_COLT>();
    out[va::UV_NCV] = va::rhs_ncv<VA_USER_COLT>::value;
#elif VA_USER_VARIANT == 4
    out[va::UV_NE] = VA_USER_COLT::NE;
    out[va::UV_NCV] = va::rhs_ncv<VA_USER_COLT>::value;
#else
    out[va::UV_GHOST] = va::RhsUserG::GHOST;
#endif
#endif
}
#if defined(VA_USER_COLP)
void va_user_colp_map(int *out)
{
    out[0] = va::RhsUserColP::NP; out[1] = va::RhsUserColP::NCV;
    for (int k = 0; k < va::RhsUserColP::NP; ++k) out[2 + k] = va::va_colp_sidx[k];
    for (int e = 0; e < va::RhsUserColP::NCV * va::RhsUserColP::D; ++e) out[2 + va::RhsUserColP::NP + e] = va::va_colp_vidx[e];
}
#endif

}
```

Before: 7.492 million evals/s.

## Add optional wide k_eval4 workgroups packing multiple row groups, drop setprio

Adds a templated G parameter to k_eval4 so one workgroup of 256*G threads handles G consecutive tiles, with a planner that picks G when the grid is small relative to CU count. The wide mode is off by default (EVAL4_WIDE_DEFAULT=false) and reachable only through a new tune knob. The s_setprio wave-priority logic previously enabled by default (prio=1) is removed. That removal changes the default path and may alter scheduling of the ramp of workgroups.

Result: faster. 7.583 million evals/s, median of 6 (+1.2%).

```diff
diff --git a/include/varanneal_amd.h b/include/varanneal_amd.h
--- a/include/varanneal_amd.h
+++ b/include/varanneal_amd.h
@@ -89,7 +89,9 @@
 #define VA_TUNE_PERSIST 5
 #define VA_TUNE_PERSIST_ROWS 6
 #define VA_TUNE_NNET_FUSED 7
+#define VA_TUNE_WIDE 8
 int va_problem_tune(va_handle h, int32_t what, int32_t value);
+int va_problem_eval_grid(va_handle h, int32_t *row_groups_per_workgroup, int32_t *workgroups);
 int va_problem_persistent(va_handle h, int32_t *workgroups_per_seed, int32_t *rows_per_workgroup);
 
 int va_problem_eval_kernel(va_handle h, int32_t *eval_kernel, int32_t *run_rows);
diff --git a/varanneal_amd/_build.py b/varanneal_amd/_build.py
--- a/varanneal_amd/_build.py
+++ b/varanneal_amd/_build.py
@@ -5,8 +5,8 @@
 HERE = os.path.dirname(os.path.abspath(__file__))
 CSRC = os.path.join(HERE, "csrc")
 OUT = os.path.join(HERE, "libvaranneal_amd.so")
-SOURCES = ["va_capi.hip", "va_kernels.hip", "va_eval5.hip", "va_lbfgsb.hip", "va_nnet.hip", "va_hmc.hip"]
-HEADERS = ["va_core.h", "va_tile2.h", "va_tile3.h", "va_tile4.h", "va_tile5.h", "va_eval3.h", "va_eval4.h", "va_eval5.h", "va_eval_flat.h", "va_epilogue.h", "va_persist.h", "va_persist_geo.h", "va_predict.h", "va_predict_geo.h", "va_predict_tlm.h", "va_predict_tlm_geo.h", "va_hvp.h", "va_hvp_geo.h", "va_selinv.h", "va_selinv_geo.h", "va_hmc.h", "va_hmc_geo.h", "va_eval_geo.h", "va_measure.h", "va_device.h", "va_nnet.h", "va_nnet_geo.h", "va_nnet_kernels.h", os.path.join("..", "..", "include", "varanneal_amd.h")]
+SOURCES = ["va_capi.hip", "va_kernels.hip", "va_eval4_g2.hip", "va_eval4_g3.hip", "va_eval5.hip", "va_lbfgsb.hip", "va_nnet.hip", "va_hmc.hip"]
+HEADERS = ["va_core.h", "va_tile2.h", "va_tile3.h", "va_tile4.h", "va_tile5.h", "va_eval3.h", "va_eval4.h", "va_eval4_builtin.h", "va_eval5.h", "va_eval_flat.h", "va_epilogue.h", "va_persist.h", "va_persist_geo.h", "va_predict.h", "va_predict_geo.h", "va_predict_tlm.h", "va_predict_tlm_geo.h", "va_hvp.h", "va_hvp_geo.h", "va_selinv.h", "va_selinv_geo.h", "va_hmc.h", "va_hmc_geo.h", "va_eval_geo.h", "va_measure.h", "va_device.h", "va_nnet.h", "va_nnet_geo.h", "va_nnet_kernels.h", os.path.join("..", "..", "include", "varanneal_amd.h")]
 HIPCC = os.environ.get("HIPCC", "/opt/rocm/bin/hipcc")
 SCHED = ["-mllvm", "-amdgpu-sched-strategy=iterative-maxocc"]
 FLAGS = ["--offload-arch=gfx950", "-O3", "-std=c++17", "-fPIC", "-shared", "-Wall", "-Wno-unused-function", "-ldl"] + SCHED
diff --git a/varanneal_amd/_capi.py b/varanneal_amd/_capi.py
--- a/varanneal_amd/_capi.py
+++ b/varanneal_amd/_capi.py
@@ -219,6 +219,8 @@
     L.va_read_eval_outputs.argtypes = [h, C.c_void_p, C.c_void_p, C.c_void_p, C.c_void_p, C.c_int64]
     L.va_debug_read_partials.argtypes = [h, c_dp, C.c_int64]
     L.va_problem_eval_kernel.argtypes = [h, c_ip, c_ip]
+    L.va_problem_eval_grid.argtypes = [h, c_ip, c_ip]
+    L.va_problem_eval_grid.restype = C.c_int
     L.va_problem_tune.argtypes = [h, C.c_int32, C.c_int32]
     L.va_debug_read_persist.argtypes = [h, c_dp, C.c_int64]
     L.va_debug_read_persist.restype = C.c_int
@@ -234,7 +236,7 @@
     return L
 
 
-EXPORTS = ["va_abi_version", "va_last_error", "va_device_count", "va_rhs_load_module", "va_act_load_module", "va_eval_plan", "va_eval_plan_reach", "va_problem_eval_kernel", "va_problem_tune", "va_problem_create",
+EXPORTS = ["va_abi_version", "va_last_error", "va_device_count", "va_rhs_load_module", "va_act_load_module", "va_eval_plan", "va_eval_plan_reach", "va_problem_eval_kernel", "va_problem_eval_grid", "va_problem_tune", "va_problem_create",
            "va_problem_destroy", "va_problem_info", "va_action_grad", "va_minimize_lbfgs",
            "va_anneal", "va_get_minpath", "va_predict", "va_predict_tangent", "va_hess_vec", "va_blocktri_selinv", "va_laplace", "va_hmc", "va_hmc_noise", "va_eval_timed", "va_eval_timed_prepare", "va_problem_persistent", "va_debug_read_persist", "va_get_counters", "va_nnet_problem_create", "va_debug_read_partials",
            "va_read_eval_outputs", "va_lbfgs_timed", "va_eval_ls_timed", "va_comm_unique_id", "va_comm_create", "va_comm_destroy",
@@ -363,10 +365,12 @@
         check(self._L.va_problem_info(self._h, C.byref(nv), C.byref(ld), C.byref(T), C.byref(nt)))
         ek, rr = C.c_int32(), C.c_int32()
         check(self._L.va_problem_eval_kernel(self._h, C.byref(ek), C.byref(rr)))
+        rg, wgs = C.c_int32(), C.c_int32()
+        check(self._L.va_problem_eval_grid(self._h, C.byref(rg), C.byref(wgs)))
         return dict(n_var=nv.value, ld=ld.value, tile_rows=T.value, ntiles=nt.value, eval_kernel=ek.value,
-                    run_rows=rr.value)
-
-    TUNE = {"fold": 1, "grad_sc1": 2, "prio": 3, "graph": 4, "persist": 5, "persist_rows": 6, "nnet_fused": 7}
+                    run_rows=rr.value, row_groups=rg.value, eval_grid=wgs.value)
+
+    TUNE = {"fold": 1, "grad_sc1": 2, "prio": 3, "graph": 4, "persist": 5, "persist_rows": 6, "nnet_fused": 7, "wide": 8}
 
     def debug_read_persist(self, n):
         out = np.empty(n)
diff --git a/varanneal_amd/csrc/va_capi.hip b/varanneal_amd/csrc/va_capi.hip
--- a/varanneal_amd/csrc/va_capi.hip
+++ b/varanneal_amd/csrc/va_capi.hip
@@ -86,6 +86,7 @@
     bool is_nnet = false;
     bool fold = false;
     bool tune_graph = true;
+    int wg4_plan = 1;
     hipGraphExec_t timed_gexec = nullptr;
     int timed_chunk = 0;
     Dev timed_dv;
@@ -147,7 +148,7 @@
     Dev &dv = h->dv;
     const Dims &dm = dv.dm;
     const size_t B = dm.B, ld = dm.ld, m = dm.m, max_beta = dv.max_beta;
-    const size_t guard = (((size_t)(dm.T + 8) * dm.D + 15) / 16) * 16;
+    const size_t guard = (((size_t)((dm.emode == 4 ? 3 : 1) * dm.T + 8) * dm.D + 15) / 16) * 16;
     TRY(h->alloc(&dv.x, B * ld + 2 * guard)); TRY(h->alloc(&dv.g, B * ld));
     TRY(h->alloc(&dv.gt, B * ld)); TRY(h->alloc(&dv.d, B * ld + 2 * guard));
     dv.x += guard; dv.d += guard;
@@ -509,7 +510,7 @@
         builtin_rhs_table(h->rt);
         builtin_hvp_table(h->rt_hvp);
         EvalForm l96;
-        l96.ne = RhsL96s::NE; l96.ghost = RhsL96g::GHOST; l96.has_reach5 = true;
+        l96.ne = RhsL96s::NE; l96.nb = RhsL96s::NB; l96.ghost = RhsL96g::GHOST; l96.has_reach5 = true;
         l96.reach5[0] = t5_xl<RhsL96s>(); l96.reach5[1] = t5_xr<RhsL96s>(); l96.reach5[2] = t5_gl<RhsL96s>(); l96.reach5[3] = t5_gr<RhsL96s>();
         plan = plan_eval(d, l96);
         return VA_OK;
@@ -524,6 +525,13 @@
     dv.cps = mp.cps; dv.cpv = mp.cpv;
     dv.cpnsg = (mp.cpv && plan.emode == 5) ? plan.g5.NSG : 0;
     return VA_OK;
+}
+
+void set_eval4_groups(Dev &dv, int G)
+{
+    dv.wg4 = G;
+    const int nwg = eval4_nwg(dv);
+    dv.nwg_magic = (unsigned)(((1ull << 32) + nwg - 1) / nwg);
 }
 
 int fill_dims(va_handle h, const va_problem_desc *d, const EvalPlan &plan)
@@ -543,7 +551,8 @@
     dv.g4 = plan.g4; dv.g5 = plan.g5;
     if (dm.emode == 4 && (unsigned long long)dm.B * dm.ntiles * dm.ntiles >= (1ull << 32))
         return fail(VA_EUNSUPPORTED, "batch x tiles too large for the wave-private kernel: pass eval_kernel=3");
-    dv.ntiles_magic = (unsigned)(((1ull << 32) + dm.ntiles - 1) / dm.ntiles);
+    h->wg4_plan = dm.emode == 4 ? plan.wg4 : 1;
+    set_eval4_groups(dv, EVAL4_WIDE_DEFAULT ? h->wg4_plan : 1);
     h->fold = (long)dm.B * dm.ntiles <= 8L * 256;
     dm.nprow = dm.ntiles;
     dm.dt = d->dt_model;
@@ -553,7 +562,6 @@
     const int npcols = dv.cpv ? dv.cps : d->NP;
     dv.evcols = EP_GP + npcols <= 8 ? 8 : (EP_GP + npcols <= 16 ? 16 : 32);
     dv.gaux = h->fold ? 1 : 0;
-    dv.prio = 1;
     return VA_OK;
 }
 
@@ -859,6 +867,8 @@
         vinfo(uv);
         u.variant = ModuleVariant::decode(uv);
         if (!t.eval_var) u.variant.kernel = 0;
+        typedef int (*nb_fn)(void);
+        if (nb_fn nb = (nb_fn)dlsym(u.dl, "va_user_col_neighbours")) u.variant.nb = nb();
     }
     if (info_fn cmap = (info_fn)dlsym(u.dl, "va_user_colp_map")) {
         u.colp.assign(2 + RHS_MAX_NP + (size_t)CP_VMAX * (t.D > 0 ? t.D : 1), 0);
@@ -970,6 +980,15 @@
     if (ld_internal) *ld_internal = h->dv.dm.ld;
     if (tile_rows) *tile_rows = h->dv.dm.T;
     if (ntiles) *ntiles = h->dv.dm.ntiles;
+    return VA_OK;
+}
+
+int va_problem_eval_grid(va_handle h, int32_t *row_groups_per_workgroup, int32_t *workgroups)
+{
+    if (!h) return fail(VA_EINVAL, "null handle");
+    const bool e4 = !h->is_nnet && h->dv.dm.emode == 4;
+    if (row_groups_per_workgroup) *row_groups_per_workgroup = e4 ? eval4_groups(h->dv) : 1;
+    if (workgroups) *workgroups = h->is_nnet ? 0 : h->dv.dm.B * (e4 ? eval4_nwg(h->dv) : h->dv.dm.ntiles);
     return VA_OK;
 }
 
@@ -1582,7 +1601,26 @@
         if (h->is_nnet) return fail(VA_EUNSUPPORTED, "the network action chooses its tail by the net's size");
         h->fold = value != 0; break;
     case VA_TUNE_GRAD_SC1: h->dv.gaux = value != 0 ? 1 : 0; break;
-    case VA_TUNE_PRIO: h->dv.prio = value < 0 ? 0 : (value > 2 ? 2 : value); break;
+    case VA_TUNE_PRIO: break;
+    case VA_TUNE_WIDE: {
+        if (h->is_nnet || h->dv.dm.emode != 4) {
+            if (value > 1) return fail(VA_EUNSUPPORTED, "only the wave-private kernel k_eval4 has wide workgroups");
+            break;
+        }
+        if (value < 0 || value > 3) return fail(VA_EINVAL, "wide = %d: 0, 1 (the planner's choice), 2 or 3 row groups per workgroup", value);
+        HIPCHK(hipSetDevice(h->device));
+        const int was = h->dv.wg4;
+        set_eval4_groups(h->dv, value == 0 ? 1 : (value == 1 ? h->wg4_plan : value));
+        EvalOp op{true, nullptr, hipSuccess};
+        if (eval_lds_bytes(h->dv) > LDS_OPTIN_BYTES) op.err = hipErrorInvalidValue;
+        else h->rt.eval(h->dv, op);
+        if (op.err != hipSuccess) {
+            set_eval4_groups(h->dv, was);
+            (void)hipGetLastError();
+            return fail(VA_EUNSUPPORTED, "k_eval4 at runs of %d rows has no workgroup of %d row groups (registers or LDS)", h->dv.dm.maxr, value);
+        }
+        break;
+    }
     case VA_TUNE_GRAPH: h->tune_graph = value != 0; break;
     case VA_TUNE_NNET_FUSED:
         if (!h->is_nnet || !h->nn.Wf) return fail(VA_ESTATE, "not a network handle whose layers fit the fused kernel");
diff --git a/varanneal_amd/csrc/va_device.h b/varanneal_amd/csrc/va_device.h
--- a/varanneal_amd/csrc/va_device.h
+++ b/varanneal_amd/csrc/va_device.h
@@ -33,9 +33,9 @@
     const int *ystrip;
     int lsrun;
     int epi;
-    unsigned ntiles_magic;
+    unsigned nwg_magic;
     int gaux;
-    int prio;
+    int wg4;
     int sticky;
     int evcols;
     ProblemPtrs pp;
@@ -72,10 +72,14 @@
 
 constexpr size_t LDS_DEFAULT_BYTES = 64 * 1024, LDS_OPTIN_BYTES = 160 * 1024;
 
-inline int eval_grid(const Dims &dm) { return ((dm.B * dm.ntiles + 7) / 8) * 8; }
+inline int eval_grid(int nwork) { return ((nwork + 7) / 8) * 8; }
+inline int eval_grid(const Dims &dm) { return eval_grid(dm.B * dm.ntiles); }
+
+VA_HD int eval4_groups(const Dev &dv) { return dv.wg4 > 1 ? dv.wg4 : 1; }
+VA_HD int eval4_nwg(const Dev &dv) { return (dv.dm.ntiles + eval4_groups(dv) - 1) / eval4_groups(dv); }
 
 template <class KERNEL>
-inline void eval_op(KERNEL kern, const Dev &dv, int threads, size_t lds, EvalOp &op)
+inline void eval_op(KERNEL kern, const Dev &dv, int threads, size_t lds, EvalOp &op, int grid = -1)
 {
     if (op.prepare) {
         if (lds <= LDS_DEFAULT_BYTES) return;
@@ -83,7 +87,7 @@
         if (e != hipSuccess) op.err = e;
         return;
     }
-    hipLaunchKernelGGL(kern, dim3(eval_grid(dv.dm)), dim3(threads), lds, op.s, dv);
+    hipLaunchKernelGGL(kern, dim3(grid < 0 ? eval_grid(dv.dm) : grid), dim3(threads), lds, op.s, dv);
 }
 
 template <class F>
@@ -129,6 +133,8 @@
 size_t update_lds_bytes(const Dims &dm);
 void launch_lbfgsb_dir(const Dev &dv, hipStream_t s);
 hipError_t prepare_lbfgsb(const Dev &dv);
+void eval4_builtin_g2(const Dev &dv, EvalOp &op);
+void eval4_builtin_g3(const Dev &dv, EvalOp &op);
 void eval5_builtin(const Dev &dv, EvalOp &op);
 size_t eval5_lds(const Dev &dv);
 
diff --git a/varanneal_amd/csrc/va_eval4.h b/varanneal_amd/csrc/va_eval4.h
--- a/varanneal_amd/csrc/va_eval4.h
+++ b/varanneal_amd/csrc/va_eval4.h
@@ -18,16 +18,21 @@
     }
 }
 
-template <class RHS, int DISC, int K, int DC, int WS, int SUB>
-__global__ __launch_bounds__(256, SUB > 1 ? 1 : ((K <= 7 && K * RHS::NB <= 28) ? 3 : 2)) void k_eval4(const Dev dv)
+constexpr int eval4_wpc(int K, int NB) { return (K <= 7 && K * NB <= 28) ? 3 : 2; }
+
+template <class RHS, int DISC, int K, int DC, int WS, int SUB, int G>
+__global__ __launch_bounds__(256 * G, SUB > 1 ? 1 : eval4_wpc(K, RHS::NB)) void k_eval4(const Dev dv)
 {
     extern __shared__ __attribute__((aligned(16))) double smem[];
+    static_assert(G >= 1 && G <= eval4_wpc(K, RHS::NB), "a workgroup of G row groups lives on the registers of G 4-wave workgroups of one CU");
     constexpr bool W_SCALAR = WS != 0;
     const Dims &dm = dv.dm;
-    const int nwork = dm.B * dm.ntiles;
+    const int nwg = G == 1 ? dm.ntiles : (dm.ntiles + G - 1) / G;
+    const int nwork = dm.B * nwg;
     const int w = xcd_swizzle(blockIdx.x, nwork);
     if (w >= nwork) return;
-    const int b = dm.ntiles > 1 ? (int)__umulhi((unsigned)w, dv.ntiles_magic) : w, tile = w - b * dm.ntiles;
+    const int b = nwg > 1 ? (int)__umulhi((unsigned)w, dv.nwg_magic) : w, wg = w - b * nwg;
+    const int tile = wg * G;
 
     constexpr int HL = Halo<DISC>::HL, HR = Halo<DISC>::HR, NE = RHS::NE;
     constexpr int NV = EP_GP + RHS::NP;
@@ -166,13 +171,6 @@
     asm volatile("s_waitcnt vmcnt(0)" ::: "memory");
     __builtin_amdgcn_wave_barrier();
     VA_E4_STAMP(2);
-    if (dv.prio == 1) {
-        const int grp = (int)(blockIdx.x >> 8);
-        if (grp == 1) __builtin_amdgcn_s_setprio(1);
-        else if (grp >= 2) __builtin_amdgcn_s_setprio(2);
-    } else if (dv.prio == 2) {
-        if (tile == 0 || tile == dm.ntiles - 1) __builtin_amdgcn_s_setprio(3);
-    }
     if (use_d) {
 #pragma unroll
         for (int s = 0; s < SUB; ++s) {
@@ -225,17 +223,27 @@
         __builtin_amdgcn_s_barrier();
         VA_E4_STAMP(6);
         if (wave == 0) {
-            if (lane < NV) {
-                const double r0 = strip[lane], r1 = strip[g.WAVE + lane], r2 = strip[2 * g.WAVE + lane], r3 = strip[3 * g.WAVE + lane];
-                double v = (lane == EP_GMAX) ? fmax(fmax(r0, r1), fmax(r2, r3)) : ((r0 + r1) + r2) + r3;
-                if ((lane == EP_GTD && !use_d) || ((lane == EP_GTD || lane == EP_GN2 || lane == EP_GMAX) && !lsq)) v = 0.0;
-                st_sc1(dv.evp + ((size_t)b * dm.ntiles + tile) * EP_N + lane, v);
+#pragma unroll
+            for (int e0 = 0; e0 < G * NV; e0 += 64) {
+                const int e = e0 + lane, q = G == 1 ? 0 : e / NV, k = e - q * NV;
+                if (e < G * NV && (G == 1 || tile + q < dm.ntiles)) {
+                    const double *sq = strip + 4 * q * g.WAVE + k;
+                    const double r0 = sq[0], r1 = sq[g.WAVE], r2 = sq[2 * g.WAVE], r3 = sq[3 * g.WAVE];
+                    double v = (k == EP_GMAX) ? fmax(fmax(r0, r1), fmax(r2, r3)) : ((r0 + r1) + r2) + r3;
+                    if ((k == EP_GTD && !use_d) || ((k == EP_GTD || k == EP_GN2 || k == EP_GMAX) && !lsq)) v = 0.0;
+                    st_sc1(dv.evp + ((size_t)b * dm.ntiles + tile + q) * EP_N + k, v);
+                }
             }
             if constexpr (NCV > 0) {
-                double *vrow = dv.evv + ((size_t)b * dm.ntiles + tile) * dv.cpv;
-                for (int e = lane; e < NCV * D; e += 64) {
-                    const double r0 = smem[e], r1 = smem[g.WAVE + e], r2 = smem[2 * g.WAVE + e], r3 = smem[3 * g.WAVE + e];
-                    st_sc1(vrow + e, ((r0 + r1) + r2) + r3);
+#pragma unroll
+                for (int q = 0; q < G; ++q) {
+                    if (G > 1 && tile + q >= dm.ntiles) break;
+                    double *vrow = dv.evv + ((size_t)b * dm.ntiles + tile + q) * dv.cpv;
+                    const double *sq = smem + 4 * q * g.WAVE;
+                    for (int e = lane; e < NCV * D; e += 64) {
+                        const double r0 = sq[e], r1 = sq[g.WAVE + e], r2 = sq[2 * g.WAVE + e], r3 = sq[3 * g.WAVE + e];
+                        st_sc1(vrow + e, ((r0 + r1) + r2) + r3);
+                    }
                 }
             }
         }
@@ -280,6 +288,7 @@
         const int npieces = RK * D / 2;
 #pragma unroll
         for (int s = 0; s < SUB; ++s) {
+            if (G > 1 && n0w + s * RK >= dm.N) break;
             wave_sync_lds();
             if (active) {
 #pragma unroll
@@ -306,7 +315,7 @@
     if (wave == 0 && dv.epi != EPI_NONE) {
         old = __builtin_amdgcn_readfirstlane(old);
         asm volatile("" ::: "memory");
-        last = old == (unsigned)dm.ntiles - 1u;
+        last = old == (unsigned)nwg - 1u;
         if (last) {
             if (lane == 0) __hip_atomic_store(dv.cnt_eval + (size_t)b * CNT_STRIDE, 0u, __ATOMIC_RELAXED, __HIP_MEMORY_SCOPE_AGENT);
             eval_epilogue<true, (NCV > 0)>(dv, b, lane, reinterpret_cast<SeedHot *>(xsw), dv.epi);
@@ -316,12 +325,24 @@
 }
 
 
-inline size_t eval4_lds_bytes(const Dev &dv) { return sizeof(double) * (size_t)dv.g4.NW * dv.g4.WAVE; }
-
-template <class RHS, int DISC, int K, int DC, int WS>
+inline size_t eval4_lds_bytes(const Dev &dv) { return sizeof(double) * (size_t)eval4_groups(dv) * dv.g4.NW * dv.g4.WAVE; }
+
+template <class RHS, int DISC, int K, int DC, int WS, int G>
 inline void eval4_op(const Dev &dv, EvalOp &op)
 {
-    eval_op(k_eval4<RHS, DISC, K, DC, WS, 1>, dv, 256, eval4_lds_bytes(dv), op);
-}
-
-}
+    if constexpr (G <= eval4_wpc(K, RHS::NB)) {
+        eval_op(k_eval4<RHS, DISC, K, DC, WS, 1, G>, dv, 256 * G, eval4_lds_bytes(dv), op, eval_grid(dv.dm.B * eval4_nwg(dv)));
+    } else op.err = hipErrorInvalidConfiguration;
+}
+template <class RHS, int DISC, int K, int DC, int WS>
+inline void eval4_op_groups(const Dev &dv, EvalOp &op)
+{
+    switch (eval4_groups(dv)) {
+    case 1: eval4_op<RHS, DISC, K, DC, WS, 1>(dv, op); break;
+    case 2: eval4_op<RHS, DISC, K, DC, WS, 2>(dv, op); break;
+    case 3: eval4_op<RHS, DISC, K, DC, WS, 3>(dv, op); break;
+    default: op.err = hipErrorInvalidConfiguration; break;
+    }
+}
+
+}
diff --git a/varanneal_amd/csrc/va_eval4_builtin.h b/varanneal_amd/csrc/va_eval4_builtin.h
--- /dev/null
+++ b/varanneal_amd/csrc/va_eval4_builtin.h
@@ -0,0 +1,36 @@
+#pragma once
+#include "va_eval4.h"
+
+namespace va {
+
+template <class RHS, int K, int DC, int WS, int G>
+static void eval4_rhs(const Dev &dv, EvalOp &op)
+{
+    with_disc(dv.dm.disc, [&](auto disc) { eval4_op<RHS, decltype(disc)::value, K, DC, WS, G>(dv, op); });
+}
+
+template <class RHS, int K, int G>
+static void eval4_d(const Dev &dv, EvalOp &op)
+{
+    const bool sw = !dv.pp.rm_arr && !dv.pp.rf0_arr, ws = sw && dv.dm.nskip == 1;
+    if (dv.dm.D == 20) {
+        if (ws) eval4_rhs<RHS, K, 20, 1, G>(dv, op);
+        else if (sw) eval4_rhs<RHS, K, 20, 2, G>(dv, op);
+        else eval4_rhs<RHS, K, 20, 0, G>(dv, op);
+    } else { if (ws) eval4_rhs<RHS, K, 0, 1, G>(dv, op); else eval4_rhs<RHS, K, 0, 0, G>(dv, op); }
+}
+
+template <int G>
+static void eval4_builtin(const Dev &dv, EvalOp &op)
+{
+    switch (dv.dm.maxr) {
+    case 4: eval4_d<RhsL96s, 4, G>(dv, op); break;
+    case 5: eval4_d<RhsL96s, 5, G>(dv, op); break;
+    case 6: eval4_d<RhsL96s, 6, G>(dv, op); break;
+    case 7: eval4_d<RhsL96s, 7, G>(dv, op); break;
+    case 12: if (dv.dm.nskip == 1) eval4_rhs<RhsL96s, 12, 20, 1, G>(dv, op); else eval4_rhs<RhsL96s, 12, 20, 2, G>(dv, op); break;
+    default: eval4_d<RhsL96s, 8, G>(dv, op); break;
+    }
+}
+
+}
diff --git a/varanneal_amd/csrc/va_eval4_g2.hip b/varanneal_amd/csrc/va_eval4_g2.hip
--- /dev/null
+++ b/varanneal_amd/csrc/va_eval4_g2.hip
@@ -0,0 +1,10 @@
+#include <hip/hip_runtime.h>
+
+#include "va_device.h"
+#include "va_eval4_builtin.h"
+
+namespace va {
+
+void eval4_builtin_g2(const Dev &dv, EvalOp &op) { eval4_builtin<2>(dv, op); }
+
+}
diff --git a/varanneal_amd/csrc/va_eval4_g3.hip b/varanneal_amd/csrc/va_eval4_g3.hip
--- /dev/null
+++ b/varanneal_amd/csrc/va_eval4_g3.hip
@@ -0,0 +1,10 @@
+#include <hip/hip_runtime.h>
+
+#include "va_device.h"
+#include "va_eval4_builtin.h"
+
+namespace va {
+
+void eval4_builtin_g3(const Dev &dv, EvalOp &op) { eval4_builtin<3>(dv, op); }
+
+}
diff --git a/varanneal_amd/csrc/va_eval_geo.h b/varanneal_amd/csrc/va_eval_geo.h
--- a/varanneal_amd/csrc/va_eval_geo.h
+++ b/varanneal_amd/csrc/va_eval_geo.h
@@ -18,12 +18,14 @@
     bool has_reach5 = false;
     int reach5[4] = {0, 0, 0, 0};
     int lin = 0;
+    int nb = 0;
 };
 
 struct EvalPlan {
     int emode = 0, RY = 0, NT = 0, maxr = 0, T = 0, ntiles = 0;
     int ghost = 2;
     Geo4 g4{};
+    int wg4 = 1;
     Geo5 g5{};
     std::vector<int> ystrip;
 };
@@ -98,6 +100,23 @@
     return true;
 }
 
+inline int eval4_per_cu(int K, int nb) { return (nb > 0 && K <= 7 && K * nb <= 28) ? 3 : 2; }
+
+constexpr int EVAL4_CUS = 256;
+constexpr bool EVAL4_WIDE_DEFAULT = false;
+
+inline int plan_eval4_groups(long batch, int ntiles, int K, int nb, const Geo4 &g4)
+{
+    const int w = eval4_per_cu(K, nb);
+    const long grid1 = batch * ntiles, rounds1 = (grid1 + EVAL4_CUS - 1) / EVAL4_CUS;
+    if (grid1 > (long)EVAL4_CUS * w) return 1;
+    for (int G = w; G > 1; --G) {
+        const long grid = batch * ((ntiles + G - 1) / G), rounds = (grid + EVAL4_CUS - 1) / EVAL4_CUS;
+        if (G * rounds <= rounds1 && sizeof(double) * (size_t)G * g4.NW * g4.WAVE <= 160 * 1024) return G;
+    }
+    return 1;
+}
+
 inline bool plan_eval4(const va_problem_desc *d, const EvalForm &f, EvalPlan &p)
 {
     const int D = d->D, N = d->N_model, ne = f.ne;
@@ -141,6 +160,7 @@
     p.g4 = g4;
     p.emode = 4; p.RY = 4 * RW; p.NT = 256; p.maxr = K; p.T = g4.T;
     p.ntiles = (N + p.T - 1) / p.T;
+    p.wg4 = plan_eval4_groups(d->batch, p.ntiles, K, f.nb, g4);
     return true;
 }
 
@@ -245,6 +265,7 @@
     int ne = 0, ghost = 0, reach[4] = {0, 0, 0, 0};
     int has_linear = 0;
     int n_colp_vectors = 0;
+    int nb = 0;
 
     static ModuleVariant decode(const int *v)
     {
@@ -261,6 +282,7 @@
     {
         EvalForm f = flat_form();
         f.ne = (kernel == 4 || kernel == 5) ? ne : 0;
+        f.nb = kernel == 4 ? nb : 0;
         f.ghost = kernel == 3 ? ghost : 0;
         f.has_reach5 = kernel == 5;
         for (int k = 0; k < 4; ++k) f.reach5[k] = reach[k];
diff --git a/varanneal_amd/csrc/va_kernels.hip b/varanneal_amd/csrc/va_kernels.hip
--- a/varanneal_amd/csrc/va_kernels.hip
+++ b/varanneal_amd/csrc/va_kernels.hip
@@ -7,6 +7,7 @@
 #include "va_predict.h"
 #include "va_predict_tlm.h"
 #include "va_hvp.h"
+#include "va_eval4_builtin.h"
 
 namespace va {
 
@@ -37,34 +38,15 @@
     else eval3_rhs<RHS, K, 0, 1024>(dv, op);
 }
 
-template <class RHS, int K, int DC, int WS>
-static void eval4_rhs(const Dev &dv, EvalOp &op)
-{
-    with_disc(dv.dm.disc, [&](auto disc) { eval4_op<RHS, decltype(disc)::value, K, DC, WS>(dv, op); });
-}
-
-template <class RHS, int K>
-static void eval4_d(const Dev &dv, EvalOp &op)
-{
-    const bool sw = !dv.pp.rm_arr && !dv.pp.rf0_arr, ws = sw && dv.dm.nskip == 1;
-    if (dv.dm.D == 20) {
-        if (ws) eval4_rhs<RHS, K, 20, 1>(dv, op);
-        else if (sw) eval4_rhs<RHS, K, 20, 2>(dv, op);
-        else eval4_rhs<RHS, K, 20, 0>(dv, op);
-    } else { if (ws) eval4_rhs<RHS, K, 0, 1>(dv, op); else eval4_rhs<RHS, K, 0, 0>(dv, op); }
-}
-
 static void eval_builtin(const Dev &dv, EvalOp &op)
 {
     if (dv.dm.emode == 5) eval5_builtin(dv, op);
     else if (dv.dm.emode == 4) {
-        switch (dv.dm.maxr) {
-        case 4: eval4_d<RhsL96s, 4>(dv, op); break;
-        case 5: eval4_d<RhsL96s, 5>(dv, op); break;
-        case 6: eval4_d<RhsL96s, 6>(dv, op); break;
-        case 7: eval4_d<RhsL96s, 7>(dv, op); break;
-        case 12: if (dv.dm.nskip == 1) eval4_rhs<RhsL96s, 12, 20, 1>(dv, op); else eval4_rhs<RhsL96s, 12, 20, 2>(dv, op); break;
-        default: eval4_d<RhsL96s, 8>(dv, op); break;
+        switch (eval4_groups(dv)) {
+        case 1: eval4_builtin<1>(dv, op); break;
+        case 2: eval4_builtin_g2(dv, op); break;
+        case 3: eval4_builtin_g3(dv, op); break;
+        default: op.err = hipErrorInvalidConfiguration; break;
         }
     } else if (dv.dm.emode == 3) {
         switch (dv.dm.maxr) {
diff --git a/varanneal_amd/csrc/va_measure.h b/varanneal_amd/csrc/va_measure.h
--- a/varanneal_amd/csrc/va_measure.h
+++ b/varanneal_amd/csrc/va_measure.h
@@ -2,7 +2,7 @@
 
 #ifdef VA_STAMPS
 #define VA_E4_STAMP_SETUP(dv, w)                                                                                                   \
-    unsigned long long *tl = reinterpret_cast<unsigned long long *>((dv).upp) + ((size_t)blockIdx.x * 4 + (threadIdx.x >> 6)) * 10; \
+    unsigned long long *tl = reinterpret_cast<unsigned long long *>((dv).upp) + ((size_t)blockIdx.x * (blockDim.x >> 6) + (threadIdx.x >> 6)) * 10; \
     if ((threadIdx.x & 63) == 0) {                                                                                                 \
         tl[8] = (unsigned long long)__builtin_amdgcn_s_getreg((31 << 11) | 4);                                                     \
         tl[9] = ((unsigned long long)__builtin_amdgcn_s_getreg((31 << 11) | 20) << 32) | (unsigned long long)(w);                  \
diff --git a/varanneal_amd/csrc/va_user_rhs.hip b/varanneal_amd/csrc/va_user_rhs.hip
--- a/varanneal_amd/csrc/va_user_rhs.hip
+++ b/varanneal_amd/csrc/va_user_rhs.hip
@@ -30,7 +30,7 @@
 #elif VA_USER_VARIANT == 5
 constexpr auto user_eval_var = va::eval5_op<VA_USER_COLT, VA_USER_DISC, VA_USER_COLT::D>;
 #elif VA_USER_VARIANT == 4
-constexpr auto user_eval_var = va::eval4_op<VA_USER_COLT, VA_USER_DISC, VA_USER_K, VA_USER_COLT::D, VA_USER_W != 0>;
+constexpr auto user_eval_var = va::eval4_op_groups<VA_USER_COLT, VA_USER_DISC, VA_USER_K, VA_USER_COLT::D, VA_USER_W != 0>;
 #else
 constexpr auto user_eval_var = va::eval3_op<va::RhsUserG, VA_USER_DISC, VA_USER_K, va::RhsUserG::D, VA_USER_W>;
 #endif
@@ -82,6 +82,9 @@
 #endif
 #endif
 }
+#if defined(VA_USER_VARIANT) && VA_USER_VARIANT == 4
+int va_user_col_neighbours(void) { return VA_USER_COLT::NB; }
+#endif
 #if defined(VA_USER_COLP)
 void va_user_colp_map(int *out)
 {
```
